# 001camellia/Speech-Imagery-EEG

Hardware: AMD Instinct MI355X
Metric: epochs/sec (B=256, C=122, T=1000) IGN 3-class (higher is better)
Workload: dtype f32

## Files before the change

### include/ign_abi.h

```cpp
#ifndef IGN_ABI_H
#define IGN_ABI_H

#include <stddef.h>
#include <stdint.h>

#ifdef __cplusplus
extern "C" {
#endif

#define IGN_ABI_VERSION 1

#define IGN_E_ARG      (-1001)
#define IGN_E_UNSUP    (-1002)
#define IGN_E_TOOBIG   (-1003)

#define IGN_DIST_L1    0
#define IGN_DIST_MSE   1
#define IGN_DIST_COS   2
#define IGN_DIST_PEARS 3
#define IGN_GATE_RBF   0x00
#define IGN_GATE_LTS   0x10

int         ign_abi_version(void);
const char* ign_last_error(void);

int ign_instnorm_fwd(const float* x_btc, float* xn_bct, float* xt_bct, int B, int T, int C, float eps,
                     void* stream);
int ign_instnorm_fwd_amax(const float* x_btc, float* xn_bct, float* xt_bct, int B, int T, int C, float eps, float* amax_slot,
                          void* stream);

int ign_transpose_btc_to_bct(const float* x_btc, float* out_bct, int B, int T, int C, void* stream);

int ign_standardise_nct_to_btc(const float* x_nct, float* out_btc, float* stats_ws, int B, int C, int T, float eps,
                               void* stream);

int ign_shapelet_fwd(const float* xn_bct, const float* w_kcl, const float* thr_kc,
                     float* p_out, float* dmin_out, int ld, int col0,
                     int32_t* tstar, float* zmu, float* d_save, float* xstat_save,
                     int B, int C, int T, int K, int L, int stride, float eps, int mode, void* stream);

int ign_shapelet_fwd_bank(const float* xn_bct, int G, const float* const* w_kcl, const float* const* thr_kc, float* p_out,
                          float* dmin_out, int ld, const int* col0, int32_t* const* tstar, float* const* zmu,
                          float* const* d_save, float* const* xstat_save, int B, int C, int T, const int* K, const int* L,
                          const int* stride, float eps, int mode, void* stream);

size_t ign_shapelet_bwd_workspace_bytes(int B, int C, int T, int K, int L, int stride, int mode);
int ign_shapelet_bwd(const float* xn_bct, const float* w_kcl, const float* g_out, const float* p_out,
                     const float* dmin_out, int ld, int col0,
                     const int32_t* tstar, const float* zmu, const float* d_save,
                     const float* xstat_save, const float* wnorm_kc ,
                     float* gw_kcl, void* workspace,
                     int B, int C, int T, int K, int L, int stride, float eps, int mode, void* stream);

size_t ign_shapelet_bwd_bank_workspace_bytes(int G, int B, int C, int T, const int* K, const int* L, const int* stride, int mode);
int ign_shapelet_bwd_bank(const float* xn_bct, int G, const float* const* w_kcl, const float* g_out, const float* p_out,
                          const float* dmin_out, int ld, const int* col0, const int32_t* const* tstar, const float* const* zmu,
                          const float* const* d_save, const float* const* xstat_save, const float* const* wnorm_kc,
                          float* const* gw_kcl, const float* const* gw_add, const float* add_scale_dev, void* workspace,
                          int B, int C, int T, const int* K, const int* L, const int* stride, float eps, int mode, void* stream);

int ign_attn_fwd(const float* q, const float* k, const float* v, float* out, float* lse,
                 int B, int L, int S, int H, int E,
                 long long q_sb, long long q_sl, long long k_sb, long long k_sl, long long v_sb, long long v_sl,
                 float scale, void* stream);
int ign_attn_fwd_x6(const float* q, const float* k, const float* v, float* out, float* lse, int B, int L, int S, int H, int E,
                    long long q_sb, long long q_sl, long long k_sb, long long k_sl, long long v_sb, long long v_sl,
                    float scale, void* stream);
int ign_attn_bwd(const float* q, const float* k, const float* v, const float* out, const float* lse, const float* gout,
                 float* gq, float* gk, float* gv, float* delta_ws,
                 int B, int L, int S, int H, int E,
                 long long q_sb, long long q_sl, long long k_sb, long long k_sl, long long v_sb, long long v_sl,
                 float scale, void* stream);
int ign_attn_bwd_x6(const float* q, const float* k, const float* v, const float* out, const float* lse, const float* gout,
                 float* gq, float* gk, float* gv, float* delta_ws,
                 int B, int L, int S, int H, int E,
                 long long q_sb, long long q_sl, long long k_sb, long long k_sl, long long v_sb, long long v_sl,
                 float scale, void* stream);
int ign_attn_fwd_bf16(const float* q, const float* k, const float* v, float* out, float* lse, int B, int L, int S, int H, int E,
                    long long q_sb, long long q_sl, long long k_sb, long long k_sl, long long v_sb, long long v_sl,
                    float scale, void* stream);
int ign_attn_bwd_bf16(const float* q, const float* k, const float* v, const float* out, const float* lse, const float* gout,
                 float* gq, float* gk, float* gv, float* delta_ws,
                 int B, int L, int S, int H, int E,
                 long long q_sb, long long q_sl, long long k_sb, long long k_sl, long long v_sb, long long v_sl,
                 float scale, void* stream);
int ign_attn_bwd_x6_strided(const float* q, const float* k, const float* v, const float* out, const float* lse, const float* gout,
                 float* gq, float* gk, float* gv, float* delta_ws,
                 int B, int L, int S, int H, int E,
                 long long q_sb, long long q_sl, long long k_sb, long long k_sl, long long v_sb, long long v_sl,
                 float scale, void* stream,
                            long long g_sb, long long g_sl, int bf16);

int ign_attn_fwd_h3(const float* q, const float* k, const float* v, float* out, float* lse,
                    int B, int L, int S, int H, int E,
                    long long q_sb, long long q_sl, long long k_sb, long long k_sl, long long v_sb, long long v_sl,
                    float scale, void* stream, const float* bq, const float* bk, const float* bv);
int ign_attn_bwd_h3(const float* q, const float* k, const float* v, const float* out, const float* lse, const float* gout,
                    float* gq, float* gk, float* gv, float* delta_ws,
                    int B, int L, int S, int H, int E,
                    long long q_sb, long long q_sl, long long k_sb, long long k_sl, long long v_sb, long long v_sl,
                    float scale, void* stream, long long g_sb, long long g_sl,
                    const float* bq, const float* bk, const float* bv, const float* bgo,
                    float* g_amax );

#define IGN_ATTN_MATH_F32  0
#define IGN_ATTN_MATH_X6   1
#define IGN_ATTN_MATH_BF16 2
#define IGN_ATTN_MATH_H3   3
int ign_attn_fwd_dropout(const float* q, const float* k, const float* v, float* out, float* lse,
                         int B, int L, int S, int H, int E,
                         long long q_sb, long long q_sl, long long k_sb, long long k_sl, long long v_sb, long long v_sl,
                         float scale, void* stream, int math, const float* bq, const float* bk, const float* bv,
                         float p, unsigned long long seed);
int ign_attn_bwd_dropout(const float* q, const float* k, const float* v, const float* out, const float* lse, const float* gout,
                         float* gq, float* gk, float* gv, float* delta_ws,
                         int B, int L, int S, int H, int E,
                         long long q_sb, long long q_sl, long long k_sb, long long k_sl, long long v_sb, long long v_sl,
                         float scale, void* stream, int math, long long g_sb, long long g_sl,
                         const float* bq, const float* bk, const float* bv, const float* bgo, float* g_amax,
                         float p, unsigned long long seed);
int ign_attn_dropout_mask(unsigned char* keep, int B, int H, int L, int S, float p, unsigned long long seed, void* stream);

int ign_head_fwd(const float* X, const float* W, const float* bias, float* out, int B, int F, int N, long long ldx,
                 void* stream);
int ign_head_bwd(const float* g_out, const float* X, const float* W, float* gX, float* gW, float* gbias,
                 int B, int F, int N, long long ldx, void* stream);
int ign_head_bwd_acc(const float* g_out, const float* X, const float* W, float* gX, float* gW, float* gbias,
                     const float* gW_add, const float* add_scale_dev, int B, int F, int N, long long ldx, void* stream);

int ign_gate_fwd(const float* sbm, const float* dnn, float* out, float* eta, int B, int N, float gating_value,
                 int use_gating_value, void* stream);
int ign_gate_bwd(const float* sbm, const float* dnn, const float* gout, const float* geta, float* gsbm, float* gdnn,
                 int B, int N, float gating_value, int use_gating_value, void* stream);

int ign_loss_fwd_bwd(const float* sbm, const float* dnn, const long long* labels, float* out, float* eta, float* loss2,
                     float* gsbm, float* gdnn, int B, int N, float beta, void* stream);
int ign_loss_fwd_bwd_reg(const float* sbm, const float* dnn, const long long* labels, const float* reg, float* out, float* eta,
                         float* loss2, float* gsbm, float* gdnn, int B, int N, float beta, void* stream);

int ign_diversity_fwd_bwd(const float* w_kcl, float* loss_part_c, float* gw_kcl, int K, int C, int L, float eps,
                          void* stream);

size_t ign_sbm_reg_workspace_bytes(int G, int C, long long nW);
int ign_sbm_reg_fwd_bwd(const float* W, float* gW_reg, long long nW, float lambda_reg, int G, const float* const* w_kcl,
                        float* const* gw_kcl, const int* K, const int* L, int C, float lambda_div, float eps, float* loss_out,
                        void* workspace, void* stream);

int ign_adam_step(float* param, const float* grad, float* exp_avg, float* exp_avg_sq, long long n, float lr,
                  float beta1, float beta2, float eps, int step, void* stream);

int ign_gather_flat(const void* const* src, const long long* off, const long long* n, int count, float* flat, void* stream);

int ign_adam_step_dev(float* param, const float* grad, float* exp_avg, float* exp_avg_sq, long long n, float lr,
                      float beta1, float beta2, float eps, int* step_dev, float* bc_dev, void* stream);

size_t ign_conv1_sumsq_workspace_bytes(int rows, int F1, int k1);
int ign_conv1_sumsq_fwd(const float* x, const float* w1, const float* mu, float* m2, void* workspace,
                        int rows, int T, int F1, int k1, int pad_left, void* stream);
int ign_conv1_sumsq_bwd(const float* x, const float* w1, const float* mu, float* g_fj, void* workspace,
                        int rows, int T, int F1, int k1, int pad_left, void* stream);

long long ign_layernorm_parts(long long R, int D);
int ign_layernorm_fwd(const float* x, const float* gamma, const float* beta, float* y, float* mean, float* rstd, long long R, int D,
                      float eps, void* stream);
int ign_layernorm_res_fwd(const float* x, const float* res, float* sum, const float* gamma, const float* beta, float* y,
                          float* mean, float* rstd, long long R, int D, float eps, void* stream);
int ign_layernorm_bwd(const float* x, const float* gy, const float* gamma, const float* mean, const float* rstd, float* gx,
                      float* dgamma, float* dbeta, float* part, long long R, int D, void* stream);
int ign_layernorm_bwd_amax(const float* x, const float* gy, const float* gamma, const float* mean, const float* rstd, float* gx,
                           float* dgamma, float* dbeta, float* part, float* amax_slot, long long R, int D, void* stream);
long long ign_autocorr_parts(int rows);
int ign_autocorr_fwd(const float* x_rows, float* part, int rows, int T, int K, void* stream);
long long ign_edge_lagprod_parts(int rows);
int ign_edge_lagprod_fwd(const float* x_rows, float* part, int rows, int T, int k, int pad_left, void* stream);
size_t ign_bn1_data_stats_workspace_bytes(int rows, int T, int k);
int ign_bn1_data_stats(const float* x_rows, int rows, int T, int k, int pad_left, void* workspace, double* G, double* S, void* stream);
int ign_autocorr_sum_fwd(const float* x_rows, float* part, float* rowsum_part, int rows, int T, int K, int* used_parts, void* stream);
int ign_bn1_fold_fwd(const float* w1, const float* gamma, const float* beta, const float* rs, const double* G, const double* S,
                     double n, float eps, float momentum, float* running_mean, float* running_var, float* alpha, float* cshift,
                     double* saved , int F1, int k, int Dm, void* stream);
int ign_bn1_fold_bwd(const float* g_alpha, const float* g_cshift, const float* w1, const float* gamma, const float* rs,
                     const double* S, const double* saved, double n, float* g_w1, float* g_gamma, float* g_beta, float* g_rs,
                     int F1, int k, int Dm, void* stream);
int ign_dwconv1d_fwd(const float* x, const float* w, float* y, int B, int C, int T, int k, int pad_left, int flip,
                     void* stream);
size_t ign_dwconv1d_bwd_weight_workspace_bytes(int B, int C, int k);
int ign_dwconv1d_bwd_weight(const float* x, const float* dy, float* dw, void* workspace, int B, int C, int T, int k,
                            int pad_left, void* stream);

int ign_chan_contract_fwd(const float* x_bct, const float* wt_ci64, float* u_bot, int B, int Ci, int Co, int T, void* stream);
size_t ign_chan_contract_bwd_weight_workspace_bytes(int B, int Ci, int Co, int T);
int ign_chan_contract_bwd_weight(const float* du_bot, const float* x_bct, float* dw_oc, void* workspace, int B, int Ci, int Co,
                                 int T, void* stream);

size_t ign_chan_stats_workspace_bytes(int B, int C);
int ign_chan_stats(const float* v_bct, double* sums_c2, void* workspace, int B, int C, int T, void* stream);
int ign_affine_elu_pool_fwd(const float* v_bct, const float* scale_c, const float* shift_c, float* out, int B, int C, int T, int P,
                            void* stream);
int ign_bn_elu_pool_bwd_sums(const float* v_bct, const float* dout, const float* scale_c, const float* shift_c, const float* mean_c,
                             double* sums_c2, void* workspace, int B, int C, int T, int P, void* stream);
int ign_bn_elu_pool_bwd_apply(const float* v_bct, const float* dout, const float* scale_c, const float* shift_c, const float* ka_c,
                              const float* kb_c, const float* kc_c, float* dv_bct, int B, int C, int T, int P, void* stream);
int ign_bn_fold_fwd(const double* sums_c2, const float* alpha_c, const float* cshift_c, const float* gamma_c, const float* beta_c,
                    float* scale_c, float* shift_c, double* fold_c2, float* running_mean, float* running_var, int C, long long n,
                    float eps, float momentum, void* stream);
int ign_bn_fold_bwd(const double* sums_c2, const double* fold_c2, const float* alpha_c, const float* gamma_c, float* ka_c, float* kb_c,
                    float* kc_c, float* dgamma_c, float* dbeta_c, float* dalpha_c, int C, long long n, float eps, void* stream);

long long ign_clconv_mtiles(long long M);
int ign_clconv_pack_weights(const float* w_oik, float* wt_fwd, float* wt_dgrad, int Co, int Ci, int k, void* stream);
int ign_clconv_fwd(const float* x, const float* wt_fwd, const float* bias, const float* pro_a, const float* pro_b,
                   float* y, float* stat_part, int B, int Tin, int Ci, int Co, int k, void* stream);
int ign_clconv_dgrad(const float* dyp, const float* wt_dgrad, const float* y_in, const float* a_in, const float* b_in,
                     const float* mean_in, const float* invstd_in, float* g_in, float* stat_part,
                     int B, int Tin, int Ci, int Co, int k, void* stream);
int ign_clconv_kpad(int C);
long long ign_clconv_x3_elems(int rows, int chans, int k);
long long ign_clconv_x6_mtiles(int B, int rows);
int ign_clconv_pack_weights_x3(const float* w_oik, void* wt3_fwd, void* wt3_dgrad, int Co, int Ci, int k, void* stream);
int ign_clconv_fwd_x6(const float* x, const void* wt3_fwd, const float* bias, const float* pro_a, const float* pro_b,
                      float* y, float* stat_part, int B, int Tin, int Ci, int Co, int k, void* stream);
int ign_clconv_dgrad_x6(const float* dyp, const void* wt3_dgrad, const float* y_in, const float* a_in, const float* b_in,
                        const float* mean_in, const float* invstd_in, float* g_in, float* stat_part,
                        int B, int Tin, int Ci, int Co, int k, void* stream);
size_t ign_clconv_wgrad_x6_workspace_bytes(int B, int Tin, int Ci, int Co, int k);
int ign_clconv_wgrad_x6(const float* dyp, int dy_pad, const float* x, const float* pro_a, const float* pro_b,
                        float* dw_oik, void* workspace, int B, int Tin, int Ci, int Co, int k, void* stream);
int ign_clconv_wgrad_x6_nsplit(int B, int Tin, int Ci, int Co, int k);
int ign_clconv_wgrad_reduce_multi(int n, const void* const* part, float* const* dw_oik, const int* nsplit, const int* Co,
                                  const int* Ci, const int* k, void* stream);
int ign_clconv_pack_weights_x3_multi(int n, const float* const* w_oik, void* const* wt3_fwd, void* const* wt3_dgrad,
                                     const int* Co, const int* Ci, const int* k, long long* const* counters, void* stream);

int ign_absmax(const float* x, long long n, float* slot , void* stream);
int ign_absmax_multi(int n, const float* const* x, const long long* count, float* const* slots, void* stream);
int ign_fcn_scan(int nl, const float* const* w, const long long* nw, const float* const* gamma_prev, const float* const* beta_prev,
                 const int* C_prev, const long long* R_prev, float* slots , float* zero, long long nzero,
                 void* stream);
int ign_clconv_pack_weights_h2_multi(int n, const float* const* w_oik, void* const* wt_fwd, void* const* wt_dgrad, const int* Co,
                                     const int* Ci, const int* k, long long* const* counters, const float* const* w_bounds,
                                     void* stream);
int ign_clconv_fwd_h3(const float* x, const void* wt_h2, const float* bias, const float* pro_a, const float* pro_b, float* y,
                      float* stat_part, const float* bound_in, const float* bound_w, int B, int Tin, int Ci, int Co, int k,
                      void* stream);
int ign_clconv_fwd_h3_amax(const float* x, const void* wt_h2, const float* bias, const float* pro_a, const float* pro_b, float* y,
                           float* stat_part, const float* bound_in, const float* bound_w, float* amax_out, int B, int Tin, int Ci,
                           int Co, int k, void* stream);
int ign_linear_dgrad_gelu_h3(const float* g, const void* wd_h2, const float* u, float* du, const float* bound_g, const float* bound_w,
                             float* amax_out, long long M, int Co, int Ci, void* stream);
int ign_clconv_dgrad_h3(const float* dyp, const void* wt_h2_dgrad, const float* y_in, const float* a_in, const float* b_in,
                        const float* mean_in, const float* invstd_in, float* g_in, float* stat_part, const float* bound_dy,
                        const float* bound_w, int B, int Tin, int Ci, int Co, int k, void* stream);
int ign_clconv_wgrad_h3(const float* dyp, int dy_pad, const float* x, const float* pro_a, const float* pro_b, float* dw_oik,
                        void* workspace, const float* bound_dy, const float* bound_x, int B, int Tin, int Ci, int Co, int k,
                        void* stream);
int ign_linear_wgrad_h3(const float* dy, const float* x, float* dw, float* db, void* workspace, const float* bound_dy,
                        const float* bound_x, long long M, int Ci, int Co, void* stream);
int ign_bn_bwd_apply_amax(const float* g, const float* y, const float* a, const float* mean, const float* invstd,
                          const float* dbeta, const float* dgamma, float* dyp, float* amax_slot, int B, int T, int C, int pad,
                          int training, void* stream);

int ign_clconv_fwd_bf16(const float* x, const void* wt3_fwd, const float* bias, const float* pro_a, const float* pro_b,
                        float* y, float* stat_part, int B, int Tin, int Ci, int Co, int k, void* stream);
int ign_clconv_dgrad_bf16(const float* dyp, const void* wt3_dgrad, const float* y_in, const float* a_in, const float* b_in,
                          const float* mean_in, const float* invstd_in, float* g_in, float* stat_part,
                          int B, int Tin, int Ci, int Co, int k, void* stream);
int ign_clconv_wgrad_bf16(const float* dyp, int dy_pad, const float* x, const float* pro_a, const float* pro_b,
                          float* dw_oik, void* workspace, int B, int Tin, int Ci, int Co, int k, void* stream);
int ign_linear_wgrad_x6(const float* dy, const float* x, float* dw, float* db, void* workspace, long long M, int Ci, int Co,
                        void* stream);
int ign_linear_wgrad_bf16(const float* dy, const float* x, float* dw, float* db, void* workspace, long long M, int Ci, int Co,
                          void* stream);
size_t ign_clconv_wgrad_workspace_bytes(int B, int Tin, int Ci, int Co, int k);
int ign_clconv_wgrad(const float* dyp, int dy_pad, const float* x, const float* pro_a, const float* pro_b,
                     float* dw_oik, void* workspace, int B, int Tin, int Ci, int Co, int k, void* stream);

int ign_bn_finalize_fwd(const float* part, int nparts, long long R, int C, const float* gamma, const float* beta,
                        float eps, float momentum, float* running_mean, float* running_var,
                        float* a, float* b, float* mean, float* invstd, void* stream);
int ign_bn_affine_eval(const float* running_mean, const float* running_var, const float* gamma, const float* beta,
                       float eps, int C, float* a, float* b, float* mean, float* invstd, void* stream);
int ign_bn_relu_pool_fwd(const float* y, const float* a, const float* b, float* pooled, int B, int T, int C, void* stream);
int ign_bn_relu_pool_head_fwd(const float* y, const float* a, const float* b, float* pooled, const float* W, const float* bias,
                              float* logits, int B, int T, int C, int N, void* stream);
long long ign_bn_relu_pool_bwd_parts(int B, int T);
int ign_bn_relu_pool_bwd(const float* y, const float* gpool, const float* a, const float* b, const float* mean,
                         const float* invstd, float* g, float* part, int B, int T, int C, void* stream);
int ign_bn_finalize_bwd(const float* part, int nparts, int C, float* dbeta, float* dgamma, void* stream);
int ign_bn_bwd_apply(const float* g, const float* y, const float* a, const float* mean, const float* invstd,
                     const float* dbeta, const float* dgamma, float* dyp, int B, int T, int C, int pad, int training,
                     void* stream);

int ign_timing_enable(int on);
int ign_timing_read(const char* label, double* total_ms, long long* launches);

#ifdef __cplusplus
}
#endif
#endif
```

### speech-imagery-eeg_amd/csrc/ign_bn.hip

```cpp
#include "ign_clconv.h"

__device__ __forceinline__ void atomic_absmax(float* slot, float v) { ign_atomic_absmax(slot, v); }
__device__ __forceinline__ float block_max_1024(float v, float* sh) {
#pragma unroll
    for (int o = 32; o > 0; o >>= 1) v = fmaxf(v, __shfl_xor(v, o, 64));
    if ((threadIdx.x & 63) == 0) sh[threadIdx.x >> 6] = v;
    __syncthreads();
    if (threadIdx.x == 0) {
        const int nw = (blockDim.x + 63) >> 6;
        for (int i = 1; i < nw; ++i) v = fmaxf(v, sh[i]);
    }
    return v;
}


constexpr int BN_CH = 8, BN_SL = 128;
__device__ __forceinline__ void bn_sum_partials(const float* __restrict__ part, int nparts, int C, double* s_out, double* q_out) {
    __shared__ double sh[2][BN_SL][BN_CH + 1];
    const int cl = threadIdx.x % BN_CH, sl = threadIdx.x / BN_CH;
    const int c = blockIdx.x * BN_CH + cl;
    double s = 0.0, q = 0.0;
    if (c < C) {
        const int per = (nparts + BN_SL - 1) / BN_SL;
        const int i0 = sl * per, i1 = min(nparts, i0 + per);
        float fs = 0.f, fq = 0.f;
        int n = 0;
        for (int i = i0; i < i1; ++i) {
            fs += part[((size_t)i * 2 + 0) * C + c];
            fq += part[((size_t)i * 2 + 1) * C + c];
            if (++n == 64) { s += (double)fs; q += (double)fq; fs = fq = 0.f; n = 0; }
        }
        s += (double)fs; q += (double)fq;
    }
    sh[0][sl][cl] = s;
    sh[1][sl][cl] = q;
    __syncthreads();
    s = q = 0.0;
    if (sl == 0) {
        for (int k = 0; k < BN_SL; ++k) { s += sh[0][k][cl]; q += sh[1][k][cl]; }
    }
    *s_out = s; *q_out = q;
}

__global__ void __launch_bounds__(1024) bn_finalize_fwd_kernel(const float* __restrict__ part, int nparts, long long R, int C,
                                       const float* __restrict__ gamma, const float* __restrict__ beta, float eps, float momentum,
                                       float* __restrict__ run_mean, float* __restrict__ run_var, float* __restrict__ a,
                                       float* __restrict__ b, float* __restrict__ mean_out, float* __restrict__ invstd_out) {
    double s, q;
    bn_sum_partials(part, nparts, C, &s, &q);
    const int c = blockIdx.x * BN_CH + threadIdx.x % BN_CH;
    if (threadIdx.x / BN_CH != 0 || c >= C) return;
    const double m = s / (double)R;
    double var = q / (double)R - m * m;
    if (var < 0.0) var = 0.0;
    const float inv = (float)(1.0 / sqrt(var + (double)eps));
    const float av = gamma[c] * inv;
    a[c] = av;
    b[c] = beta[c] - av * (float)m;
    mean_out[c] = (float)m;
    invstd_out[c] = inv;
    if (run_mean) {
        run_mean[c] = (1.f - momentum) * run_mean[c] + momentum * (float)m;
        const double unb = (R > 1) ? var * (double)R / (double)(R - 1) : var;
        run_var[c] = (1.f - momentum) * run_var[c] + momentum * (float)unb;
    }
}

__global__ void bn_affine_eval_kernel(const float* __restrict__ run_mean, const float* __restrict__ run_var,
                                      const float* __restrict__ gamma, const float* __restrict__ beta, float eps, int C,
                                      float* __restrict__ a, float* __restrict__ b, float* __restrict__ mean_out,
                                      float* __restrict__ invstd_out) {
    const int c = blockIdx.x * 256 + threadIdx.x;
    if (c >= C) return;
    const float inv = 1.f / sqrtf(run_var[c] + eps);
    const float av = gamma[c] * inv;
    a[c] = av;
    b[c] = beta[c] - av * run_mean[c];
    mean_out[c] = run_mean[c];
    invstd_out[c] = inv;
}

__global__ void __launch_bounds__(1024) bn_finalize_bwd_kernel(const float* __restrict__ part, int nparts, int C,
                                                               float* __restrict__ dbeta, float* __restrict__ dgamma) {
    double s, q;
    bn_sum_partials(part, nparts, C, &s, &q);
    const int c = blockIdx.x * BN_CH + threadIdx.x % BN_CH;
    if (threadIdx.x / BN_CH != 0 || c >= C) return;
    dbeta[c] = (float)s;
    dgamma[c] = (float)q;
}

__global__ void __launch_bounds__(256) bn_relu_pool_fwd_kernel(const float* __restrict__ y, const float* __restrict__ a,
                                                               const float* __restrict__ b, float* __restrict__ pooled, int T,
                                                               int C, const float* __restrict__ W,
                                                               const float* __restrict__ bias, float* __restrict__ logits, int N) {
    extern __shared__ float sm[];
    const int c4 = C / 4, rif = 256 / c4;
    const int col = (threadIdx.x % c4) * 4, rofs = threadIdx.x / c4;
    const float* yb = y + (size_t)blockIdx.x * T * C;
    float s[4] = {0.f, 0.f, 0.f, 0.f};
    if (rofs < rif) {
        const float4 av = *reinterpret_cast<const float4*>(a + col), bv = *reinterpret_cast<const float4*>(b + col);
        for (int t = rofs; t < T; t += rif) {
            const float4 yv = *reinterpret_cast<const float4*>(yb + (size_t)t * C + col);
            s[0] += fmaxf(fmaf(av.x, yv.x, bv.x), 0.f);
            s[1] += fmaxf(fmaf(av.y, yv.y, bv.y), 0.f);
            s[2] += fmaxf(fmaf(av.z, yv.z, bv.z), 0.f);
            s[3] += fmaxf(fmaf(av.w, yv.w, bv.w), 0.f);
        }
#pragma unroll
        for (int q = 0; q < 4; ++q) sm[rofs * C + col + q] = s[q];
    }
    __syncthreads();
    for (int c = threadIdx.x; c < C; c += 256) {
        float u = 0.f;
        for (int q = 0; q < rif; ++q) u += sm[q * C + c];
        u /= (float)T;
        pooled[(size_t)blockIdx.x * C + c] = u;
        if (W) sm[c] = u;
    }
    if (!W) return;
    __syncthreads();
    const int wave = threadIdx.x >> 6, lane = threadIdx.x & 63;
    for (int n = wave; n < N; n += 4) {
        float u = 0.f;
        for (int c = lane; c < C; c += 64) u = fmaf(sm[c], W[(size_t)n * C + c], u);
#pragma unroll
        for (int o = 32; o > 0; o >>= 1) u += __shfl_xor(u, o, 64);
        if (lane == 0) logits[(size_t)blockIdx.x * N + n] = u + (bias ? bias[n] : 0.f);
    }
}

constexpr int POOL_ROWS = 128;
__global__ void __launch_bounds__(256) bn_relu_pool_bwd_kernel(const float* __restrict__ y, const float* __restrict__ gpool,
                                                               const float* __restrict__ a, const float* __restrict__ b,
                                                               const float* __restrict__ mean, const float* __restrict__ invstd,
                                                               float* __restrict__ g, float* __restrict__ part, int T, int C) {
    extern __shared__ float sm[];
    const int c4 = C / 4, rif = 256 / c4;
    const int col = (threadIdx.x % c4) * 4, rofs = threadIdx.x / c4;
    const int bi = blockIdx.y;
    const int t0 = blockIdx.x * POOL_ROWS, t1 = min(T, t0 + POOL_ROWS);
    float s0[4] = {0.f, 0.f, 0.f, 0.f}, s1[4] = {0.f, 0.f, 0.f, 0.f};
    if (rofs < rif) {
        float av[4], bv[4], mv[4], iv[4], gp[4];
        vload<4>(av, a + col); vload<4>(bv, b + col); vload<4>(mv, mean + col); vload<4>(iv, invstd + col);
        vload<4>(gp, gpool + (size_t)bi * C + col);
        const float invT = 1.f / (float)T;
        for (int t = t0 + rofs; t < t1; t += rif) {
            const size_t off = ((size_t)bi * T + t) * C + col;
            float yy[4], gg[4];
            vload<4>(yy, y + off);
#pragma unroll
            for (int q = 0; q < 4; ++q) {
                gg[q] = (fmaf(av[q], yy[q], bv[q]) > 0.f) ? gp[q] * invT : 0.f;
                s0[q] += gg[q];
                s1[q] = fmaf(gg[q], (yy[q] - mv[q]) * iv[q], s1[q]);
            }
            vstore<4>(g + off, gg);
        }
#pragma unroll
        for (int q = 0; q < 4; ++q) { sm[rofs * C + col + q] = s0[q]; sm[(rif + rofs) * C + col + q] = s1[q]; }
    }
    __syncthreads();
    const size_t pi = (size_t)bi * gridDim.x + blockIdx.x;
    for (int c = threadIdx.x; c < C; c += 256) {
        float u = 0.f, v = 0.f;
        for (int q = 0; q < rif; ++q) { u += sm[q * C + c]; v += sm[(rif + q) * C + c]; }
        part[(pi * 2 + 0) * C + c] = u;
        part[(pi * 2 + 1) * C + c] = v;
    }
}

constexpr int APPLY_ROWS = 64;
__global__ void __launch_bounds__(256) bn_bwd_apply_kernel(const float* __restrict__ g, const float* __restrict__ y,
                                                           const float* __restrict__ a, const float* __restrict__ mean,
                                                           const float* __restrict__ invstd, const float* __restrict__ dbeta,
                                                           const float* __restrict__ dgamma, float* __restrict__ dyp, int T, int C,
                                                           int pad, long long rows_padded, float invR, int training,
                                                           float* __restrict__ amax_slot) {
    const int c4 = C / 4, rif = 256 / c4;
    const int col = (threadIdx.x % c4) * 4, rofs = threadIdx.x / c4;
    if (rofs >= rif) return;
    float amax = 0.f;
    float ca[4], c1[4], c0[4];
    vload<4>(ca, a + col);
    if (training) {
        float mv[4], iv[4], db[4], dg[4];
        vload<4>(mv, mean + col); vload<4>(iv, invstd + col); vload<4>(db, dbeta + col); vload<4>(dg, dgamma + col);
#pragma unroll
        for (int q = 0; q < 4; ++q) {
            c1[q] = -ca[q] * iv[q] * dg[q] * invR;
            c0[q] = -ca[q] * (db[q] - mv[q] * iv[q] * dg[q]) * invR;
        }
    } else {
#pragma unroll
        for (int q = 0; q < 4; ++q) c1[q] = c0[q] = 0.f;
    }
    const int Tp = T + 2 * pad;
    const long long r0 = (long long)blockIdx.x * APPLY_ROWS;
    const long long r1 = min(rows_padded, r0 + APPLY_ROWS);
    for (long long row = r0 + rofs; row < r1; row += rif) {
        const long long bi = row / Tp;
        const int tp = (int)(row - bi * Tp);
        float out[4] = {0.f, 0.f, 0.f, 0.f};
        if (tp >= pad && tp < pad + T) {
            const size_t off = ((size_t)bi * T + (tp - pad)) * C + col;
            float gg[4], yy[4] = {0.f, 0.f, 0.f, 0.f};
            vload<4>(gg, g + off);
            if (training) vload<4>(yy, y + off);
#pragma unroll
            for (int q = 0; q < 4; ++q) { out[q] = fmaf(ca[q], gg[q], fmaf(c1[q], yy[q], c0[q])); amax = fmaxf(amax, fabsf(out[q])); }
        }
        vstore<4>(dyp + (size_t)row * C + col, out);
    }
    if (amax_slot) {
#pragma unroll
        for (int o = 32; o > 0; o >>= 1) amax = fmaxf(amax, __shfl_xor(amax, o, 64));
        if ((threadIdx.x & 63) == 0) atomic_absmax(amax_slot, amax);
    }
}

__global__ void __launch_bounds__(256) absmax_kernel(const float* __restrict__ x, long long n, float* __restrict__ slot) {
    __shared__ float sh[16];
    float m = 0.f;
    const long long n4 = n >> 2;
    for (long long i = (long long)blockIdx.x * 256 + threadIdx.x; i < n4; i += (long long)gridDim.x * 256) {
        const float4 v = reinterpret_cast<const float4*>(x)[i];
        m = fmaxf(fmaxf(m, fmaxf(fabsf(v.x), fabsf(v.y))), fmaxf(fabsf(v.z), fabsf(v.w)));
    }
    if (blockIdx.x == 0)
        for (long long i = (n4 << 2) + threadIdx.x; i < n; i += 256) m = fmaxf(m, fabsf(x[i]));
    m = block_max_1024(m, sh);
    if (threadIdx.x == 0) atomic_absmax(slot, m);
}

constexpr int AMM_MAX = 16;
struct AbsmaxMultiTable { const float* x[AMM_MAX]; long long n[AMM_MAX]; float* slot[AMM_MAX]; };
__global__ void __launch_bounds__(256) absmax_multi_kernel(const AbsmaxMultiTable t) {
    __shared__ float sh[16];
    const int g = blockIdx.y;
    const float* __restrict__ x = t.x[g];
    const long long n = t.n[g];
    float m = 0.f;
    if (((uintptr_t)x & 15) == 0) {
        const long long n4 = n >> 2;
        for (long long i = (long long)blockIdx.x * 256 + threadIdx.x; i < n4; i += (long long)gridDim.x * 256) {
            const float4 v = reinterpret_cast<const float4*>(x)[i];
            m = fmaxf(fmaxf(m, fmaxf(fabsf(v.x), fabsf(v.y))), fmaxf(fabsf(v.z), fabsf(v.w)));
        }
        if (blockIdx.x == 0)
            for (long long i = (n4 << 2) + threadIdx.x; i < n; i += 256) m = fmaxf(m, fabsf(x[i]));
    } else {
        for (long long i = (long long)blockIdx.x * 256 + threadIdx.x; i < n; i += (long long)gridDim.x * 256) m = fmaxf(m, fabsf(x[i]));
    }
    m = block_max_1024(m, sh);
    if (threadIdx.x == 0) atomic_absmax(t.slot[g], m);
}

constexpr int SCAN_LMAX = 8;
struct FcnScanTable {
    const float* w[SCAN_LMAX]; long long nw[SCAN_LMAX];
    const float* gamma[SCAN_LMAX]; const float* beta[SCAN_LMAX]; int C[SCAN_LMAX]; float sqrtR[SCAN_LMAX];
};
__global__ void __launch_bounds__(1024) fcn_scan_kernel(const FcnScanTable t, float* __restrict__ slots, float* __restrict__ zero,
                                                        long long nzero) {
    __shared__ float sh[16];
    const int l = blockIdx.x;
    for (long long i = (long long)l * 1024 + threadIdx.x; i < nzero; i += (long long)gridDim.x * 1024) zero[i] = 0.f;
    float m = 0.f;
    for (long long i = threadIdx.x; i < t.nw[l]; i += 1024) m = fmaxf(m, fabsf(t.w[l][i]));
    m = block_max_1024(m, sh);
    if (threadIdx.x == 0) slots[4 * l + 0] = m;
    __syncthreads();
    float a = 0.f;
    if (t.gamma[l])
        for (int c = threadIdx.x; c < t.C[l]; c += 1024) a = fmaxf(a, fmaf(fabsf(t.gamma[l][c]), t.sqrtR[l], fabsf(t.beta[l][c])));
    a = block_max_1024(a, sh);
    if (threadIdx.x == 0) { slots[4 * l + 1] = a; slots[4 * l + 2] = 0.f; slots[4 * l + 3] = 0.f; }
}

extern "C" int ign_absmax(const float* x, long long n, float* slot, void* stream) {
    if (!x || !slot || n <= 0 || ((uintptr_t)x & 15)) { ign_set_error("ign_absmax: null / unaligned pointer or n <= 0"); return IGN_E_ARG; }
    const long long blocks = (n / 4 + 256 * 8 - 1) / (256 * 8);
    IgnScopedTimer tm("absmax", (hipStream_t)stream);
    hipLaunchKernelGGL(absmax_kernel, dim3((unsigned)(blocks < 1 ? 1 : (blocks > 2048 ? 2048 : blocks))), dim3(256), 0,
                       (hipStream_t)stream, x, n, slot);
    return ign_check_launch("absmax_kernel");
}

extern "C" int ign_absmax_multi(int n, const float* const* x, const long long* count, float* const* slots, void* stream) {
    if (n <= 0 || n > AMM_MAX || !x || !count || !slots) { ign_set_error("ign_absmax_multi: n=%d outside 1..%d or null table", n, AMM_MAX); return IGN_E_ARG; }
    AbsmaxMultiTable t;
    long long nmax = 0;
    for (int i = 0; i < n; ++i) {
        if (!x[i] || !slots[i] || count[i] <= 0) { ign_set_error("ign_absmax_multi: tensor %d: null pointer or empty", i); return IGN_E_ARG; }
        t.x[i] = x[i]; t.n[i] = count[i]; t.slot[i] = slots[i];
        nmax = count[i] > nmax ? count[i] : nmax;
    }
    long long blocks = (nmax / 4 + 256 * 8 - 1) / (256 * 8);
    blocks = blocks < 1 ? 1 : (blocks > 256 ? 256 : blocks);
    IgnScopedTimer tm("absmax", (hipStream_t)stream);
    hipLaunchKernelGGL(absmax_multi_kernel, dim3((unsigned)blocks, (unsigned)n), dim3(256), 0, (hipStream_t)stream, t);
    return ign_check_launch("absmax_multi_kernel");
}

extern "C" int ign_fcn_scan(int nl, const float* const* w, const long long* nw, const float* const* gamma_prev,
                            const float* const* beta_prev, const int* C_prev, const long long* R_prev, float* slots, float* zero,
                            long long nzero, void* stream) {
    if (nzero < 0 || (nzero > 0 && !zero)) { ign_set_error("ign_fcn_scan: nzero=%lld with zero=%p", nzero, (void*)zero); return IGN_E_ARG; }
    if (nl <= 0 || nl > SCAN_LMAX || !w || !nw || !slots) { ign_set_error("ign_fcn_scan: nl=%d outside 1..%d or null table", nl, SCAN_LMAX); return IGN_E_ARG; }
    FcnScanTable t;
    for (int l = 0; l < nl; ++l) {
        if (!w[l] || nw[l] <= 0) { ign_set_error("ign_fcn_scan: layer %d: null weights", l); return IGN_E_ARG; }
        t.w[l] = w[l]; t.nw[l] = nw[l];
        const bool has = gamma_prev && gamma_prev[l];
        if (has && (!beta_prev || !beta_prev[l] || !C_prev || !R_prev || C_prev[l] <= 0 || R_prev[l] <= 1)) {
            ign_set_error("ign_fcn_scan: layer %d: BatchNorm in front needs beta, C > 0 and R > 1", l);
            return IGN_E_ARG;
        }
        t.gamma[l] = has ? gamma_prev[l] : nullptr; t.beta[l] = has ? beta_prev[l] : nullptr;
        t.C[l] = has ? C_prev[l] : 0; t.sqrtR[l] = has ? sqrtf((float)(R_prev[l] - 1)) : 0.f;
    }
    hipLaunchKernelGGL(fcn_scan_kernel, dim3(nl), dim3(1024), 0, (hipStream_t)stream, t, slots, zero, nzero);
    return ign_check_launch("fcn_scan_kernel");
}

static int bn_check(const char* who, long long R, int C) {
    if (R <= 0 || C <= 0 || (C & 3) || C > 1024) {
        ign_set_error("%s: need R > 0 and 4 <= C <= 1024 with C %% 4 == 0 (R=%lld C=%d)", who, R, C);
        return IGN_E_ARG;
    }
    return 0;
}

extern "C" int ign_bn_finalize_fwd(const float* part, int nparts, long long R, int C, const float* gamma, const float* beta,
                                   float eps, float momentum, float* running_mean, float* running_var, float* a, float* b,
                                   float* mean, float* invstd, void* stream) {
    if (!part || nparts <= 0 || R <= 0 || C <= 0 || !gamma || !beta || !a || !b || !mean || !invstd) {
        ign_set_error("ign_bn_finalize_fwd: bad argument");
        return IGN_E_ARG;
    }
    hipLaunchKernelGGL(bn_finalize_fwd_kernel, dim3((C + BN_CH - 1) / BN_CH), dim3(BN_CH * BN_SL), 0, (hipStream_t)stream, part, nparts, R, C, gamma, beta,
                       eps, momentum, running_mean, running_var, a, b, mean, invstd);
    return ign_check_launch("bn_finalize_fwd_kernel");
}

extern "C" int ign_bn_affine_eval(const float* running_mean, const float* running_var, const float* gamma, const float* beta,
                                  float eps, int C, float* a, float* b, float* mean, float* invstd, void* stream) {
    if (!running_mean || !running_var || !gamma || !beta || C <= 0 || !a || !b || !mean || !invstd) {
        ign_set_error("ign_bn_affine_eval: bad argument");
        return IGN_E_ARG;
    }
    hipLaunchKernelGGL(bn_affine_eval_kernel, dim3((C + 255) / 256), dim3(256), 0, (hipStream_t)stream, running_mean, running_var,
                       gamma, beta, eps, C, a, b, mean, invstd);
    return ign_check_launch("bn_affine_eval_kernel");
}

extern "C" int ign_bn_finalize_bwd(const float* part, int nparts, int C, float* dbeta, float* dgamma, void* stream) {
    if (!part || nparts <= 0 || C <= 0 || !dbeta || !dgamma) {
        ign_set_error("ign_bn_finalize_bwd: bad argument");
        return IGN_E_ARG;
    }
    hipLaunchKernelGGL(bn_finalize_bwd_kernel, dim3((C + BN_CH - 1) / BN_CH), dim3(BN_CH * BN_SL), 0, (hipStream_t)stream, part, nparts, C, dbeta, dgamma);
    return ign_check_launch("bn_finalize_bwd_kernel");
}

extern "C" int ign_bn_relu_pool_fwd(const float* y, const float* a, const float* b, float* pooled, int B, int T, int C,
                                    void* stream) {
    int rc;
    if ((rc = bn_check("ign_bn_relu_pool_fwd", (long long)B * T, C))) return rc;
    if (!y || !a || !b || !pooled) { ign_set_error("ign_bn_relu_pool_fwd: null pointer"); return IGN_E_ARG; }
    const int rif = 256 / (C / 4);
    IgnScopedTimer tm("bn_relu_pool_fwd", (hipStream_t)stream);
    hipLaunchKernelGGL(bn_relu_pool_fwd_kernel, dim3(B), dim3(256), (size_t)rif * C * 4, (hipStream_t)stream, y, a, b, pooled, T, C,
                       (const float*)nullptr, (const float*)nullptr, (float*)nullptr, 0);
    return ign_check_launch("bn_relu_pool_fwd_kernel");
}

extern "C" int ign_bn_relu_pool_head_fwd(const float* y, const float* a, const float* b, float* pooled, const float* W,
                                         const float* bias, float* logits, int B, int T, int C, int N, void* stream) {
    int rc;
    if ((rc = bn_check("ign_bn_relu_pool_head_fwd", (long long)B * T, C))) return rc;
    if (!y || !a || !b || !pooled || !W || !logits || N <= 0) {
        ign_set_error("ign_bn_relu_pool_head_fwd: null pointer or N=%d", N);
        return IGN_E_ARG;
    }
    const int rif = 256 / (C / 4);
    IgnScopedTimer tm("bn_relu_pool_fwd", (hipStream_t)stream);
    hipLaunchKernelGGL(bn_relu_pool_fwd_kernel, dim3(B), dim3(256), (size_t)rif * C * 4, (hipStream_t)stream, y, a, b, pooled, T, C,
                       W, bias, logits, N);
    return ign_check_launch("bn_relu_pool_fwd_kernel");
}

extern "C" long long ign_bn_relu_pool_bwd_parts(int B, int T) { return (long long)B * ((T + POOL_ROWS - 1) / POOL_ROWS); }

extern "C" int ign_bn_relu_pool_bwd(const float* y, const float* gpool, const float* a, const float* b, const float* mean,
                                    const float* invstd, float* g, float* part, int B, int T, int C, void* stream) {
    int rc;
    if ((rc = bn_check("ign_bn_relu_pool_bwd", (long long)B * T, C))) return rc;
    if (!y || !gpool || !a || !b || !mean || !invstd || !g || !part) { ign_set_error("ign_bn_relu_pool_bwd: null pointer"); return IGN_E_ARG; }
    const int rif = 256 / (C / 4);
    IgnScopedTimer tm("bn_relu_pool_bwd", (hipStream_t)stream);
    hipLaunchKernelGGL(bn_relu_pool_bwd_kernel, dim3((T + POOL_ROWS - 1) / POOL_ROWS, B), dim3(256), (size_t)2 * rif * C * 4,
                       (hipStream_t)stream, y, gpool, a, b, mean, invstd, g, part, T, C);
    return ign_check_launch("bn_relu_pool_bwd_kernel");
}

extern "C" int ign_bn_bwd_apply(const float* g, const float* y, const float* a, const float* mean, const float* invstd,
                                const float* dbeta, const float* dgamma, float* dyp, int B, int T, int C, int pad, int training,
                                void* stream) {
    return ign_bn_bwd_apply_amax(g, y, a, mean, invstd, dbeta, dgamma, dyp, nullptr, B, T, C, pad, training, stream);
}

extern "C" int ign_bn_bwd_apply_amax(const float* g, const float* y, const float* a, const float* mean, const float* invstd,
                                     const float* dbeta, const float* dgamma, float* dyp, float* amax_slot, int B, int T, int C,
                                     int pad, int training, void* stream) {
    int rc;
    if ((rc = bn_check("ign_bn_bwd_apply", (long long)B * T, C))) return rc;
    if (!g || !a || !dyp || pad < 0 || (training && (!y || !mean || !invstd || !dbeta || !dgamma))) {
        ign_set_error("ign_bn_bwd_apply: null pointer / negative pad");
        return IGN_E_ARG;
    }
    const long long rows = (long long)B * (T + 2 * pad);
    IgnScopedTimer tm("bn_bwd_apply", (hipStream_t)stream);
    hipLaunchKernelGGL(bn_bwd_apply_kernel, dim3((unsigned)((rows + APPLY_ROWS - 1) / APPLY_ROWS)), dim3(256), 0, (hipStream_t)stream,
                       g, y, a, mean, invstd, dbeta, dgamma, dyp, T, C, pad, rows, 1.0f / (float)((long long)B * T), training, amax_slot);
    return ign_check_launch("bn_bwd_apply_kernel");
}
```

### speech-imagery-eeg_amd/csrc/ign_clconv.h

```cpp
#pragma once
#include "ign_common.h"

typedef float f32x16 __attribute__((ext_vector_type(16)));
#define MFMA32(a, b, c) __builtin_amdgcn_mfma_f32_32x32x2f32((a), (b), (c), 0, 0, 0)

__device__ __forceinline__ int acc_row16(int r, int h) { return (r & 3) + 8 * (r >> 2) + 4 * h; }

constexpr int TM = 128, TN = 128, KC = 16;
constexpr int NT_PITCH = KC + 4;
constexpr int TN_PITCH = 128 + 8;

struct RowMap {
    int rows_logical;
    int row0;
    int row_pitch;
    long long sample_pitch;
};
__device__ __forceinline__ long long row_off(const RowMap& rm, int m) {
    const int s = m / rm.rows_logical;
    const int r = m - s * rm.rows_logical;
    return (long long)s * rm.sample_pitch + (long long)(rm.row0 + r) * rm.row_pitch;
}

template <int V> struct VecT;
template <> struct VecT<1> { typedef float T; };
template <> struct VecT<2> { typedef float2 T; };
template <> struct VecT<4> { typedef float4 T; };

template <int V>
__device__ __forceinline__ void vload(float (&d)[V], const float* p) {
    if (V == 4) { const float4 t = *reinterpret_cast<const float4*>(p); d[0] = t.x; d[1] = t.y; d[2] = t.z; d[3] = t.w; }
    else if (V == 2) { const float2 t = *reinterpret_cast<const float2*>(p); d[0] = t.x; d[1] = t.y; }
    else d[0] = *p;
}
template <int V>
__device__ __forceinline__ void vstore(float* p, const float (&d)[V]) {
    if (V == 4) *reinterpret_cast<float4*>(p) = make_float4(d[0], d[1], d[2], d[3]);
    else if (V == 2) *reinterpret_cast<float2*>(p) = make_float2(d[0], d[1]);
    else *p = d[0];
}

enum { EPI_BIAS_STATS = 0, EPI_MASK_STATS = 1, EPI_GELU_BWD = 2 };

__device__ __forceinline__ float ign_gelu_grad(float u) {
    const float cdf = 0.5f * (1.f + erff(u * 0.70710678118654752f));
    const float pdf = 0.3989422804014327f * expf(-0.5f * u * u);
    return fmaf(u, pdf, cdf);
}

struct GemmNTArgs {
    const float* A; RowMap am; int K;
    const float* Bt; int ldb;
    float* C; int M, N;
    const float* bias;
    const float* pro_a; const float* pro_b; int pro_c;
    float* part;
    const float* ey; const float* ea; const float* eb; const float* emean; const float* einv;
    int mtiles, ntiles;
    const unsigned short* B3; int Kp;
    float* amax_out;
};

template <int EPI, bool FULL, bool SC = false>
__device__ __forceinline__ void nt_epilogue_body(const GemmNTArgs& a, const f32x16 (&acc)[2][2], float (&s1)[2], float (&s2)[2],
                                                 int m0, int n0, int m_lim, float osc = 1.f) {
    const int lane = threadIdx.x & 63, wave = threadIdx.x >> 6;
    const int l31 = lane & 31, h = lane >> 5;
    const int wm = wave & 1, wn = wave >> 1;
    float amax = 0.f;
#pragma unroll
    for (int j = 0; j < 2; ++j) {
        const int n = n0 + wn * 64 + j * 32 + l31;
        const bool n_ok = FULL || n < a.N;
        const int nc = n_ok ? n : a.N - 1;
        const float bv = (EPI == EPI_BIAS_STATS && a.bias) ? a.bias[nc] : 0.f;
        float ea = 0.f, eb = 0.f, em = 0.f, ei = 0.f;
        if (EPI == EPI_MASK_STATS) { ea = a.ea[nc]; eb = a.eb[nc]; em = a.emean[nc]; ei = a.einv[nc]; }
#pragma unroll
        for (int i = 0; i < 2; ++i) {
            const int mb = m0 + wm * 64 + i * 32;
            float yv[16];
            if (EPI == EPI_MASK_STATS || EPI == EPI_GELU_BWD) {
#pragma unroll
                for (int r = 0; r < 16; ++r) {
                    const int m = mb + acc_row16(r, h);
                    const int mc = FULL ? m : min(m, m_lim - 1);
                    yv[r] = a.ey[(long long)mc * a.N + nc];
                }
            }
#pragma unroll
            for (int r = 0; r < 16; ++r) {
                const int m = mb + acc_row16(r, h);
                const bool ok = FULL || (n_ok && m < m_lim);
                float v = SC ? acc[i][j][r] * osc : acc[i][j][r];
                if (EPI == EPI_BIAS_STATS) {
                    v += bv;
                    if (ok) { s1[j] += v; s2[j] = fmaf(v, v, s2[j]); }
                } else if (EPI == EPI_GELU_BWD) {
                    v *= ign_gelu_grad(yv[r]);
                } else {
                    v = (fmaf(ea, yv[r], eb) > 0.f) ? v : 0.f;
                    if (ok) { s1[j] += v; s2[j] = fmaf(v, (yv[r] - em) * ei, s2[j]); }
                }
                if (ok) a.C[(long long)m * a.N + n] = v;
                if (SC && ok) amax = fmaxf(amax, fabsf(v));
            }
        }
    }
    if (SC && a.amax_out) {
#pragma unroll
        for (int o = 32; o > 0; o >>= 1) amax = fmaxf(amax, __shfl_xor(amax, o, 64));
        if (lane == 0) ign_atomic_absmax(a.amax_out, amax);
    }
}

template <int EPI, bool SC = false>
__device__ __forceinline__ void nt_epilogue(const GemmNTArgs& a, const f32x16 (&acc)[2][2], float* red, int mt, int m0, int n0,
                                            int m_lim, float osc = 1.f) {
    const int tid = threadIdx.x, lane = tid & 63, wave = tid >> 6;
    const int l31 = lane & 31, h = lane >> 5;
    const int wm = wave & 1, wn = wave >> 1;
    float s1[2] = {0.f, 0.f}, s2[2] = {0.f, 0.f};
    if (m0 + TM <= m_lim && n0 + TN <= a.N) nt_epilogue_body<EPI, true, SC>(a, acc, s1, s2, m0, n0, m_lim, osc);
    else nt_epilogue_body<EPI, false, SC>(a, acc, s1, s2, m0, n0, m_lim, osc);
    if (a.part) {
#pragma unroll
        for (int j = 0; j < 2; ++j) {
            s1[j] += __shfl_xor(s1[j], 32, 64);
            s2[j] += __shfl_xor(s2[j], 32, 64);
            if (h == 0) {
                const int col = wn * 64 + j * 32 + l31;
                red[(wm * 2 + 0) * TN + col] = s1[j];
                red[(wm * 2 + 1) * TN + col] = s2[j];
            }
        }
        __syncthreads();
        if (tid < TN && n0 + tid < a.N) {
            a.part[((long long)mt * 2 + 0) * a.N + n0 + tid] = red[0 * TN + tid] + red[2 * TN + tid];
            a.part[((long long)mt * 2 + 1) * a.N + n0 + tid] = red[1 * TN + tid] + red[3 * TN + tid];
        }
    }
}


struct ConvX6Args {
    GemmNTArgs g;
    long long sample_pitch;
    int rows_in;
    int cin, cp, k;
    int trows;
    int tps;
    int nprod;
    const float* bound_a;
    const float* bound_b;
};

__device__ __forceinline__ float ign_pow2_scale(const float* bound) {
    if (!bound) return 1.f;
    const float b = *bound;
    if (!(b > 0.f) || !(b < INFINITY)) return 1.f;
    int e;
    (void)frexpf(b, &e);
    e = 14 - e;
    e = e < -60 ? -60 : (e > 60 ? 60 : e);
    return ldexpf(1.f, e);
}

inline int ign_vec_width(int c) { return (c % 4 == 0) ? 4 : (c % 2 == 0) ? 2 : 1; }

int ign_clconv_launch_x6t(const ConvX6Args& a, int epi, int V, bool pro, hipStream_t s);
int ign_clconv_launch_wgrad_reduce(const float* part, float* dw_oik, int nsplit, int Co, int Ci, int k, hipStream_t s);
```

### speech-imagery-eeg_amd/csrc/ign_clconv_f32.hip

```cpp
#include "ign_clconv.h"

template <int V, bool PRO, int EPI>
__global__ void __launch_bounds__(256, 2) clconv_nt_kernel(const GemmNTArgs a) {
    constexpr int VPR = KC / V;
    constexpr int RPP = 256 / VPR;
    constexpr int NPASS = TM / RPP;
    __shared__ __attribute__((aligned(16))) float smem[2][(TM + TN) * NT_PITCH];

    const int nwg = a.mtiles * a.ntiles;
    int lid = blockIdx.x;
    {
        const int per = nwg / 8;
        if (lid < per * 8) lid = (lid & 7) * per + (lid >> 3);
    }
    const int mt = lid / a.ntiles, nt = lid - mt * a.ntiles;
    const int m0 = mt * TM, n0 = nt * TN;

    const int tid = threadIdx.x, lane = tid & 63, wave = tid >> 6;
    const int l31 = lane & 31, h = lane >> 5;
    const int wm = wave & 1, wn = wave >> 1;

    const int sq = tid % VPR, sr = tid / VPR;
    const float* arow[NPASS];
    const float* brow[NPASS];
// ... 148 lines not shown
#pragma unroll
                for (int v = 0; v < VQ; ++v) rq[i][v] = 0.f;
                rq_ok[i] = false;
            }
        }
    };
    auto lstore = [&](int buf) {
        float* Ps = smem[buf];
        float* Qs = Ps + KC * TN_PITCH;
#pragma unroll
        for (int i = 0; i < 2; ++i) vstore<4>(Ps + (pr + 8 * i) * TN_PITCH + pc, rp[i]);
#pragma unroll
        for (int i = 0; i < QNPASS; ++i) {
            if (PRO && rq_ok[i]) {
#pragma unroll
                for (int v = 0; v < VQ; ++v) rq[i][v] = fmaxf(fmaf(qa[v], rq[i][v], qb[v]), 0.f);
            }
            vstore<VQ>(Qs + (qr + QRPP * i) * TN_PITCH + qc, rq[i]);
        }
    };

    if (m_begin < m_end) {
        gload(m_begin);
        lstore(0);
    }
    __syncthreads();
    int buf = 0;
    for (int mb = m_begin; mb < m_end; mb += KC, buf ^= 1) {
        if (mb + KC < m_end) gload(mb + KC);
        const float* Ps = smem[buf] + h * TN_PITCH + wm * 64 + 2 * l31;
        const float* Qs = smem[buf] + KC * TN_PITCH + h * TN_PITCH + wn * 64 + 2 * l31;
#pragma unroll
        for (int s = 0; s < KC / 2; ++s) {
            const float2 pv = *reinterpret_cast<const float2*>(Ps + 2 * s * TN_PITCH);
            const float2 qv = *reinterpret_cast<const float2*>(Qs + 2 * s * TN_PITCH);
            acc[0][0] = MFMA32(pv.x, qv.x, acc[0][0]);
            acc[0][1] = MFMA32(pv.x, qv.y, acc[0][1]);
            acc[1][0] = MFMA32(pv.y, qv.x, acc[1][0]);
            acc[1][1] = MFMA32(pv.y, qv.y, acc[1][1]);
        }
        if (mb + KC < m_end) lstore(buf ^ 1);
        __syncthreads();
    }

    float* out = a.part + (long long)split * a.NP * a.NQ;
    const int kk = q0 + wn * 64 + 2 * l31;
#pragma unroll
    for (int i = 0; i < 2; ++i)
#pragma unroll
        for (int r = 0; r < 16; ++r) {
            const int co = p0 + wm * 64 + 2 * acc_row16(r, h) + i;
            if (co < a.NP) {
                float* o = out + (long long)co * a.NQ + kk;
                if (!(a.NQ & 1) && kk + 1 < a.NQ) {
                    *reinterpret_cast<float2*>(o) = make_float2(acc[i][0][r], acc[i][1][r]);
                } else {
                    if (kk < a.NQ) o[0] = acc[i][0][r];
                    if (kk + 1 < a.NQ) o[1] = acc[i][1][r];
                }
            }
        }
}

__global__ void __launch_bounds__(256) wgrad_reduce_kernel(const float* __restrict__ part, float* __restrict__ dw, int nsplit,
                                                           int Co, int Ci, int k) {
    const long long n = (long long)Co * Ci * k;
    const long long i = (long long)blockIdx.x * 256 + threadIdx.x;
    if (i >= n) return;
    float s = 0.f;
    int p = 0;
    for (; p + 8 <= nsplit; p += 8) {
        float v[8];
#pragma unroll
        for (int u = 0; u < 8; ++u) v[u] = part[(long long)(p + u) * n + i];
#pragma unroll
        for (int u = 0; u < 8; ++u) s += v[u];
    }
    for (; p < nsplit; ++p) s += part[(long long)p * n + i];
    const int ci = (int)(i % Ci);
    const long long t = i / Ci;
    const int j = (int)(t % k);
    const long long co = t / k;
    dw[(co * Ci + ci) * k + j] = s;
}

constexpr int WRED_LMAX = 8;
struct WgradReduceTable {
    const float* part[WRED_LMAX];
    float* dw[WRED_LMAX];
    int nsplit[WRED_LMAX], Co[WRED_LMAX], Ci[WRED_LMAX], k[WRED_LMAX];
};
__global__ void __launch_bounds__(256) wgrad_reduce_multi_kernel(const WgradReduceTable t) {
    const int l = blockIdx.y;
    const int Co = t.Co[l], Ci = t.Ci[l], k = t.k[l], nsplit = t.nsplit[l];
    const float* __restrict__ part = t.part[l];
    const long long n = (long long)Co * Ci * k;
    const long long i = (long long)blockIdx.x * 256 + threadIdx.x;
    if (i >= n) return;
    float s = 0.f;
    int p = 0;
    for (; p + 8 <= nsplit; p += 8) {
        float v[8];
#pragma unroll
        for (int u = 0; u < 8; ++u) v[u] = part[(long long)(p + u) * n + i];
#pragma unroll
        for (int u = 0; u < 8; ++u) s += v[u];
    }
    for (; p < nsplit; ++p) s += part[(long long)p * n + i];
    const int ci = (int)(i % Ci);
    const long long tt = i / Ci;
    const int j = (int)(tt % k);
    const long long co = tt / k;
    t.dw[l][(co * Ci + ci) * k + j] = s;
}

extern "C" int ign_clconv_wgrad_reduce_multi(int n, const void* const* part, float* const* dw_oik, const int* nsplit, const int* Co,
                                             const int* Ci, const int* k, void* stream) {
    if (n <= 0 || n > WRED_LMAX || !part || !dw_oik || !nsplit || !Co || !Ci || !k) {
        ign_set_error("ign_clconv_wgrad_reduce_multi: n=%d outside 1..%d or null table", n, WRED_LMAX);
        return IGN_E_ARG;
    }
    WgradReduceTable t;
    long long nmax = 0;
    for (int l = 0; l < n; ++l) {
        if (!part[l] || !dw_oik[l] || nsplit[l] <= 0 || Co[l] <= 0 || Ci[l] <= 0 || k[l] <= 0) {
            ign_set_error("ign_clconv_wgrad_reduce_multi: layer %d: bad argument", l);
            return IGN_E_ARG;
        }
        t.part[l] = (const float*)part[l]; t.dw[l] = dw_oik[l]; t.nsplit[l] = nsplit[l]; t.Co[l] = Co[l]; t.Ci[l] = Ci[l]; t.k[l] = k[l];
        const long long e = (long long)Co[l] * Ci[l] * k[l];
        nmax = e > nmax ? e : nmax;
    }
    hipLaunchKernelGGL(wgrad_reduce_multi_kernel, dim3((unsigned)((nmax + 255) / 256), (unsigned)n), dim3(256), 0, (hipStream_t)stream, t);
    return ign_check_launch("wgrad_reduce_multi_kernel");
}

__global__ void __launch_bounds__(256) pack_weights_kernel(const float* __restrict__ w, float* __restrict__ wt,
                                                           float* __restrict__ wd, int Co, int Ci, int k) {
    const long long n = (long long)Co * Ci * k;
    const long long i = (long long)blockIdx.x * 256 + threadIdx.x;
    if (i >= n) return;
    const int j = (int)(i % k);
    const long long t = i / k;
    const int ci = (int)(t % Ci);
    const long long co = t / Ci;
    const float v = w[i];
    wt[(co * k + j) * Ci + ci] = v;
    if (wd) wd[((long long)ci * k + (k - 1 - j)) * Co + co] = v;
}

template <int EPI>
static int launch_nt(const GemmNTArgs& a, int V, bool pro, hipStream_t s) {
    const dim3 grid((unsigned)(a.mtiles * a.ntiles)), block(256);
#define IGN_NT(VV, PP) hipLaunchKernelGGL((clconv_nt_kernel<VV, PP, EPI>), grid, block, 0, s, a)
    if (V == 4) { if (pro) IGN_NT(4, true); else IGN_NT(4, false); }
    else if (V == 2) { if (pro) IGN_NT(2, true); else IGN_NT(2, false); }
    else { if (pro) IGN_NT(1, true); else IGN_NT(1, false); }
#undef IGN_NT
    return ign_check_launch("clconv_nt_kernel");
}

extern "C" long long ign_clconv_mtiles(long long M) { return (M + TM - 1) / TM; }

extern "C" int ign_clconv_pack_weights(const float* w_oik, float* wt_fwd, float* wt_dgrad, int Co, int Ci, int k, void* stream) {
    if (!w_oik || !wt_fwd || Co <= 0 || Ci <= 0 || k <= 0) {
        ign_set_error("ign_clconv_pack_weights: bad argument (Co=%d Ci=%d k=%d)", Co, Ci, k);
        return IGN_E_ARG;
    }
    const long long n = (long long)Co * Ci * k;
    hipLaunchKernelGGL(pack_weights_kernel, dim3((unsigned)((n + 255) / 256)), dim3(256), 0, (hipStream_t)stream, w_oik, wt_fwd,
                       wt_dgrad, Co, Ci, k);
    return ign_check_launch("pack_weights_kernel");
}

static int clconv_fwd_impl(const char* who, int x6, const float* x, const void* wt, const float* bias, const float* pro_a,
                           const float* pro_b, float* y, float* stat_part, int B, int Tin, int Ci, int Co, int k, void* stream,
                           const float* bound_a = nullptr, const float* bound_w = nullptr, float* amax_out = nullptr,
                           int epi = EPI_BIAS_STATS, const float* ey = nullptr) {
    const int Tout = Tin - k + 1;
    if (!x || !wt || !y || B <= 0 || Ci <= 0 || Co <= 0 || k <= 0 || Tout <= 0 || ((pro_a == nullptr) != (pro_b == nullptr))) {
        ign_set_error("%s: bad argument (B=%d Tin=%d Ci=%d Co=%d k=%d)", who, B, Tin, Ci, Co, k);
        return IGN_E_ARG;
    }
    const long long M = (long long)B * Tout;
    if (M > 0x7fffffffLL / 2) { ign_set_error("%s: B*Tout = %lld rows exceed the 2^30 row index space", who, M); return IGN_E_TOOBIG; }
    GemmNTArgs a{};
    a.A = x; a.am = RowMap{Tout, 0, Ci, (long long)Tin * Ci}; a.K = k * Ci;
    a.Bt = x6 ? nullptr : (const float*)wt; a.ldb = k * Ci; a.C = y; a.M = (int)M; a.N = Co; a.bias = bias;
    a.B3 = x6 ? (const unsigned short*)wt : nullptr; a.Kp = 0;
    a.pro_a = pro_a; a.pro_b = pro_b; a.pro_c = Ci; a.part = stat_part; a.amax_out = amax_out; a.ey = ey;
    a.mtiles = (int)((M + TM - 1) / TM); a.ntiles = (Co + TN - 1) / TN;
    IgnScopedTimer tm("clconv_fwd", (hipStream_t)stream);
    if (x6) {
        if (k > 16) { ign_set_error("%s: k=%d > 16 taps", who, k); return IGN_E_UNSUP; }
        ConvX6Args c{};
        c.g = a;
        c.cin = Ci; c.cp = (Ci + 15) / 16 * 16; c.k = k; c.g.Kp = k * c.cp;
        c.sample_pitch = (long long)Tin * Ci; c.rows_in = Tin; c.trows = Tout; c.tps = (Tout + TM - 1) / TM;
        c.g.mtiles = B * c.tps; c.nprod = x6; c.bound_a = bound_a; c.bound_b = bound_w;
        return ign_clconv_launch_x6t(c, epi, ign_vec_width(Ci), pro_a != nullptr, (hipStream_t)stream);
    }
    if (epi != EPI_BIAS_STATS) { ign_set_error("%s: epilogue %d needs the split kernels", who, epi); return IGN_E_UNSUP; }
    return launch_nt<EPI_BIAS_STATS>(a, ign_vec_width(Ci), pro_a != nullptr, (hipStream_t)stream);
}

extern "C" int ign_clconv_fwd(const float* x, const float* wt, const float* bias, const float* pro_a, const float* pro_b,
                              float* y, float* stat_part, int B, int Tin, int Ci, int Co, int k, void* stream) {
    return clconv_fwd_impl("ign_clconv_fwd", 0, x, wt, bias, pro_a, pro_b, y, stat_part, B, Tin, Ci, Co, k, stream);
}

extern "C" int ign_clconv_fwd_x6(const float* x, const void* wt3, const float* bias, const float* pro_a, const float* pro_b,
                                 float* y, float* stat_part, int B, int Tin, int Ci, int Co, int k, void* stream) {
    return clconv_fwd_impl("ign_clconv_fwd_x6", 6, x, wt3, bias, pro_a, pro_b, y, stat_part, B, Tin, Ci, Co, k, stream);
}

extern "C" int ign_clconv_fwd_bf16(const float* x, const void* wt3, const float* bias, const float* pro_a, const float* pro_b,
                                   float* y, float* stat_part, int B, int Tin, int Ci, int Co, int k, void* stream) {
    return clconv_fwd_impl("ign_clconv_fwd_bf16", 1, x, wt3, bias, pro_a, pro_b, y, stat_part, B, Tin, Ci, Co, k, stream);
}

extern "C" int ign_clconv_fwd_h3(const float* x, const void* wt_h2, const float* bias, const float* pro_a, const float* pro_b,
                                 float* y, float* stat_part, const float* bound_in, const float* bound_w, int B, int Tin, int Ci,
                                 int Co, int k, void* stream) {
    return ign_clconv_fwd_h3_amax(x, wt_h2, bias, pro_a, pro_b, y, stat_part, bound_in, bound_w, nullptr, B, Tin, Ci, Co, k, stream);
}

extern "C" int ign_clconv_fwd_h3_amax(const float* x, const void* wt_h2, const float* bias, const float* pro_a, const float* pro_b,
                                      float* y, float* stat_part, const float* bound_in, const float* bound_w, float* amax_out, int B,
                                      int Tin, int Ci, int Co, int k, void* stream) {
    if (!bound_in || !bound_w) { ign_set_error("ign_clconv_fwd_h3: null operand bound"); return IGN_E_ARG; }
    return clconv_fwd_impl("ign_clconv_fwd_h3", 3, x, wt_h2, bias, pro_a, pro_b, y, stat_part, B, Tin, Ci, Co, k, stream, bound_in,
                           bound_w, amax_out);
}

extern "C" int ign_linear_dgrad_gelu_h3(const float* g, const void* wd_h2, const float* u, float* du, const float* bound_g,
                                        const float* bound_w, float* amax_out, long long M, int Co, int Ci, void* stream) {
    if (!bound_g || !bound_w || !u) { ign_set_error("ign_linear_dgrad_gelu_h3: null bound / pre-activation"); return IGN_E_ARG; }
    if (M <= 0 || M > 0x3fffffffLL || Ci % 256 || Co % 4) {
        ign_set_error("ign_linear_dgrad_gelu_h3: needs 0 < M < 2^30, Ci %% 256 == 0, Co %% 4 == 0 (M=%lld Co=%d Ci=%d)", M, Co, Ci);
        return IGN_E_UNSUP;
    }
    return clconv_fwd_impl("ign_linear_dgrad_gelu_h3", 3, g, wd_h2, nullptr, nullptr, nullptr, du, nullptr, 1, (int)M, Co, Ci, 1, stream,
                           bound_g, bound_w, amax_out, EPI_GELU_BWD, u);
}

static int clconv_dgrad_impl(const char* who, int x6, const float* dyp, const void* wt_dgrad, const float* y_in, const float* a_in,
                             const float* b_in, const float* mean_in, const float* invstd_in, float* g_in, float* stat_part, int B,
                             int Tin, int Ci, int Co, int k, void* stream, const float* bound_a = nullptr,
                             const float* bound_w = nullptr) {
    const int Tout = Tin - k + 1;
    if (!dyp || !wt_dgrad || !y_in || !a_in || !b_in || !mean_in || !invstd_in || !g_in || B <= 0 || Ci <= 0 || Co <= 0 || k <= 0 ||
        Tout <= 0) {
        ign_set_error("%s: bad argument (B=%d Tin=%d Ci=%d Co=%d k=%d)", who, B, Tin, Ci, Co, k);
        return IGN_E_ARG;
    }
    const long long M = (long long)B * Tin;
    if (M > 0x7fffffffLL / 2) { ign_set_error("%s: B*Tin = %lld rows exceed the 2^30 row index space", who, M); return IGN_E_TOOBIG; }
    GemmNTArgs a{};
    a.A = dyp; a.am = RowMap{Tin, 0, Co, (long long)(Tout + 2 * (k - 1)) * Co}; a.K = k * Co;
    a.Bt = x6 ? nullptr : (const float*)wt_dgrad; a.ldb = k * Co; a.C = g_in; a.M = (int)M; a.N = Ci;
    a.B3 = x6 ? (const unsigned short*)wt_dgrad : nullptr; a.Kp = 0;
    a.part = stat_part; a.ey = y_in; a.ea = a_in; a.eb = b_in; a.emean = mean_in; a.einv = invstd_in;
    a.mtiles = (int)((M + TM - 1) / TM); a.ntiles = (Ci + TN - 1) / TN;
    IgnScopedTimer tm("clconv_dgrad", (hipStream_t)stream);
    if (x6) {
        if (k > 16) { ign_set_error("%s: k=%d > 16 taps", who, k); return IGN_E_UNSUP; }
        ConvX6Args c{};
        c.g = a;
        c.cin = Co; c.cp = (Co + 15) / 16 * 16; c.k = k; c.g.Kp = k * c.cp;
        c.sample_pitch = (long long)(Tout + 2 * (k - 1)) * Co; c.rows_in = Tout + 2 * (k - 1); c.trows = Tin; c.tps = (Tin + TM - 1) / TM;
        c.g.mtiles = B * c.tps; c.nprod = x6; c.bound_a = bound_a; c.bound_b = bound_w;
        return ign_clconv_launch_x6t(c, EPI_MASK_STATS, ign_vec_width(Co), false, (hipStream_t)stream);
    }
    return launch_nt<EPI_MASK_STATS>(a, ign_vec_width(Co), false, (hipStream_t)stream);
}

extern "C" int ign_clconv_dgrad(const float* dyp, const float* wt_dgrad, const float* y_in, const float* a_in, const float* b_in,
                                const float* mean_in, const float* invstd_in, float* g_in, float* stat_part, int B, int Tin,
                                int Ci, int Co, int k, void* stream) {
    return clconv_dgrad_impl("ign_clconv_dgrad", 0, dyp, wt_dgrad, y_in, a_in, b_in, mean_in, invstd_in, g_in, stat_part, B, Tin,
                             Ci, Co, k, stream);
}

extern "C" int ign_clconv_dgrad_x6(const float* dyp, const void* wt3_dgrad, const float* y_in, const float* a_in, const float* b_in,
                                   const float* mean_in, const float* invstd_in, float* g_in, float* stat_part, int B, int Tin,
                                   int Ci, int Co, int k, void* stream) {
    return clconv_dgrad_impl("ign_clconv_dgrad_x6", 6, dyp, wt3_dgrad, y_in, a_in, b_in, mean_in, invstd_in, g_in, stat_part, B,
                             Tin, Ci, Co, k, stream);
}

extern "C" int ign_clconv_dgrad_bf16(const float* dyp, const void* wt3_dgrad, const float* y_in, const float* a_in, const float* b_in,
                                     const float* mean_in, const float* invstd_in, float* g_in, float* stat_part, int B, int Tin,
                                     int Ci, int Co, int k, void* stream) {
    return clconv_dgrad_impl("ign_clconv_dgrad_bf16", 1, dyp, wt3_dgrad, y_in, a_in, b_in, mean_in, invstd_in, g_in, stat_part, B,
                             Tin, Ci, Co, k, stream);
}

extern "C" int ign_clconv_dgrad_h3(const float* dyp, const void* wt_h2_dgrad, const float* y_in, const float* a_in, const float* b_in,
                                   const float* mean_in, const float* invstd_in, float* g_in, float* stat_part, const float* bound_dy,
                                   const float* bound_w, int B, int Tin, int Ci, int Co, int k, void* stream) {
    if (!bound_dy || !bound_w) { ign_set_error("ign_clconv_dgrad_h3: null operand bound"); return IGN_E_ARG; }
    return clconv_dgrad_impl("ign_clconv_dgrad_h3", 3, dyp, wt_h2_dgrad, y_in, a_in, b_in, mean_in, invstd_in, g_in, stat_part, B,
                             Tin, Ci, Co, k, stream, bound_dy, bound_w);
}

static int wgrad_splits(long long M, int tiles) {
    long long s = (1024 + tiles - 1) / tiles;
    const long long max_s = (M + 8 * KC - 1) / (8 * KC);
    if (s > max_s) s = max_s;
    if (s < 1) s = 1;
    return (int)s;
}

extern "C" size_t ign_clconv_wgrad_workspace_bytes(int B, int Tin, int Ci, int Co, int k) {
    const int Tout = Tin - k + 1;
    if (B <= 0 || Tout <= 0 || Ci <= 0 || Co <= 0) return 0;
    const int tiles = ((Co + 127) / 128) * ((k * Ci + 127) / 128);
    return (size_t)wgrad_splits((long long)B * Tout, tiles) * Co * k * Ci * sizeof(float);
}

extern "C" int ign_clconv_wgrad(const float* dyp, int dy_pad, const float* x, const float* pro_a, const float* pro_b,
                                float* dw_oik, void* workspace, int B, int Tin, int Ci, int Co, int k, void* stream) {
    static const char* who = "ign_clconv_wgrad";
    const int Tout = Tin - k + 1;
    if (!dyp || !x || !dw_oik || !workspace || B <= 0 || Ci <= 0 || Co <= 0 || k <= 0 || Tout <= 0 || dy_pad < 0 ||
        ((pro_a == nullptr) != (pro_b == nullptr))) {
        ign_set_error("%s: bad argument (B=%d Tin=%d Ci=%d Co=%d k=%d pad=%d)", who, B, Tin, Ci, Co, k, dy_pad);
        return IGN_E_ARG;
    }
    if (Co % 4) { ign_set_error("%s: Co=%d must be a multiple of 4", who, Co); return IGN_E_UNSUP; }
    const long long M = (long long)B * Tout;
    if (M > 0x7fffffffLL / 2) { ign_set_error("%s: B*Tout = %lld rows exceed the 2^30 row index space", who, M); return IGN_E_TOOBIG; }
    hipStream_t s = (hipStream_t)stream;
    GemmTNArgs a{};
    a.P = dyp; a.pm = RowMap{Tout, dy_pad, Co, (long long)(Tout + 2 * dy_pad) * Co}; a.NP = Co;
    a.Q = x; a.qm = RowMap{Tout, 0, Ci, (long long)Tin * Ci}; a.NQ = k * Ci;
    a.pro_a = pro_a; a.pro_b = pro_b; a.pro_c = Ci;
    a.part = (float*)workspace; a.M = (int)M;
    a.ptiles = (Co + 127) / 128; a.qtiles = (k * Ci + 127) / 128;
    a.nsplit = wgrad_splits(M, a.ptiles * a.qtiles);
    const dim3 grid((unsigned)(a.ptiles * a.qtiles), (unsigned)a.nsplit), block(256);
    const int V = ign_vec_width(Ci);
    const bool pro = pro_a != nullptr;
    {
        IgnScopedTimer tm("clconv_wgrad", s);
#define IGN_TN(VV, PP) hipLaunchKernelGGL((clconv_tn_kernel<VV, PP>), grid, block, 0, s, a)
        if (V == 4) { if (pro) IGN_TN(4, true); else IGN_TN(4, false); }
        else if (V == 2) { if (pro) IGN_TN(2, true); else IGN_TN(2, false); }
        else { if (pro) IGN_TN(1, true); else IGN_TN(1, false); }
#undef IGN_TN
    }
    int rc;
    if ((rc = ign_check_launch("clconv_tn_kernel"))) return rc;
    return ign_clconv_launch_wgrad_reduce((const float*)workspace, dw_oik, a.nsplit, Co, Ci, k, s);
}

int ign_clconv_launch_wgrad_reduce(const float* part, float* dw_oik, int nsplit, int Co, int Ci, int k, hipStream_t s) {
    const long long n = (long long)Co * Ci * k;
    hipLaunchKernelGGL(wgrad_reduce_kernel, dim3((unsigned)((n + 255) / 256)), dim3(256), 0, s, part, dw_oik, nsplit, Co, Ci, k);
    return ign_check_launch("wgrad_reduce_kernel");
}
```

### speech-imagery-eeg_amd/csrc/ign_clconv_x6.hip

```cpp
#include "ign_clconv.h"

typedef __bf16 bf16x8 __attribute__((ext_vector_type(8)));
constexpr int X6_PITCH = KC + 8;
constexpr int X6_PLANE = TM * X6_PITCH;
constexpr int X6_BLOCK = 3 * TN * KC;

typedef float f32x2 __attribute__((ext_vector_type(2)));
typedef __bf16 bf16x2 __attribute__((ext_vector_type(2)));
__device__ __forceinline__ void split3_pair(f32x2 v, bf16x2& x0, bf16x2& x1, bf16x2& x2) {
    x0 = __builtin_convertvector(v, bf16x2);
    f32x2 r = v - __builtin_convertvector(x0, f32x2);
    x1 = __builtin_convertvector(r, bf16x2);
    r -= __builtin_convertvector(x1, f32x2);
    x2 = __builtin_convertvector(r, bf16x2);
}
template <int V>
__device__ __forceinline__ void split3_store(const float (&t)[V], __bf16* d, int plane);
template <>
__device__ __forceinline__ void split3_store<1>(const float (&t)[1], __bf16* d, int plane);
__device__ __forceinline__ void split3(float v, __bf16& x0, __bf16& x1, __bf16& x2) {
    x0 = (__bf16)v;
    float r = v - (float)x0;
    x1 = (__bf16)r;
    r -= (float)x1;
    x2 = (__bf16)r;
}
template <>
__device__ __forceinline__ void split3_store<1>(const float (&t)[1], __bf16* d, int plane) {
    __bf16 x0, x1, x2;
    split3(t[0], x0, x1, x2);
    d[0] = x0; d[plane] = x1; d[2 * plane] = x2;
}
template <>
__device__ __forceinline__ void split3_store<2>(const float (&t)[2], __bf16* d, int plane) {
    bf16x2 x0, x1, x2;
    split3_pair(f32x2{t[0], t[1]}, x0, x1, x2);
    *reinterpret_cast<bf16x2*>(d) = x0;
    *reinterpret_cast<bf16x2*>(d + plane) = x1;
    *reinterpret_cast<bf16x2*>(d + 2 * plane) = x2;
}
template <>
__device__ __forceinline__ void split3_store<4>(const float (&t)[4], __bf16* d, int plane) {
    typedef __bf16 bf16x4 __attribute__((ext_vector_type(4)));
    bf16x2 a0, a1, a2, b0, b1, b2;
    split3_pair(f32x2{t[0], t[1]}, a0, a1, a2);
    split3_pair(f32x2{t[2], t[3]}, b0, b1, b2);
    *reinterpret_cast<bf16x4*>(d) = __builtin_shufflevector(a0, b0, 0, 1, 2, 3);
    *reinterpret_cast<bf16x4*>(d + plane) = __builtin_shufflevector(a1, b1, 0, 1, 2, 3);
    *reinterpret_cast<bf16x4*>(d + 2 * plane) = __builtin_shufflevector(a2, b2, 0, 1, 2, 3);
}

typedef _Float16 f16x2 __attribute__((ext_vector_type(2)));
typedef _Float16 f16x4 __attribute__((ext_vector_type(4)));
typedef _Float16 f16x8 __attribute__((ext_vector_type(8)));
__device__ __forceinline__ void split2h_pair(f32x2 v, f16x2& x0, f16x2& x1) {
    x0 = __builtin_convertvector(v, f16x2);
    x1 = __builtin_convertvector(v - __builtin_convertvector(x0, f32x2), f16x2);
}
template <int V>
__device__ __forceinline__ void split2h_store(const float (&t)[V], __bf16* d, int plane) {
    _Float16* dh = reinterpret_cast<_Float16*>(d);
    if constexpr (V == 1) {
        const _Float16 x0 = (_Float16)t[0];
        dh[0] = x0; dh[plane] = (_Float16)(t[0] - (float)x0);
    } else if constexpr (V == 2) {
        f16x2 x0, x1;
        split2h_pair(f32x2{t[0], t[1]}, x0, x1);
        *reinterpret_cast<f16x2*>(dh) = x0;
        *reinterpret_cast<f16x2*>(dh + plane) = x1;
    } else {
        f16x2 a0, a1, b0, b1;
        split2h_pair(f32x2{t[0], t[1]}, a0, a1);
        split2h_pair(f32x2{t[2], t[3]}, b0, b1);
        *reinterpret_cast<f16x4*>(dh) = __builtin_shufflevector(a0, b0, 0, 1, 2, 3);
        *reinterpret_cast<f16x4*>(dh + plane) = __builtin_shufflevector(a1, b1, 0, 1, 2, 3);
    }
}

template <int V, int NP>
__device__ __forceinline__ void split_store(const float (&t)[V], __bf16* d, int plane) {
    if constexpr (NP == 3) {
        split3_store<V>(t, d, plane);
    } else if constexpr (NP == 2) {
        split2h_store<V>(t, d, plane);
    } else if constexpr (V == 1) {
        d[0] = (__bf16)t[0];
    } else if constexpr (V == 2) {
        *reinterpret_cast<bf16x2*>(d) = __builtin_convertvector(f32x2{t[0], t[1]}, bf16x2);
    } else {
        typedef __bf16 bf16x4 __attribute__((ext_vector_type(4)));
        const bf16x2 a = __builtin_convertvector(f32x2{t[0], t[1]}, bf16x2), b = __builtin_convertvector(f32x2{t[2], t[3]}, bf16x2);
        *reinterpret_cast<bf16x4*>(d) = __builtin_shufflevector(a, b, 0, 1, 2, 3);
    }
}

template <int NP>
__device__ __forceinline__ f32x16 mfma16(const bf16x8& a, const bf16x8& b, const f32x16& c) {
    if constexpr (NP == 2)
        return __builtin_amdgcn_mfma_f32_32x32x16_f16(__builtin_bit_cast(f16x8, a), __builtin_bit_cast(f16x8, b), c, 0, 0, 0);
    else
        return __builtin_amdgcn_mfma_f32_32x32x16_bf16(a, b, c, 0, 0, 0);
}

#ifndef IGN_H3_WAVES
#define IGN_H3_WAVES 3
#endif
constexpr int X6T_SPAN = TM + 15;
constexpr int X6T_APLANE = X6T_SPAN * X6_PITCH;

template <int NP> struct X6tLds {
    static constexpr int NPL = (NP == 2) ? 2 : 3;
    static constexpr int ABUF = NPL * X6T_APLANE, BBUF = NPL * X6_PLANE;
    static constexpr size_t BYTES = (size_t)2 * (ABUF + BBUF) * sizeof(unsigned short);
};
template <int NP, int EPI> struct X6tWaves { static constexpr int N = (NP == 2 && EPI == EPI_BIAS_STATS) ? IGN_H3_WAVES : 2; };
template <int V, bool PRO, int EPI, int NP>
__global__ void __launch_bounds__(256, (X6tWaves<NP, EPI>::N)) clconv_x6t_kernel(const ConvX6Args ca) {
    const GemmNTArgs& a = ca.g;
    constexpr int VPR = KC / V;
    constexpr int APASS = (X6T_SPAN * VPR + 255) / 256;
    constexpr int X6T_ABUF = X6tLds<NP>::ABUF, X6T_BBUF = X6tLds<NP>::BBUF;
    extern __shared__ __attribute__((aligned(16))) unsigned short smem16[];
    __bf16* Abuf = reinterpret_cast<__bf16*>(smem16);
    __bf16* Bbuf = Abuf + 2 * X6T_ABUF;

    const int nwg = a.mtiles * a.ntiles;
    int lid = blockIdx.x;
    {
        const int per = nwg / 8;
        if (lid < per * 8) lid = (lid & 7) * per + (lid >> 3);
    }
    const int mt = lid / a.ntiles, nt = lid - mt * a.ntiles;
    const int bi = mt / ca.tps, tt = mt - bi * ca.tps;
    const int t0 = tt * TM, n0 = nt * TN;
    const int tid = threadIdx.x, lane = tid & 63, wave = tid >> 6;
    const int l31 = lane & 31, h = lane >> 5;
    const int wm = wave & 1, wn = wave >> 1;
    const int span = TM + ca.k - 1;
    const int nvec = span * VPR;

    const float* abase = a.A + (long long)bi * ca.sample_pitch;
    const int brw = tid >> 1, bh = tid & 1;
    const unsigned short* bsrc = a.B3 + (size_t)nt * (size_t)(ca.cp / KC) * ca.k * X6_BLOCK + (size_t)brw * KC + 8 * bh;
    constexpr size_t bplane = (size_t)TN * KC;

    f32x16 acc[2][2];
#pragma unroll
    for (int i = 0; i < 2; ++i)
#pragma unroll
        for (int j = 0; j < 2; ++j)
#pragma unroll
            for (int r = 0; r < 16; ++r) acc[i][j][r] = 0.f;

    float ra[APASS][V];
    float pa[V], pb[V];
    bool a_ok = false;
    uint4 rb00, rb01 = {}, rb02 = {}, rb10, rb11 = {}, rb12 = {};
    const int ncc = ca.cp / KC;
    const int nstep = ncc * ca.k;

    const float sa = (NP == 2) ? ign_pow2_scale(ca.bound_a) : 1.f;
    const float osc = (NP == 2) ? 1.f / (sa * ign_pow2_scale(ca.bound_b)) : 1.f;
    auto aload = [&](int cc) {
        const int ch = cc * KC + (tid % VPR) * V;
        a_ok = ch < ca.cin;
        if (PRO && a_ok) {
            vload<V>(pa, a.pro_a + ch); vload<V>(pb, a.pro_b + ch);
            if constexpr (NP == 2) {
#pragma unroll
                for (int v = 0; v < V; ++v) { pa[v] *= sa; pb[v] *= sa; }
            }
        }
#pragma unroll
        for (int p = 0; p < APASS; ++p) {
            const int idx = tid + p * 256;
            const int row = idx / VPR;
            if (a_ok && idx < nvec) vload<V>(ra[p], abase + (long long)min(t0 + row, ca.rows_in - 1) * ca.cin + ch);
            else {
#pragma unroll
                for (int v = 0; v < V; ++v) ra[p][v] = 0.f;
            }
        }
    };
    auto astore = [&](int buf) {
        __bf16* st = Abuf + buf * X6T_ABUF;
#pragma unroll
        for (int p = 0; p < APASS; ++p) {
            const int idx = tid + p * 256;
            if (idx < nvec) {
                const int row = idx / VPR, q = idx - row * VPR;
                float tv[V];
#pragma unroll
                for (int v = 0; v < V; ++v) {
                    tv[v] = ra[p][v];
                    if (PRO && a_ok) tv[v] = fmaxf(fmaf(pa[v], tv[v], pb[v]), 0.f);
                    else if (NP == 2) tv[v] *= sa;
                }
                split_store<V, NP>(tv, st + row * X6_PITCH + q * V, X6T_APLANE);
            }
        }
    };
    auto boff = [&](int st) {
        st = min(st, nstep - 1);
        return (size_t)st * X6_BLOCK;
    };
    auto bstore = [&](int buf, const uint4& r0, const uint4& r1, const uint4& r2) {
        __bf16* st = Bbuf + buf * X6T_BBUF + brw * X6_PITCH + 8 * bh;
        *reinterpret_cast<uint4*>(st) = r0;
        if constexpr (NP >= 2) *reinterpret_cast<uint4*>(st + X6_PLANE) = r1;
        if constexpr (NP == 3) *reinterpret_cast<uint4*>(st + 2 * X6_PLANE) = r2;
    };
#define IGN_BLOAD(r0, r1, r2, st)                                                                       \
    do {                                                                                                \
        const size_t off_ = boff(st);                                                                   \
        r0 = *reinterpret_cast<const uint4*>(bsrc + off_);                                              \
        if constexpr (NP >= 2) r1 = *reinterpret_cast<const uint4*>(bsrc + bplane + off_);              \
        if constexpr (NP == 3) r2 = *reinterpret_cast<const uint4*>(bsrc + 2 * bplane + off_);          \
    } while (0)

    aload(0);
    IGN_BLOAD(rb00, rb01, rb02, 0);
    IGN_BLOAD(rb10, rb11, rb12, 1);
    astore(0);
    bstore(0, rb00, rb01, rb02);
    __syncthreads();

    int cc = 0, j = 0;
    auto body = [&](int step, bool odd) {
        if (odd) IGN_BLOAD(rb10, rb11, rb12, step + 2);
        else IGN_BLOAD(rb00, rb01, rb02, step + 2);
        const bool next_span = cc + 1 < ncc;
        if (j == 0 && next_span) aload(cc + 1);
        const __bf16* As = Abuf + (cc & 1) * X6T_ABUF + (wm * 64 + l31 + j) * X6_PITCH + 8 * h;
        const __bf16* Bs = Bbuf + (step & 1) * X6T_BBUF + (wn * 64 + l31) * X6_PITCH + 8 * h;
        bf16x8 af[2][NP], bf[2][NP];
#pragma unroll
        for (int i = 0; i < 2; ++i)
#pragma unroll
            for (int pl = 0; pl < NP; ++pl) {
                af[i][pl] = *reinterpret_cast<const bf16x8*>(As + pl * X6T_APLANE + i * 32 * X6_PITCH);
                bf[i][pl] = *reinterpret_cast<const bf16x8*>(Bs + pl * X6_PLANE + i * 32 * X6_PITCH);
            }
        __builtin_amdgcn_sched_barrier(0);
#define IGN_X6(pa_, pb_)                                                                                   \
        acc[0][0] = mfma16<NP>(af[0][pa_], bf[0][pb_], acc[0][0]);                                         \
        acc[0][1] = mfma16<NP>(af[0][pa_], bf[1][pb_], acc[0][1]);                                         \
        acc[1][0] = mfma16<NP>(af[1][pa_], bf[0][pb_], acc[1][0]);                                         \
        acc[1][1] = mfma16<NP>(af[1][pa_], bf[1][pb_], acc[1][1]);
        if constexpr (NP == 3) { IGN_X6(2, 0) IGN_X6(0, 2) IGN_X6(1, 1) IGN_X6(1, 0) IGN_X6(0, 1) }
        if constexpr (NP == 2) { IGN_X6(1, 0) IGN_X6(0, 1) }
        IGN_X6(0, 0)
#undef IGN_X6
        __builtin_amdgcn_sched_barrier(0);
        if (odd) bstore((step + 1) & 1, rb00, rb01, rb02);
        else bstore((step + 1) & 1, rb10, rb11, rb12);
        if (j + 1 == ca.k) {
            if (next_span) astore((cc + 1) & 1);
            j = 0; ++cc;
        } else {
            ++j;
        }
        __syncthreads();
    };
    for (int step = 0; step < nstep; step += 2) {
        body(step, false);
        if (step + 1 < nstep) body(step + 1, true);
    }
#undef IGN_BLOAD
    const int m0 = bi * ca.trows + t0;
    nt_epilogue<EPI, NP == 2>(a, acc, reinterpret_cast<float*>(smem16), mt, m0, n0, bi * ca.trows + min(ca.trows, t0 + TM), osc);
}

#ifndef IGN_H3W_WAVES
#define IGN_H3W_WAVES 2
#endif
template <int NP> struct X6wLds {
    static constexpr int NPL = NP == 3 ? 3 : (NP == 2 ? 2 : 1);
    static constexpr int ABUF = NPL * TM * X6_PITCH;
    static constexpr int BBUF = 2 * NPL * X6_PLANE;
    static constexpr size_t BYTES = (size_t)2 * (ABUF + BBUF) * sizeof(unsigned short);
    static constexpr int WAVES = NP == 2 ? IGN_H3W_WAVES : 2;
};

template <int NP, int EPI = EPI_BIAS_STATS>
__global__ void __launch_bounds__(512, X6wLds<NP>::WAVES) clconv_x6w_kernel(const ConvX6Args ca) {
    const GemmNTArgs& a = ca.g;
    extern __shared__ __attribute__((aligned(16))) unsigned short smem16[];
    constexpr int X6W_ABUF = X6wLds<NP>::ABUF, X6W_BBUF = X6wLds<NP>::BBUF, NPL = X6wLds<NP>::NPL;
    __bf16* Abuf = reinterpret_cast<__bf16*>(smem16);
    __bf16* Bbuf = Abuf + 2 * X6W_ABUF;
    constexpr int APLANE = TM * X6_PITCH;

    const int ntw = a.N / 256;
    const int nwg = a.mtiles * ntw;
    int lid = blockIdx.x;
    {
        const int per = nwg / 8;
        if (lid < per * 8) lid = (lid & 7) * per + (lid >> 3);
    }
    const int mt = lid / ntw, nw = lid - mt * ntw;
    const int m0 = mt * TM, n0 = nw * 256;
    const int tid = threadIdx.x, lane = tid & 63, wave = tid >> 6;
    const int l31 = lane & 31, h = lane >> 5;
    const int wm = wave & 1, wn = wave >> 1;
    const int ncc = ca.cp / KC;

    f32x16 acc[2][2];
#pragma unroll
    for (int i = 0; i < 2; ++i)
#pragma unroll
        for (int j = 0; j < 2; ++j)
#pragma unroll
            for (int r = 0; r < 16; ++r) acc[i][j][r] = 0.f;

    const int arow = tid >> 2, ach = (tid & 3) * 4;
    const float* ap = a.A + (long long)min(m0 + arow, a.M - 1) * ca.cin + ach;
    float ra0[4], ra1[4];
    const int bt = tid >> 8, brw = (tid & 255) >> 1, bh = tid & 1;
    const unsigned short* bsrc = a.B3 + (size_t)(2 * nw + bt) * (size_t)ncc * X6_BLOCK + (size_t)brw * KC + 8 * bh;
    constexpr size_t bplane = (size_t)TN * KC;
    uint4 rb00, rb01 = {}, rb02 = {}, rb10, rb11 = {}, rb12 = {};

    const float sa = (NP == 2) ? ign_pow2_scale(ca.bound_a) : 1.f;
    const float osc = (NP == 2) ? 1.f / (sa * ign_pow2_scale(ca.bound_b)) : 1.f;
#define IGN_ALOADW(ra_, cc_)                                                                 \
    do {                                                                                     \
        const int c_ = min((cc_), ncc - 1);                                                  \
        if (c_ * KC + ach < ca.cin) vload<4>(ra_, ap + c_ * KC);           \
        else ra_[0] = ra_[1] = ra_[2] = ra_[3] = 0.f;                                        \
    } while (0)
    auto astore = [&](int buf, const float (&r)[4]) {
        if constexpr (NP == 2) {
            const float rs[4] = {r[0] * sa, r[1] * sa, r[2] * sa, r[3] * sa};
            split_store<4, NP>(rs, Abuf + buf * X6W_ABUF + arow * X6_PITCH + ach, APLANE);
        } else {
            split_store<4, NP>(r, Abuf + buf * X6W_ABUF + arow * X6_PITCH + ach, APLANE);
        }
    };
    auto bstore = [&](int buf, const uint4& r0, const uint4& r1, const uint4& r2) {
        __bf16* st = Bbuf + buf * X6W_BBUF + bt * NPL * X6_PLANE + brw * X6_PITCH + 8 * bh;
        *reinterpret_cast<uint4*>(st) = r0;
        if constexpr (NP >= 2) *reinterpret_cast<uint4*>(st + X6_PLANE) = r1;
        if constexpr (NP == 3) *reinterpret_cast<uint4*>(st + 2 * X6_PLANE) = r2;
    };
#define IGN_BLOADW(r0, r1, r2, st)                                                                      \
    do {                                                                                                \
        const size_t off_ = (size_t)min((st), ncc - 1) * X6_BLOCK;                                      \
        r0 = *reinterpret_cast<const uint4*>(bsrc + off_);                                              \
        if constexpr (NP >= 2) r1 = *reinterpret_cast<const uint4*>(bsrc + bplane + off_);              \
        if constexpr (NP == 3) r2 = *reinterpret_cast<const uint4*>(bsrc + 2 * bplane + off_);          \
    } while (0)

    IGN_ALOADW(ra0, 0);
    IGN_BLOADW(rb00, rb01, rb02, 0);
    IGN_ALOADW(ra1, 1);
    IGN_BLOADW(rb10, rb11, rb12, 1);
    astore(0, ra0);
    bstore(0, rb00, rb01, rb02);
    __syncthreads();

    const bool late = wave >= 4;
    auto mm = [&](int step) {
        const __bf16* As = Abuf + (step & 1) * X6W_ABUF + (wm * 64 + l31) * X6_PITCH + 8 * h;
        const __bf16* Bs = Bbuf + (step & 1) * X6W_BBUF + (wn >> 1) * NPL * X6_PLANE + ((wn & 1) * 64 + l31) * X6_PITCH + 8 * h;
        bf16x8 af[2][NP], bf[2][NP];
#pragma unroll
        for (int i = 0; i < 2; ++i)
#pragma unroll
            for (int pl = 0; pl < NP; ++pl) {
                af[i][pl] = *reinterpret_cast<const bf16x8*>(As + pl * APLANE + i * 32 * X6_PITCH);
                bf[i][pl] = *reinterpret_cast<const bf16x8*>(Bs + pl * X6_PLANE + i * 32 * X6_PITCH);
            }
        __builtin_amdgcn_sched_barrier(0);
#define IGN_X6(pa_, pb_)                                                                                   \
        acc[0][0] = mfma16<NP>(af[0][pa_], bf[0][pb_], acc[0][0]);                                         \
        acc[0][1] = mfma16<NP>(af[0][pa_], bf[1][pb_], acc[0][1]);                                         \
        acc[1][0] = mfma16<NP>(af[1][pa_], bf[0][pb_], acc[1][0]);                                         \
        acc[1][1] = mfma16<NP>(af[1][pa_], bf[1][pb_], acc[1][1]);
        if constexpr (NP == 3) { IGN_X6(2, 0) IGN_X6(0, 2) IGN_X6(1, 1) }
        if constexpr (NP >= 2) { IGN_X6(1, 0) IGN_X6(0, 1) }
        IGN_X6(0, 0)
#undef IGN_X6
        __builtin_amdgcn_sched_barrier(0);
    };
    auto body = [&](int step, bool odd) {
        if (odd) { IGN_BLOADW(rb10, rb11, rb12, step + 2); IGN_ALOADW(ra1, step + 2); }
        else { IGN_BLOADW(rb00, rb01, rb02, step + 2); IGN_ALOADW(ra0, step + 2); }
        const bool next = step + 1 < ncc;
        auto st = [&]() {
            if (odd) { bstore((step + 1) & 1, rb00, rb01, rb02); if (next) astore((step + 1) & 1, ra0); }
            else { bstore((step + 1) & 1, rb10, rb11, rb12); if (next) astore((step + 1) & 1, ra1); }
            __builtin_amdgcn_sched_barrier(0);
        };
        if (late) { st(); mm(step); } else { mm(step); st(); }
        __syncthreads();
    };
    for (int step = 0; step < ncc; step += 2) {
        body(step, false);
        if (step + 1 < ncc) body(step + 1, true);
    }
#undef IGN_BLOADW
#undef IGN_ALOADW
    float s1[2] = {0.f, 0.f}, s2[2] = {0.f, 0.f};
    const int m_lim = a.M;
    if (m0 + TM <= m_lim) nt_epilogue_body<EPI, true, NP == 2>(a, acc, s1, s2, m0, n0, m_lim, osc);
    else nt_epilogue_body<EPI, false, NP == 2>(a, acc, s1, s2, m0, n0, m_lim, osc);
}

__device__ __forceinline__ void pack_weights_x3t_body(const float* __restrict__ w, unsigned short* __restrict__ wt3,
                                                      unsigned short* __restrict__ wd3, int Co, int Ci, int k, int Cip, int Cop,
                                                      long long i, const float* __restrict__ bound = nullptr) {
    const long long nf = (long long)((Co + TN - 1) / TN) * (Cip / KC) * k * (TN * KC);
    const long long nd = wd3 ? (long long)((Ci + TN - 1) / TN) * (Cop / KC) * k * (TN * KC) : 0;
    const bool fwd = i < nf;
    if (!fwd && i >= nf + nd) return;
    const long long e = fwd ? i : i - nf;
    const int q = (int)(e % KC);
    long long t = e / KC;
    const int row = (int)(t % TN);
    t /= TN;
    const int j = (int)(t % k);
    t /= k;
    const int ncc = (fwd ? Cip : Cop) / KC;
    const int cc = (int)(t % ncc);
    const int nt = (int)(t / ncc);
    const int n = nt * TN + row, c = cc * KC + q;
    float v = 0.f;
    if (fwd) { if (n < Co && c < Ci) v = w[((long long)n * Ci + c) * k + j]; }
    else     { if (n < Ci && c < Co) v = w[((long long)c * Ci + n) * k + (k - 1 - j)]; }
    const long long blk = ((long long)(nt * ncc + cc) * k + j) * X6_BLOCK + (long long)row * KC + q;
    if (bound) {
        const float sv = v * ign_pow2_scale(bound);
        const _Float16 h0 = (_Float16)sv;
        _Float16* dh = reinterpret_cast<_Float16*>(fwd ? wt3 : wd3) + blk;
        dh[0] = h0; dh[TN * KC] = (_Float16)(sv - (float)h0);
        return;
    }
    __bf16 x0, x1, x2;
    split3(v, x0, x1, x2);
    __bf16* dst = reinterpret_cast<__bf16*>(fwd ? wt3 : wd3) + blk;
    dst[0] = x0; dst[TN * KC] = x1; dst[2 * TN * KC] = x2;
}

__global__ void __launch_bounds__(256) pack_weights_x3t_kernel(const float* __restrict__ w, unsigned short* __restrict__ wt3,
                                                               unsigned short* __restrict__ wd3, int Co, int Ci, int k, int Cip,
                                                               int Cop) {
    pack_weights_x3t_body(w, wt3, wd3, Co, Ci, k, Cip, Cop, (long long)blockIdx.x * 256 + threadIdx.x);
}

constexpr int PACK_LMAX = 8;
struct PackMultiTable {
    const float* w[PACK_LMAX];
    unsigned short* wt3[PACK_LMAX];
    unsigned short* wd3[PACK_LMAX];
    long long* counter[PACK_LMAX];
    const float* bound[PACK_LMAX];
    int Co[PACK_LMAX], Ci[PACK_LMAX], k[PACK_LMAX];
};
__global__ void __launch_bounds__(256) pack_weights_x3t_multi_kernel(const PackMultiTable t) {
    const int l = blockIdx.y;
    if (blockIdx.x == 0 && threadIdx.x == 0 && t.counter[l]) *t.counter[l] += 1;
    pack_weights_x3t_body(t.w[l], t.wt3[l], t.wd3[l], t.Co[l], t.Ci[l], t.k[l], (t.Ci[l] + 15) / 16 * 16, (t.Co[l] + 15) / 16 * 16,
                          (long long)blockIdx.x * 256 + threadIdx.x, t.bound[l]);
}

typedef short s16x4 __attribute__((ext_vector_type(4)));
typedef short s16x8 __attribute__((ext_vector_type(8)));
constexpr int WG_PITCH = 64 + 32;

struct WgradX6Args {
    const float* dy; long long dy_sample_pitch; int dy_row0;
    const float* x; long long x_sample_pitch;
    const float* pro_a; const float* pro_b;
    float* part;
    int B, Tin, Tout, Ci, Co, k;
    int cps;
    int nunits, nsplit, citiles;
    const float* bound_dy; const float* bound_x;
};

__device__ __forceinline__ bf16x8 lds_tr8(const __bf16* p0, const __bf16* p1) {
    typedef __attribute__((address_space(3))) s16x4* lds_p;
    const s16x4 lo = __builtin_amdgcn_ds_read_tr16_b64_v4i16((lds_p)(p0));
    const s16x4 hi = __builtin_amdgcn_ds_read_tr16_b64_v4i16((lds_p)(p1));
    const s16x8 v = __builtin_shufflevector(lo, hi, 0, 1, 2, 3, 4, 5, 6, 7);
    return __builtin_bit_cast(bf16x8, v);
}

template <int KT, int NR, int VX, bool PRO, int NP>
__global__ void __launch_bounds__(256, ((NP == 2 && KT <= 5) ? IGN_H3_WAVES : 2)) clconv_wgrad_x6_kernel(const WgradX6Args a) {
    constexpr int RU = 16 * NR;
    constexpr int SPAN = RU + KT - 1;
    constexpr int PPLANE = RU * WG_PITCH, QPLANE = SPAN * WG_PITCH;
    constexpr int NPL = (NP == 2) ? 2 : 3;
    constexpr int STAGE = NPL * (PPLANE + QPLANE);
    constexpr int XVPR = 64 / VX;
    constexpr int XPASS = (SPAN * XVPR + 255) / 256;
    constexpr int DPASS = NR;
    extern __shared__ __attribute__((aligned(16))) unsigned short smem16[];
    __bf16* smem = reinterpret_cast<__bf16*>(smem16);

    const int tile = blockIdx.x;
    const int cot = tile / a.citiles, cit = tile - cot * a.citiles;
    const int co0 = cot * 64, ci0 = cit * 64;
    const int split = blockIdx.y;
    const int per = (a.nunits + a.nsplit - 1) / a.nsplit;
    const int u_begin = split * per, u_end = min(a.nunits, u_begin + per);

    const int tid = threadIdx.x, lane = tid & 63, wave = tid >> 6;
    const int l31 = lane & 31, h = lane >> 5;
    const int wco = wave & 1, wci = wave >> 1;

    const int dr = tid >> 4, dc = (tid & 15) * 4;
    const bool d_ok = co0 + dc < a.Co;
    const int xq = (tid % XVPR) * VX;
    const bool x_ok = ci0 + xq < a.Ci;
    float pa[VX], pb[VX];
    if (PRO && x_ok) { vload<VX>(pa, a.pro_a + ci0 + xq); vload<VX>(pb, a.pro_b + ci0 + xq); }
    const float sdy = (NP == 2) ? ign_pow2_scale(a.bound_dy) : 1.f;
    const float sx = (NP == 2) ? ign_pow2_scale(a.bound_x) : 1.f;
    const float osc = (NP == 2) ? 1.f / (sdy * sx) : 1.f;
    if (NP == 2 && PRO && x_ok) {
#pragma unroll
        for (int v = 0; v < VX; ++v) { pa[v] *= sx; pb[v] *= sx; }
    }

    f32x16 acc[KT];
#pragma unroll
    for (int j = 0; j < KT; ++j)
#pragma unroll
        for (int r = 0; r < 16; ++r) acc[j][r] = 0.f;

    float rd[DPASS][4], rx[XPASS][VX];
    auto gload = [&](int u) {
        const int b = u / a.cps, t0 = (u - b * a.cps) * RU;
        const float* dyb = a.dy + (long long)b * a.dy_sample_pitch + (long long)a.dy_row0 * a.Co + co0 + dc;
        const float* xb = a.x + (long long)b * a.x_sample_pitch + ci0 + xq;
#pragma unroll
        for (int p = 0; p < DPASS; ++p) {
            const int t = t0 + dr + 16 * p;
            if (d_ok && t < a.Tout) vload<4>(rd[p], dyb + (long long)t * a.Co);
            else { rd[p][0] = rd[p][1] = rd[p][2] = rd[p][3] = 0.f; }
        }
#pragma unroll
        for (int p = 0; p < XPASS; ++p) {
            const int row = (tid + p * 256) / XVPR;
            if (x_ok && row < SPAN) vload<VX>(rx[p], xb + (long long)min(t0 + row, a.Tin - 1) * a.Ci);
            else {
#pragma unroll
                for (int v = 0; v < VX; ++v) rx[p][v] = 0.f;
            }
        }
    };
    auto lstore = [&](int buf) {
        __bf16* P = smem + buf * STAGE;
        __bf16* Q = P + NPL * PPLANE;
#pragma unroll
        for (int p = 0; p < DPASS; ++p) {
            if constexpr (NP == 2) {
#pragma unroll
                for (int v = 0; v < 4; ++v) rd[p][v] *= sdy;
            }
            split_store<4, NP>(rd[p], P + (dr + 16 * p) * WG_PITCH + dc, PPLANE);
        }
#pragma unroll
        for (int p = 0; p < XPASS; ++p) {
            const int row = (tid + p * 256) / XVPR;
            if (row < SPAN) {
                float tv[VX];
#pragma unroll
                for (int v = 0; v < VX; ++v) {
                    tv[v] = rx[p][v];
                    if (PRO && x_ok) tv[v] = fmaxf(fmaf(pa[v], tv[v], pb[v]), 0.f);
                    else if (NP == 2) tv[v] *= sx;
                }
                split_store<VX, NP>(tv, Q + row * WG_PITCH + xq, QPLANE);
            }
        }
    };

    const int u16 = lane & 15, q4 = u16 >> 2, p4 = u16 & 3, G1 = (lane >> 4) & 1;
    const int row_lo = 8 * h + q4;
    const int acol = wco * 32 + 16 * G1 + 4 * p4;
    const int bcol = wci * 32 + 16 * G1 + 4 * p4;

    if (u_begin < u_end) {
        gload(u_begin);
        lstore(0);
    }
    __syncthreads();
    int buf = 0;
    for (int u = u_begin; u < u_end; ++u, buf ^= 1) {
        if (u + 1 < u_end) gload(u + 1);
        const __bf16* P = smem + buf * STAGE;
        const __bf16* Q = P + NPL * PPLANE;
#pragma unroll
        for (int s = 0; s < NR; ++s) {
            bf16x8 af[NP];
#pragma unroll
            for (int pl = 0; pl < NP; ++pl) {
                const __bf16* base = P + pl * PPLANE + (16 * s + row_lo) * WG_PITCH + acol;
                af[pl] = lds_tr8(base, base + 4 * WG_PITCH);
            }
            bf16x8 bf[2][NP];
#pragma unroll
            for (int pl = 0; pl < NP; ++pl) {
                const __bf16* base = Q + pl * QPLANE + (16 * s + row_lo) * WG_PITCH + bcol;
                bf[0][pl] = lds_tr8(base, base + 4 * WG_PITCH);
            }
#pragma unroll
            for (int j = 0; j < KT; ++j) {
                if (j + 1 < KT) {
#pragma unroll
                    for (int pl = 0; pl < NP; ++pl) {
                        const __bf16* base = Q + pl * QPLANE + (16 * s + row_lo + j + 1) * WG_PITCH + bcol;
                        bf[(j + 1) & 1][pl] = lds_tr8(base, base + 4 * WG_PITCH);
                    }
                }
                __builtin_amdgcn_sched_barrier(0);
                const bf16x8(&b)[NP] = bf[j & 1];
                if constexpr (NP == 3) {
                    acc[j] = mfma16<NP>(af[2], b[0], acc[j]);
                    acc[j] = mfma16<NP>(af[0], b[2], acc[j]);
                    acc[j] = mfma16<NP>(af[1], b[1], acc[j]);
                }
                if constexpr (NP >= 2) {
                    acc[j] = mfma16<NP>(af[1], b[0], acc[j]);
                    acc[j] = mfma16<NP>(af[0], b[1], acc[j]);
                }
                acc[j] = mfma16<NP>(af[0], b[0], acc[j]);
                __builtin_amdgcn_sched_barrier(0);
            }
        }
        if (u + 1 < u_end) lstore(buf ^ 1);
        __syncthreads();
    }

    float* out = a.part + (long long)split * a.Co * a.k * a.Ci;
    const int ci = ci0 + wci * 32 + l31;
    if (ci < a.Ci) {
#pragma unroll
        for (int j = 0; j < KT; ++j)
#pragma unroll
            for (int r = 0; r < 16; ++r) {
                const int co = co0 + wco * 32 + acc_row16(r, h);
                if (co < a.Co) out[((long long)co * a.k + j) * a.Ci + ci] = (NP == 2) ? acc[j][r] * osc : acc[j][r];
            }
    }
}

constexpr int W1_PITCH = 128 + 32;
constexpr int W1_PLANE = 16 * W1_PITCH;

struct Wgrad1Args {
    const float* dy; const float* x; float* part;
    float* part_b;
    long long M;
    int Ci, Co, nunits, nsplit, citiles, ntiles;
    const float* bound_dy; const float* bound_x;
};

template <int NP>
__global__ void __launch_bounds__(256, (NP == 2 ? IGN_H3_WAVES : 2)) clconv_wgrad_x6_k1_kernel(const Wgrad1Args a) {
    extern __shared__ __attribute__((aligned(16))) unsigned short smem16[];
    __bf16* smem = reinterpret_cast<__bf16*>(smem16);
    constexpr int NPL = (NP == 2) ? 2 : 3;
    constexpr int W1_STAGE = 2 * NPL * W1_PLANE;
    const int xcd = blockIdx.x & 7, seq = blockIdx.x >> 3;
    const int tile = seq % a.ntiles;
    const int split = (seq / a.ntiles) * 8 + xcd;
    if (split >= a.nsplit) return;
    const int cot = tile / a.citiles, cit = tile - cot * a.citiles;
    const int co0 = cot * 128, ci0 = cit * 128;
    const int per = (a.nunits + a.nsplit - 1) / a.nsplit;
    const int u_begin = split * per, u_end = min(a.nunits, u_begin + per);

    const int tid = threadIdx.x, lane = tid & 63, wave = tid >> 6;
    const int l31 = lane & 31, h = lane >> 5;
    const int wco = wave & 1, wci = wave >> 1;

    const int sr = tid >> 5, sc = (tid & 31) * 4;
    const bool d_ok = co0 + sc < a.Co, x_ok = ci0 + sc < a.Ci;
    const float* dyp = a.dy + co0 + sc;
    const float* xp = a.x + ci0 + sc;

    f32x16 acc[2][2];
#pragma unroll
    for (int i = 0; i < 2; ++i)
#pragma unroll
        for (int j = 0; j < 2; ++j)
#pragma unroll
            for (int r = 0; r < 16; ++r) acc[i][j][r] = 0.f;

    float rd[2][4], rx[2][4];
    const float sdy = (NP == 2) ? ign_pow2_scale(a.bound_dy) : 1.f;
    const float sx = (NP == 2) ? ign_pow2_scale(a.bound_x) : 1.f;
    const float osc = (NP == 2) ? 1.f / (sdy * sx) : 1.f;
    const bool want_b = a.part_b != nullptr && cit == 0;
    float bsum[4] = {0.f, 0.f, 0.f, 0.f};
    auto gload = [&](int u) {
#pragma unroll
        for (int p = 0; p < 2; ++p) {
            const long long m = (long long)u * 16 + sr + 8 * p;
            if (d_ok && m < a.M) vload<4>(rd[p], dyp + m * a.Co);
            else { rd[p][0] = rd[p][1] = rd[p][2] = rd[p][3] = 0.f; }
            if (x_ok && m < a.M) vload<4>(rx[p], xp + m * a.Ci);
            else { rx[p][0] = rx[p][1] = rx[p][2] = rx[p][3] = 0.f; }
        }
    };
    auto lstore = [&](int buf) {
        __bf16* P = smem + buf * W1_STAGE;
        __bf16* Q = P + NPL * W1_PLANE;
        if (want_b) {
#pragma unroll
            for (int v = 0; v < 4; ++v) bsum[v] += rd[0][v] + rd[1][v];
        }
#pragma unroll
        for (int p = 0; p < 2; ++p) {
            if constexpr (NP == 2) {
#pragma unroll
                for (int v = 0; v < 4; ++v) { rd[p][v] *= sdy; rx[p][v] *= sx; }
            }
            split_store<4, NP>(rd[p], P + (sr + 8 * p) * W1_PITCH + sc, W1_PLANE);
            split_store<4, NP>(rx[p], Q + (sr + 8 * p) * W1_PITCH + sc, W1_PLANE);
        }
    };

    const int u16 = lane & 15, q4 = u16 >> 2, p4 = u16 & 3, G1 = (lane >> 4) & 1;
    const int roff = (8 * h + q4) * W1_PITCH + 16 * G1 + 4 * p4;

    if (u_begin < u_end) {
        gload(u_begin);
        lstore(0);
    }
    __syncthreads();
    int buf = 0;
    for (int u = u_begin; u < u_end; ++u, buf ^= 1) {
        if (u + 1 < u_end) gload(u + 1);
        const __bf16* P = smem + buf * W1_STAGE + roff + wco * 64;
        const __bf16* Q = smem + buf * W1_STAGE + NPL * W1_PLANE + roff + wci * 64;
        bf16x8 bf[2][NP], af[2][NP];
#pragma unroll
        for (int j = 0; j < 2; ++j)
#pragma unroll
            for (int pl = 0; pl < NP; ++pl) {
                bf[j][pl] = lds_tr8(Q + pl * W1_PLANE + 32 * j, Q + pl * W1_PLANE + 32 * j + 4 * W1_PITCH);
                af[j][pl] = lds_tr8(P + pl * W1_PLANE + 32 * j, P + pl * W1_PLANE + 32 * j + 4 * W1_PITCH);
            }
        __builtin_amdgcn_sched_barrier(0);
#define IGN_W1(pa_, pb_)                                                                                   \
        acc[0][0] = mfma16<NP>(af[0][pa_], bf[0][pb_], acc[0][0]);                                         \
        acc[0][1] = mfma16<NP>(af[0][pa_], bf[1][pb_], acc[0][1]);                                         \
        acc[1][0] = mfma16<NP>(af[1][pa_], bf[0][pb_], acc[1][0]);                                         \
        acc[1][1] = mfma16<NP>(af[1][pa_], bf[1][pb_], acc[1][1]);
        if constexpr (NP == 3) { IGN_W1(2, 0) IGN_W1(0, 2) IGN_W1(1, 1) }
        if constexpr (NP >= 2) { IGN_W1(1, 0) IGN_W1(0, 1) }
        IGN_W1(0, 0)
#undef IGN_W1
        __builtin_amdgcn_sched_barrier(0);
        if (u + 1 < u_end) lstore(buf ^ 1);
        __syncthreads();
    }

    if (want_b) {
        float* red = reinterpret_cast<float*>(smem16);
        *reinterpret_cast<float4*>(red + sr * 128 + sc) = make_float4(bsum[0], bsum[1], bsum[2], bsum[3]);
        __syncthreads();
        if (tid < 128 && co0 + tid < a.Co) {
            float t = 0.f;
#pragma unroll
            for (int r = 0; r < 8; ++r) t += red[r * 128 + tid];
            a.part_b[(long long)split * a.Co + co0 + tid] = t;
        }
    }
    float* out = a.part + (long long)split * a.Co * a.Ci;
#pragma unroll
    for (int j = 0; j < 2; ++j) {
        const int ci = ci0 + wci * 64 + 32 * j + l31;
        if (ci < a.Ci) {
#pragma unroll
            for (int i = 0; i < 2; ++i)
#pragma unroll
                for (int r = 0; r < 16; ++r) {
                    const int co = co0 + wco * 64 + 32 * i + acc_row16(r, h);
                    if (co < a.Co) out[(long long)co * a.Ci + ci] = (NP == 2) ? acc[i][j][r] * osc : acc[i][j][r];
                }
        }
    }
}

template <int EPI, int NP>
static int launch_x6t(const ConvX6Args& a, int V, bool pro, hipStream_t s) {
    const dim3 grid((unsigned)(a.g.mtiles * a.g.ntiles)), block(256);
#define IGN_X6T(VV, PP)                                                                                                      \
    do {                                                                                                                     \
        static bool once = false;                                                                                            \
        if (!once) {                                                                                                         \
            (void)hipFuncSetAttribute(reinterpret_cast<const void*>(&clconv_x6t_kernel<VV, PP, EPI, NP>),                     \
                                      hipFuncAttributeMaxDynamicSharedMemorySize, (int)X6tLds<NP>::BYTES);                   \
            once = true;                                                                                                     \
        }                                                                                                                    \
        hipLaunchKernelGGL((clconv_x6t_kernel<VV, PP, EPI, NP>), grid, block, X6tLds<NP>::BYTES, s, a);                       \
    } while (0)
    if (V == 4) { if (pro) IGN_X6T(4, true); else IGN_X6T(4, false); }
    else if (V == 2) { if (pro) IGN_X6T(2, true); else IGN_X6T(2, false); }
    else { if (pro) IGN_X6T(1, true); else IGN_X6T(1, false); }
#undef IGN_X6T
    return ign_check_launch("clconv_x6t_kernel");
}

template <int NP, int EPI = EPI_BIAS_STATS>
static int launch_x6w(const ConvX6Args& a, hipStream_t s) {
    static bool once = false;
    if (!once) {
        (void)hipFuncSetAttribute(reinterpret_cast<const void*>(&clconv_x6w_kernel<NP, EPI>), hipFuncAttributeMaxDynamicSharedMemorySize,
                                  (int)X6wLds<NP>::BYTES);
        once = true;
    }
    const unsigned nwg = (unsigned)(a.g.mtiles * (a.g.N / 256));
    hipLaunchKernelGGL((clconv_x6w_kernel<NP, EPI>), dim3(nwg), dim3(512), X6wLds<NP>::BYTES, s, a);
    return ign_check_launch("clconv_x6w_kernel");
}

int ign_clconv_launch_x6t(const ConvX6Args& a, int epi, int V, bool pro, hipStream_t s) {
    if (epi == EPI_GELU_BWD) {
        if (!(a.k == 1 && a.g.N % 256 == 0 && V == 4 && !pro && !a.g.part && a.tps * 1 == a.g.mtiles && a.trows == a.g.M && a.nprod == 3
              && a.g.ey)) {
            ign_set_error("ign_clconv_launch_x6t: the GELU-gradient epilogue needs k = 1, N %% 256 == 0, C %% 4 == 0, the f16x3 arithmetic");
            return IGN_E_UNSUP;
        }
        return launch_x6w<2, EPI_GELU_BWD>(a, s);
    }
    if (a.k == 1 && a.g.N % 256 == 0 && V == 4 && !pro && epi == EPI_BIAS_STATS && !a.g.part &&
        a.tps * 1 == a.g.mtiles && a.trows == a.g.M)
        return a.nprod == 1 ? launch_x6w<1>(a, s) : a.nprod == 3 ? launch_x6w<2>(a, s) : launch_x6w<3>(a, s);
    if (a.nprod == 1)
        return epi == EPI_BIAS_STATS ? launch_x6t<EPI_BIAS_STATS, 1>(a, V, pro, s) : launch_x6t<EPI_MASK_STATS, 1>(a, V, pro, s);
    if (a.nprod == 3)
        return epi == EPI_BIAS_STATS ? launch_x6t<EPI_BIAS_STATS, 2>(a, V, pro, s) : launch_x6t<EPI_MASK_STATS, 2>(a, V, pro, s);
    return epi == EPI_BIAS_STATS ? launch_x6t<EPI_BIAS_STATS, 3>(a, V, pro, s) : launch_x6t<EPI_MASK_STATS, 3>(a, V, pro, s);
}

extern "C" int ign_clconv_kpad(int C) { return (C + 15) / 16 * 16; }
extern "C" long long ign_clconv_x3_elems(int rows, int chans, int k) {
    return 3LL * ((rows + TN - 1) / TN) * TN * k * ((chans + 15) / 16 * 16);
}
extern "C" long long ign_clconv_x6_mtiles(int B, int rows) { return (long long)B * ((rows + TM - 1) / TM); }

extern "C" int ign_clconv_pack_weights_x3(const float* w_oik, void* wt3_fwd, void* wt3_dgrad, int Co, int Ci, int k, void* stream) {
    if (!w_oik || !wt3_fwd || Co <= 0 || Ci <= 0 || k <= 0) {
        ign_set_error("ign_clconv_pack_weights_x3: bad argument (Co=%d Ci=%d k=%d)", Co, Ci, k);
        return IGN_E_ARG;
    }
    const int Cip = ign_clconv_kpad(Ci), Cop = ign_clconv_kpad(Co);
    const long long n = ign_clconv_x3_elems(Co, Ci, k) / 3 + (wt3_dgrad ? ign_clconv_x3_elems(Ci, Co, k) / 3 : 0);
    hipLaunchKernelGGL(pack_weights_x3t_kernel, dim3((unsigned)((n + 255) / 256)), dim3(256), 0, (hipStream_t)stream, w_oik,
                       (unsigned short*)wt3_fwd, (unsigned short*)wt3_dgrad, Co, Ci, k, Cip, Cop);
    return ign_check_launch("pack_weights_x3t_kernel");
}

static int pack_multi_impl(int n, const float* const* w_oik, void* const* wt3_fwd, void* const* wt3_dgrad, const int* Co, const int* Ci,
                           const int* k, long long* const* counters, const float* const* bounds, void* stream);

extern "C" int ign_clconv_pack_weights_x3_multi(int n, const float* const* w_oik, void* const* wt3_fwd, void* const* wt3_dgrad,
                                               const int* Co, const int* Ci, const int* k, long long* const* counters, void* stream) {
    return pack_multi_impl(n, w_oik, wt3_fwd, wt3_dgrad, Co, Ci, k, counters, nullptr, stream);
}

extern "C" int ign_clconv_pack_weights_h2_multi(int n, const float* const* w_oik, void* const* wt_fwd, void* const* wt_dgrad,
                                               const int* Co, const int* Ci, const int* k, long long* const* counters,
                                               const float* const* w_bounds, void* stream) {
    if (!w_bounds) { ign_set_error("ign_clconv_pack_weights_h2_multi: null bound table"); return IGN_E_ARG; }
    for (int l = 0; l < n && l < PACK_LMAX; ++l)
        if (!w_bounds[l]) { ign_set_error("ign_clconv_pack_weights_h2_multi: layer %d: null weight bound", l); return IGN_E_ARG; }
    return pack_multi_impl(n, w_oik, wt_fwd, wt_dgrad, Co, Ci, k, counters, w_bounds, stream);
}

static int pack_multi_impl(int n, const float* const* w_oik, void* const* wt3_fwd, void* const* wt3_dgrad, const int* Co, const int* Ci,
                           const int* k, long long* const* counters, const float* const* bounds, void* stream) {
    if (n <= 0 || n > PACK_LMAX || !w_oik || !wt3_fwd || !Co || !Ci || !k) {
        ign_set_error("ign_clconv_pack_weights_x3_multi: n=%d outside 1..%d or null table", n, PACK_LMAX);
        return IGN_E_ARG;
    }
    PackMultiTable t;
    long long nmax = 0;
    for (int l = 0; l < n; ++l) {
        if (!w_oik[l] || !wt3_fwd[l] || Co[l] <= 0 || Ci[l] <= 0 || k[l] <= 0) {
            ign_set_error("ign_clconv_pack_weights_x3_multi: layer %d: bad argument (Co=%d Ci=%d k=%d)", l, Co[l], Ci[l], k[l]);
            return IGN_E_ARG;
        }
        t.w[l] = w_oik[l]; t.wt3[l] = (unsigned short*)wt3_fwd[l]; t.wd3[l] = wt3_dgrad ? (unsigned short*)wt3_dgrad[l] : nullptr;
        t.counter[l] = counters ? counters[l] : nullptr;
        t.bound[l] = bounds ? bounds[l] : nullptr;
        t.Co[l] = Co[l]; t.Ci[l] = Ci[l]; t.k[l] = k[l];
        const long long e = ign_clconv_x3_elems(Co[l], Ci[l], k[l]) / 3 + (t.wd3[l] ? ign_clconv_x3_elems(Ci[l], Co[l], k[l]) / 3 : 0);
        nmax = e > nmax ? e : nmax;
    }
    hipLaunchKernelGGL(pack_weights_x3t_multi_kernel, dim3((unsigned)((nmax + 255) / 256), (unsigned)n), dim3(256), 0,
                       (hipStream_t)stream, t);
    return ign_check_launch("pack_weights_x3t_multi_kernel");
}

template <int KT, int NR, int NP>
static int launch_wgrad_x6(const WgradX6Args& a, int V, bool pro, dim3 grid, hipStream_t s) {
    constexpr size_t lds = (size_t)2 * (NP == 2 ? 2 : 3) * ((16 * NR) + (16 * NR + KT - 1)) * WG_PITCH * sizeof(unsigned short);
#define IGN_WG(VV, PP)                                                                                                       \
    do {                                                                                                                     \
        static bool once = false;                                                                                            \
        if (!once) {                                                                                                         \
            (void)hipFuncSetAttribute(reinterpret_cast<const void*>(&clconv_wgrad_x6_kernel<KT, NR, VV, PP, NP>),             \
                                      hipFuncAttributeMaxDynamicSharedMemorySize, (int)lds);                                 \
            once = true;                                                                                                     \
        }                                                                                                                    \
        hipLaunchKernelGGL((clconv_wgrad_x6_kernel<KT, NR, VV, PP, NP>), grid, dim3(256), lds, s, a);                         \
    } while (0)
    if (V == 4) { if (pro) IGN_WG(4, true); else IGN_WG(4, false); }
    else if (V == 2) { if (pro) IGN_WG(2, true); else IGN_WG(2, false); }
    else { if (pro) IGN_WG(1, true); else IGN_WG(1, false); }
#undef IGN_WG
    return ign_check_launch("clconv_wgrad_x6_kernel");
}

static int wgrad_x6_rows_per_unit(int k) { return (k == 8 || k == 5) ? 16 : (k == 3 || k == 2) ? 32 : 0; }
static int wgrad_x6_splits(int nunits, int tiles) {
    int s = (512 + tiles - 1) / tiles;
    const int max_s = (nunits + 15) / 16;
    if (s > max_s) s = max_s;
    return s < 1 ? 1 : s;
}

static int wgrad_x6_k1_splits(long long M, int Ci, int Co, int* nunits, int* tiles) {
    *nunits = (int)((M + 15) / 16);
    *tiles = ((Co + 127) / 128) * ((Ci + 127) / 128);
    int s = (512 + *tiles - 1) / *tiles;
    const int max_s = (*nunits + 31) / 32;
    if (s > max_s) s = max_s;
    return s < 1 ? 1 : s;
}

extern "C" size_t ign_clconv_wgrad_x6_workspace_bytes(int B, int Tin, int Ci, int Co, int k) {
    if (k == 1 && B > 0 && Tin > 0 && Ci > 0 && Co > 0) {
        int nunits, tiles;
        return (size_t)wgrad_x6_k1_splits((long long)B * Tin, Ci, Co, &nunits, &tiles) * Co * (Ci + 1) * sizeof(float);
    }
    const int Tout = Tin - k + 1, ru = wgrad_x6_rows_per_unit(k);
    if (B <= 0 || Tout <= 0 || Ci <= 0 || Co <= 0 || !ru) return 0;
    const int tiles = ((Co + 63) / 64) * ((Ci + 63) / 64);
    const int nunits = B * ((Tout + ru - 1) / ru);
    return (size_t)wgrad_x6_splits(nunits, tiles) * Co * k * Ci * sizeof(float);
}

template <int NP>
static int wgrad_x6_impl(const char* who, const float* dyp, int dy_pad, const float* x, const float* pro_a, const float* pro_b,
                         float* dw_oik, void* workspace, int B, int Tin, int Ci, int Co, int k, void* stream,
                         float* db = nullptr, const float* bound_dy = nullptr, const float* bound_x = nullptr) {
    const int Tout = Tin - k + 1, ru = wgrad_x6_rows_per_unit(k);
    const bool defer = dw_oik == nullptr && k > 1;
    if (!dyp || !x || (!dw_oik && !defer) || !workspace || B <= 0 || Ci <= 0 || Co <= 0 || k <= 0 || Tout <= 0 || dy_pad < 0 ||
        ((pro_a == nullptr) != (pro_b == nullptr))) {
        ign_set_error("%s: bad argument (B=%d Tin=%d Ci=%d Co=%d k=%d pad=%d)", who, B, Tin, Ci, Co, k, dy_pad);
        return IGN_E_ARG;
    }
    hipStream_t s = (hipStream_t)stream;
    if (k == 1) {
        if (Co % 4 || Ci % 4 || dy_pad || pro_a) {
            ign_set_error("%s: k = 1 needs Co %% 4 == 0, Ci %% 4 == 0, no padding, no prologue (Co=%d Ci=%d)", who, Co, Ci);
            return IGN_E_UNSUP;
        }
        Wgrad1Args w{};
        w.dy = dyp; w.x = x; w.part = (float*)workspace; w.M = (long long)B * Tin; w.Ci = Ci; w.Co = Co;
        int tiles;
        w.nsplit = wgrad_x6_k1_splits(w.M, Ci, Co, &w.nunits, &tiles);
        w.citiles = (Ci + 127) / 128; w.ntiles = tiles;
        w.part_b = db ? (float*)workspace + (size_t)w.nsplit * Co * Ci : nullptr;
        w.bound_dy = bound_dy; w.bound_x = bound_x;
        constexpr size_t w1_lds = (size_t)2 * 2 * (NP == 2 ? 2 : 3) * W1_PLANE * sizeof(unsigned short);
        static bool once = false;
        if (!once) {
            (void)hipFuncSetAttribute(reinterpret_cast<const void*>(&clconv_wgrad_x6_k1_kernel<NP>),
                                      hipFuncAttributeMaxDynamicSharedMemorySize, (int)w1_lds);
            once = true;
        }
        {
            IgnScopedTimer tm("clconv_wgrad", s);
            hipLaunchKernelGGL(clconv_wgrad_x6_k1_kernel<NP>, dim3((unsigned)(tiles * ((w.nsplit + 7) / 8 * 8))), dim3(256), w1_lds,
                               s, w);
        }
        int rc1 = ign_check_launch("clconv_wgrad_x6_k1_kernel");
        if (rc1) return rc1;
        if (db && (rc1 = ign_clconv_launch_wgrad_reduce(w.part_b, db, w.nsplit, Co, 1, 1, s))) return rc1;
        return ign_clconv_launch_wgrad_reduce((const float*)workspace, dw_oik, w.nsplit, Co, Ci, 1, s);
    }
    if (Co % 4 || !ru) { ign_set_error("%s: needs Co %% 4 == 0 and k in {1,2,3,5,8} (Co=%d k=%d)", who, Co, k); return IGN_E_UNSUP; }
    WgradX6Args a{};
    a.dy = dyp; a.dy_sample_pitch = (long long)(Tout + 2 * dy_pad) * Co; a.dy_row0 = dy_pad;
    a.x = x; a.x_sample_pitch = (long long)Tin * Ci; a.pro_a = pro_a; a.pro_b = pro_b;
    a.part = (float*)workspace; a.B = B; a.Tin = Tin; a.Tout = Tout; a.Ci = Ci; a.Co = Co; a.k = k;
    a.cps = (Tout + ru - 1) / ru; a.nunits = B * a.cps;
    a.bound_dy = bound_dy; a.bound_x = bound_x;
    a.citiles = (Ci + 63) / 64;
    const int tiles = ((Co + 63) / 64) * a.citiles;
    a.nsplit = wgrad_x6_splits(a.nunits, tiles);
    const dim3 grid((unsigned)tiles, (unsigned)a.nsplit);
    const int V = ign_vec_width(Ci);
    const bool pro = pro_a != nullptr;
    int rc;
    {
        IgnScopedTimer tm("clconv_wgrad", s);
        if (k == 8) rc = launch_wgrad_x6<8, 1, NP>(a, V, pro, grid, s);
        else if (k == 5) rc = launch_wgrad_x6<5, 1, NP>(a, V, pro, grid, s);
        else if (k == 3) rc = launch_wgrad_x6<3, 2, NP>(a, V, pro, grid, s);
        else rc = launch_wgrad_x6<2, 2, NP>(a, V, pro, grid, s);
    }
    if (rc) return rc;
    if (defer) return 0;
    return ign_clconv_launch_wgrad_reduce((const float*)workspace, dw_oik, a.nsplit, Co, Ci, k, s);
}

extern "C" int ign_clconv_wgrad_x6_nsplit(int B, int Tin, int Ci, int Co, int k) {
    const int Tout = Tin - k + 1, ru = wgrad_x6_rows_per_unit(k);
    if (B <= 0 || Tout <= 0 || Ci <= 0 || Co <= 0 || !ru) return 0;
    return wgrad_x6_splits(B * ((Tout + ru - 1) / ru), ((Co + 63) / 64) * ((Ci + 63) / 64));
}


extern "C" int ign_clconv_wgrad_x6(const float* dyp, int dy_pad, const float* x, const float* pro_a, const float* pro_b,
                                   float* dw_oik, void* workspace, int B, int Tin, int Ci, int Co, int k, void* stream) {
    return wgrad_x6_impl<3>("ign_clconv_wgrad_x6", dyp, dy_pad, x, pro_a, pro_b, dw_oik, workspace, B, Tin, Ci, Co, k, stream);
}

extern "C" int ign_clconv_wgrad_bf16(const float* dyp, int dy_pad, const float* x, const float* pro_a, const float* pro_b,
                                     float* dw_oik, void* workspace, int B, int Tin, int Ci, int Co, int k, void* stream) {
    return wgrad_x6_impl<1>("ign_clconv_wgrad_bf16", dyp, dy_pad, x, pro_a, pro_b, dw_oik, workspace, B, Tin, Ci, Co, k, stream);
}

extern "C" int ign_clconv_wgrad_h3(const float* dyp, int dy_pad, const float* x, const float* pro_a, const float* pro_b,
                                   float* dw_oik, void* workspace, const float* bound_dy, const float* bound_x, int B, int Tin,
                                   int Ci, int Co, int k, void* stream) {
    if (!bound_dy || !bound_x) { ign_set_error("ign_clconv_wgrad_h3: null operand bound"); return IGN_E_ARG; }
    return wgrad_x6_impl<2>("ign_clconv_wgrad_h3", dyp, dy_pad, x, pro_a, pro_b, dw_oik, workspace, B, Tin, Ci, Co, k, stream, nullptr,
                            bound_dy, bound_x);
}
extern "C" int ign_linear_wgrad_h3(const float* dy, const float* x, float* dw, float* db, void* workspace, const float* bound_dy,
                                   const float* bound_x, long long M, int Ci, int Co, void* stream) {
    if (M <= 0 || M > 0x7fffffffLL) { ign_set_error("ign_linear_wgrad_h3: M = %lld rows out of range", M); return IGN_E_ARG; }
    if (!bound_dy || !bound_x) { ign_set_error("ign_linear_wgrad_h3: null operand bound"); return IGN_E_ARG; }
    return wgrad_x6_impl<2>("ign_linear_wgrad_h3", dy, 0, x, nullptr, nullptr, dw, workspace, 1, (int)M, Ci, Co, 1, stream, db, bound_dy,
                            bound_x);
}

extern "C" int ign_linear_wgrad_x6(const float* dy, const float* x, float* dw, float* db, void* workspace, long long M, int Ci,
                                   int Co, void* stream) {
    if (M <= 0 || M > 0x7fffffffLL) { ign_set_error("ign_linear_wgrad_x6: M = %lld rows out of range", M); return IGN_E_ARG; }
    return wgrad_x6_impl<3>("ign_linear_wgrad_x6", dy, 0, x, nullptr, nullptr, dw, workspace, 1, (int)M, Ci, Co, 1, stream, db);
}
extern "C" int ign_linear_wgrad_bf16(const float* dy, const float* x, float* dw, float* db, void* workspace, long long M, int Ci,
                                     int Co, void* stream) {
    if (M <= 0 || M > 0x7fffffffLL) { ign_set_error("ign_linear_wgrad_bf16: M = %lld rows out of range", M); return IGN_E_ARG; }
    return wgrad_x6_impl<1>("ign_linear_wgrad_bf16", dy, 0, x, nullptr, nullptr, dw, workspace, 1, (int)M, Ci, Co, 1, stream, db);
}
```

### speech-imagery-eeg_amd/ign_hip/_lib.py

```python
import ctypes
import os
import threading

_CSRC = os.path.join(os.path.dirname(os.path.dirname(os.path.abspath(__file__))), "csrc")
_LOCK = threading.Lock()
_LIB = None

c_f = ctypes.POINTER(ctypes.c_float)
c_i32 = ctypes.POINTER(ctypes.c_int32)
vp, ci, cf, sz, ll, cd = ctypes.c_void_p, ctypes.c_int, ctypes.c_float, ctypes.c_size_t, ctypes.c_longlong, ctypes.c_double

SIGNATURES = {
    "ign_abi_version": (ci, []),
    "ign_last_error": (ctypes.c_char_p, []),
    "ign_instnorm_fwd": (ci, [vp, vp, vp, ci, ci, ci, cf, vp]),
    "ign_transpose_btc_to_bct": (ci, [vp, vp, ci, ci, ci, vp]),
    "ign_instnorm_fwd_amax": (ci, [vp, vp, vp, ci, ci, ci, cf, vp, vp]),
    "ign_standardise_nct_to_btc": (ci, [vp, vp, vp, ci, ci, ci, cf, vp]),
    "ign_shapelet_fwd": (ci, [vp, vp, vp, vp, vp, ci, ci, vp, vp, vp, vp, ci, ci, ci, ci, ci, ci, cf, ci, vp]),
    "ign_shapelet_fwd_bank": (ci, [vp, ci, vp, vp, vp, vp, ci, vp, vp, vp, vp, vp, ci, ci, ci, vp, vp, vp, cf, ci, vp]),
    "ign_shapelet_bwd_workspace_bytes": (sz, [ci, ci, ci, ci, ci, ci, ci]),
    "ign_layernorm_parts": (ll, [ll, ci]),
    "ign_layernorm_fwd": (ci, [vp, vp, vp, vp, vp, vp, ll, ci, cf, vp]),
    "ign_bn1_data_stats_workspace_bytes": (sz, [ci, ci, ci]),
    "ign_bn1_data_stats": (ci, [vp, ci, ci, ci, ci, vp, vp, vp, vp]),
    "ign_autocorr_sum_fwd": (ci, [vp, vp, vp, ci, ci, ci, ctypes.POINTER(ctypes.c_int), vp]),
    "ign_bn1_fold_fwd": (ci, [vp, vp, vp, vp, vp, vp, cd, cf, cf, vp, vp, vp, vp, vp, ci, ci, ci, vp]),
    "ign_bn1_fold_bwd": (ci, [vp, vp, vp, vp, vp, vp, vp, cd, vp, vp, vp, vp, ci, ci, ci, vp]),
    "ign_layernorm_res_fwd": (ci, [vp, vp, vp, vp, vp, vp, vp, vp, ll, ci, cf, vp]),
    "ign_layernorm_bwd": (ci, [vp, vp, vp, vp, vp, vp, vp, vp, vp, ll, ci, vp]),
    "ign_layernorm_bwd_amax": (ci, [vp, vp, vp, vp, vp, vp, vp, vp, vp, vp, ll, ci, vp]),
    "ign_autocorr_parts": (ll, [ci]),
    "ign_autocorr_fwd": (ci, [vp, vp, ci, ci, ci, vp]),
    "ign_edge_lagprod_parts": (ll, [ci]),
    "ign_edge_lagprod_fwd": (ci, [vp, vp, ci, ci, ci, ci, vp]),
    "ign_attn_fwd": (ci, [vp, vp, vp, vp, vp, ci, ci, ci, ci, ci, ll, ll, ll, ll, ll, ll, cf, vp]),
    "ign_attn_fwd_x6": (ci, [vp, vp, vp, vp, vp, ci, ci, ci, ci, ci, ll, ll, ll, ll, ll, ll, cf, vp]),
    "ign_attn_bwd": (ci, [vp, vp, vp, vp, vp, vp, vp, vp, vp, vp, ci, ci, ci, ci, ci, ll, ll, ll, ll, ll, ll, cf, vp]),
    "ign_attn_bwd_x6": (ci, [vp, vp, vp, vp, vp, vp, vp, vp, vp, vp, ci, ci, ci, ci, ci, ll, ll, ll, ll, ll, ll, cf, vp]),
    "ign_attn_bwd_x6_strided": (ci, [vp, vp, vp, vp, vp, vp, vp, vp, vp, vp, ci, ci, ci, ci, ci, ll, ll, ll, ll, ll, ll, cf, vp, ll, ll,
                                     ci]),
    "ign_attn_fwd_bf16": (ci, [vp, vp, vp, vp, vp, ci, ci, ci, ci, ci, ll, ll, ll, ll, ll, ll, cf, vp]),
    "ign_attn_bwd_bf16": (ci, [vp, vp, vp, vp, vp, vp, vp, vp, vp, vp, ci, ci, ci, ci, ci, ll, ll, ll, ll, ll, ll, cf, vp]),
    "ign_attn_fwd_h3": (ci, [vp, vp, vp, vp, vp, ci, ci, ci, ci, ci, ll, ll, ll, ll, ll, ll, cf, vp, vp, vp, vp]),
    "ign_attn_bwd_h3": (ci, [vp, vp, vp, vp, vp, vp, vp, vp, vp, vp, ci, ci, ci, ci, ci, ll, ll, ll, ll, ll, ll, cf, vp, ll, ll,
                             vp, vp, vp, vp, vp]),
    "ign_attn_fwd_dropout": (ci, [vp, vp, vp, vp, vp, ci, ci, ci, ci, ci, ll, ll, ll, ll, ll, ll, cf, vp, ci, vp, vp, vp, cf,
                                  ctypes.c_ulonglong]),
    "ign_attn_bwd_dropout": (ci, [vp, vp, vp, vp, vp, vp, vp, vp, vp, vp, ci, ci, ci, ci, ci, ll, ll, ll, ll, ll, ll, cf, vp, ci, ll,
                                  ll, vp, vp, vp, vp, vp, cf, ctypes.c_ulonglong]),
    "ign_attn_dropout_mask": (ci, [vp, ci, ci, ci, ci, cf, ctypes.c_ulonglong, vp]),
    "ign_head_fwd": (ci, [vp, vp, vp, vp, ci, ci, ci, ll, vp]),
    "ign_head_bwd": (ci, [vp, vp, vp, vp, vp, vp, ci, ci, ci, ll, vp]),
    "ign_gate_fwd": (ci, [vp, vp, vp, vp, ci, ci, cf, ci, vp]),
    "ign_gate_bwd": (ci, [vp, vp, vp, vp, vp, vp, ci, ci, cf, ci, vp]),
    "ign_loss_fwd_bwd": (ci, [vp, vp, vp, vp, vp, vp, vp, vp, ci, ci, cf, vp]),
    "ign_diversity_fwd_bwd": (ci, [vp, vp, vp, ci, ci, ci, cf, vp]),
    "ign_adam_step": (ci, [vp, vp, vp, vp, ll, cf, cf, cf, cf, ci, vp]),
    "ign_gather_flat": (ci, [vp, vp, vp, ci, vp, vp]),
    "ign_adam_step_dev": (ci, [vp, vp, vp, vp, ll, cf, cf, cf, cf, vp, vp, vp]),
    "ign_conv1_sumsq_workspace_bytes": (sz, [ci, ci, ci]),
    "ign_conv1_sumsq_fwd": (ci, [vp, vp, vp, vp, vp, ci, ci, ci, ci, ci, vp]),
    "ign_conv1_sumsq_bwd": (ci, [vp, vp, vp, vp, vp, ci, ci, ci, ci, ci, vp]),
    "ign_dwconv1d_fwd": (ci, [vp, vp, vp, ci, ci, ci, ci, ci, ci, vp]),
    "ign_dwconv1d_bwd_weight_workspace_bytes": (sz, [ci, ci, ci]),
    "ign_dwconv1d_bwd_weight": (ci, [vp, vp, vp, vp, ci, ci, ci, ci, ci, vp]),
    "ign_chan_contract_fwd": (ci, [vp, vp, vp, ci, ci, ci, ci, vp]),
    "ign_chan_contract_bwd_weight_workspace_bytes": (sz, [ci, ci, ci, ci]),
    "ign_chan_contract_bwd_weight": (ci, [vp, vp, vp, vp, ci, ci, ci, ci, vp]),
    "ign_chan_stats_workspace_bytes": (sz, [ci, ci]),
    "ign_chan_stats": (ci, [vp, vp, vp, ci, ci, ci, vp]),
    "ign_affine_elu_pool_fwd": (ci, [vp, vp, vp, vp, ci, ci, ci, ci, vp]),
    "ign_bn_elu_pool_bwd_sums": (ci, [vp, vp, vp, vp, vp, vp, vp, ci, ci, ci, ci, vp]),
    "ign_bn_elu_pool_bwd_apply": (ci, [vp, vp, vp, vp, vp, vp, vp, vp, ci, ci, ci, ci, vp]),
    "ign_bn_fold_fwd": (ci, [vp, vp, vp, vp, vp, vp, vp, vp, vp, vp, ci, ll, cf, cf, vp]),
    "ign_bn_fold_bwd": (ci, [vp, vp, vp, vp, vp, vp, vp, vp, vp, vp, ci, ll, cf, vp]),
    "ign_clconv_mtiles": (ll, [ll]),
    "ign_clconv_pack_weights": (ci, [vp, vp, vp, ci, ci, ci, vp]),
    "ign_clconv_fwd": (ci, [vp, vp, vp, vp, vp, vp, vp, ci, ci, ci, ci, ci, vp]),
    "ign_clconv_dgrad": (ci, [vp, vp, vp, vp, vp, vp, vp, vp, vp, ci, ci, ci, ci, ci, vp]),
    "ign_clconv_kpad": (ci, [ci]),
    "ign_clconv_x6_mtiles": (ll, [ci, ci]),
    "ign_clconv_x3_elems": (ll, [ci, ci, ci]),
    "ign_clconv_pack_weights_x3": (ci, [vp, vp, vp, ci, ci, ci, vp]),
    "ign_clconv_fwd_x6": (ci, [vp, vp, vp, vp, vp, vp, vp, ci, ci, ci, ci, ci, vp]),
    "ign_clconv_dgrad_x6": (ci, [vp, vp, vp, vp, vp, vp, vp, vp, vp, ci, ci, ci, ci, ci, vp]),
    "ign_clconv_wgrad_x6_workspace_bytes": (sz, [ci, ci, ci, ci, ci]),
    "ign_clconv_wgrad_x6": (ci, [vp, ci, vp, vp, vp, vp, vp, ci, ci, ci, ci, ci, vp]),
    "ign_clconv_fwd_bf16": (ci, [vp, vp, vp, vp, vp, vp, vp, ci, ci, ci, ci, ci, vp]),
    "ign_clconv_dgrad_bf16": (ci, [vp, vp, vp, vp, vp, vp, vp, vp, vp, ci, ci, ci, ci, ci, vp]),
    "ign_clconv_wgrad_bf16": (ci, [vp, ci, vp, vp, vp, vp, vp, ci, ci, ci, ci, ci, vp]),
    "ign_linear_wgrad_x6": (ci, [vp, vp, vp, vp, vp, ll, ci, ci, vp]),
    "ign_linear_wgrad_bf16": (ci, [vp, vp, vp, vp, vp, ll, ci, ci, vp]),
    "ign_clconv_wgrad_workspace_bytes": (sz, [ci, ci, ci, ci, ci]),
    "ign_clconv_wgrad": (ci, [vp, ci, vp, vp, vp, vp, vp, ci, ci, ci, ci, ci, vp]),
    "ign_bn_finalize_fwd": (ci, [vp, ci, ll, ci, vp, vp, cf, cf, vp, vp, vp, vp, vp, vp, vp]),
    "ign_bn_affine_eval": (ci, [vp, vp, vp, vp, cf, ci, vp, vp, vp, vp, vp]),
    "ign_bn_relu_pool_fwd": (ci, [vp, vp, vp, vp, ci, ci, ci, vp]),
    "ign_bn_relu_pool_head_fwd": (ci, [vp, vp, vp, vp, vp, vp, vp, ci, ci, ci, ci, vp]),
    "ign_bn_relu_pool_bwd_parts": (ll, [ci, ci]),
    "ign_bn_relu_pool_bwd": (ci, [vp, vp, vp, vp, vp, vp, vp, vp, ci, ci, ci, vp]),
    "ign_bn_finalize_bwd": (ci, [vp, ci, ci, vp, vp, vp]),
    "ign_bn_bwd_apply": (ci, [vp, vp, vp, vp, vp, vp, vp, vp, ci, ci, ci, ci, ci, vp]),
    "ign_timing_enable": (ci, [ci]),
    "ign_timing_read": (ci, [ctypes.c_char_p, ctypes.POINTER(ctypes.c_double), ctypes.POINTER(ctypes.c_longlong)]),
    "ign_clconv_wgrad_x6_nsplit": (ci, [ci, ci, ci, ci, ci]),
    "ign_clconv_wgrad_reduce_multi": (ci, [ci, vp, vp, vp, vp, vp, vp, vp]),
    "ign_clconv_pack_weights_x3_multi": (ci, [ci, vp, vp, vp, vp, vp, vp, vp, vp]),
    "ign_absmax": (ci, [vp, ll, vp, vp]),
    "ign_absmax_multi": (ci, [ci, vp, vp, vp, vp]),
    "ign_fcn_scan": (ci, [ci, vp, vp, vp, vp, vp, vp, vp, vp, ll, vp]),
    "ign_clconv_pack_weights_h2_multi": (ci, [ci, vp, vp, vp, vp, vp, vp, vp, vp, vp]),
    "ign_clconv_fwd_h3": (ci, [vp, vp, vp, vp, vp, vp, vp, vp, vp, ci, ci, ci, ci, ci, vp]),
    "ign_clconv_fwd_h3_amax": (ci, [vp, vp, vp, vp, vp, vp, vp, vp, vp, vp, ci, ci, ci, ci, ci, vp]),
    "ign_linear_dgrad_gelu_h3": (ci, [vp, vp, vp, vp, vp, vp, vp, ll, ci, ci, vp]),
    "ign_clconv_dgrad_h3": (ci, [vp, vp, vp, vp, vp, vp, vp, vp, vp, vp, vp, ci, ci, ci, ci, ci, vp]),
    "ign_clconv_wgrad_h3": (ci, [vp, ci, vp, vp, vp, vp, vp, vp, vp, ci, ci, ci, ci, ci, vp]),
    "ign_linear_wgrad_h3": (ci, [vp, vp, vp, vp, vp, vp, vp, ll, ci, ci, vp]),
    "ign_bn_bwd_apply_amax": (ci, [vp, vp, vp, vp, vp, vp, vp, vp, vp, ci, ci, ci, ci, ci, vp]),
    "ign_head_bwd_acc": (ci, [vp, vp, vp, vp, vp, vp, vp, vp, ci, ci, ci, ll, vp]),
    "ign_loss_fwd_bwd_reg": (ci, [vp, vp, vp, vp, vp, vp, vp, vp, vp, ci, ci, cf, vp]),
    "ign_sbm_reg_workspace_bytes": (sz, [ci, ci, ll]),
    "ign_sbm_reg_fwd_bwd": (ci, [vp, vp, ll, cf, ci, vp, vp, vp, vp, ci, cf, cf, vp, vp, vp]),
    "ign_shapelet_bwd_bank_workspace_bytes": (sz, [ci, ci, ci, ci, vp, vp, vp, ci]),
    "ign_shapelet_bwd_bank": (ci, [vp, ci, vp, vp, vp, vp, ci, vp, vp, vp, vp, vp, vp, vp, vp, vp, vp, ci, ci, ci, vp, vp, vp, cf, ci,
                                   vp]),
    "ign_shapelet_bwd": (ci, [vp, vp, vp, vp, vp, ci, ci, vp, vp, vp, vp, vp, vp, vp, ci, ci, ci, ci, ci, ci, cf, ci, vp]),
}


class IgnError(RuntimeError):
    pass


_RAW_STREAM = None

PARAM_GENERATION = [0]


def stream():
    global _RAW_STREAM
    import torch
    if _RAW_STREAM is None:
        _RAW_STREAM = getattr(torch._C, "_cuda_getCurrentRawStream", False)
    if _RAW_STREAM:
        return ctypes.c_void_p(_RAW_STREAM(torch.cuda.current_device()))
    return ctypes.c_void_p(torch.cuda.current_stream().cuda_stream)


def lib_path():
    return os.path.join(_CSRC, "libign_hip.so")


def lib():
    global _LIB
    if _LIB is not None:
        return _LIB
    with _LOCK:
        if _LIB is None:
            path = lib_path()
            if not os.path.exists(path):
                raise IgnError(f"{path} not found: the HIP extension is not built "
                               f"(run `make -C {_CSRC} -j8` or __graft_entry__.build()); there is no CPU fallback")
            h = ctypes.CDLL(path)
            for name, (res, args) in SIGNATURES.items():
                fn = getattr(h, name)
                fn.restype, fn.argtypes = res, args
            if h.ign_abi_version() != 1:
                raise IgnError(f"{path}: ABI version {h.ign_abi_version()} != 1")
            _LIB = h
    return _LIB


def require():
    return lib()


def check(rc, what):
    if rc != 0:
        msg = lib().ign_last_error().decode("utf-8", "replace")
        raise IgnError(f"{what} failed (rc={rc}): {msg}")


def timing_enable(on=True):
    lib().ign_timing_enable(1 if on else 0)


def timing_read(label):
    ms, n = ctypes.c_double(0.0), ctypes.c_longlong(0)
    check(lib().ign_timing_read(label.encode(), ctypes.byref(ms), ctypes.byref(n)), "ign_timing_read")
    return ms.value, n.value
```

### speech-imagery-eeg_amd/ign_hip/fcn.py

```python
import ctypes
import os

import torch

from . import _lib


CONV_MATH = os.environ.get("IGN_CONV_MATH", "f16x3")
DEBUG = None


def _ptr(t):
    return ctypes.c_void_p(t.data_ptr()) if t is not None else None


_stream = _lib.stream


def _attached_bound(t):
    cb = getattr(t, "_ign_bound", None)
    if cb is None or cb[1] != t._version or cb[2] != t.data_ptr():
        return None
    if torch.cuda.is_current_stream_capturing() and not (len(cb) > 3 and cb[3]):
        return None
    return cb[0]


class BnState:

    def __init__(self, bn):
        self.eps = float(bn.eps)
        self.use_batch_stats = bn.training or not bn.track_running_stats
        self.running_mean = self.running_var = None
        self.momentum = 0.0
        self.bump = None
        if bn.track_running_stats:
            self.running_mean, self.running_var = bn.running_mean, bn.running_var
            if bn.training:
                if bn.momentum is None:
                    if bn.num_batches_tracked is not None:
                        bn.num_batches_tracked.add_(1)
                    self.momentum = 1.0 / float(bn.num_batches_tracked)
                else:
                    self.bump = bn.num_batches_tracked
                    self.momentum = float(bn.momentum)
        self.update_running = bn.training and bn.track_running_stats


class FcnBodyFn(torch.autograd.Function):

    @staticmethod
    def forward(ctx, x, states_math, *params):
        L = _lib.lib()
        states, math, has_head = states_math
        head_w, head_b = (params[-2], params[-1]) if has_head else (None, None)
        if has_head:
            params = params[:-2]
        if not x.is_cuda or x.dtype != torch.float32:
            raise _lib.IgnError(f"fcn_body: needs a float32 GPU tensor, got {x.dtype} on {x.device} (no CPU fallback)")
        x = x.contiguous()
        B = x.shape[0]
        nl = len(params) // 4
        dev = x.device
        f32 = dict(device=dev, dtype=torch.float32)
        need_grad = any(ctx.needs_input_grad[2:2 + len(params)])
        if math == "f16x3" and not (all(st.use_batch_stats for st in states) and nl <= 8):
            math = "bf16x6"
        h3 = math == "f16x3"
        x6 = math in ("bf16x6", "bf16", "f16x3")
        conv_fwd = L.ign_clconv_fwd_bf16 if math == "bf16" else L.ign_clconv_fwd_x6
        slots = zbuf = xbound = None
        fp = lambda t, off: ctypes.c_void_p(t.data_ptr() + 4 * off)
        inputs, affine, wds, shapes = [x], [], [], []
        pa = pb = None
        packed = None
        if x6 and nl <= 8:
            ws_ = [params[4 * l].contiguous() for l in range(nl)]
            wts = [torch.empty(int(L.ign_clconv_x3_elems(w.shape[0], w.shape[1], w.shape[2])), device=dev, dtype=torch.bfloat16)
                   for w in ws_]
            wds_ = [torch.empty(int(L.ign_clconv_x3_elems(w.shape[1], w.shape[0], w.shape[2])), device=dev, dtype=torch.bfloat16)
                    if (l > 0 and need_grad) else None for l, w in enumerate(ws_)]
            vpa, ia, lla = ctypes.c_void_p * nl, ctypes.c_int * nl, ctypes.c_longlong * nl
            pv = lambda ts: vpa(*[(t.data_ptr() if t is not None else None) for t in ts])
            bumps = [st.bump for st in states]
            bump_tab = pv(bumps) if any(b is not None for b in bumps) else None
            dims = (ia(*[w.shape[0] for w in ws_]), ia(*[w.shape[1] for w in ws_]), ia(*[w.shape[2] for w in ws_]))
            if h3:
                slots = torch.empty(4 * nl, **f32)
                gam = [None] + [params[4 * (l - 1) + 2].contiguous() for l in range(1, nl)]
                bet = [None] + [params[4 * (l - 1) + 3].contiguous() for l in range(1, nl)]
                Touts, T_ = [], x.shape[1]
                for w in ws_:
                    T_ = T_ - w.shape[2] + 1
                    Touts.append(T_)
                zbuf = torch.empty(sum(w.shape[0] for w in ws_), **f32) if need_grad else None
                _lib.check(L.ign_fcn_scan(nl, pv(ws_), lla(*[w.numel() for w in ws_]), pv(gam), pv(bet),
                                          ia(*([0] + [ws_[l - 1].shape[0] for l in range(1, nl)])),
                                          lla(*([0] + [B * Touts[l - 1] for l in range(1, nl)])), _ptr(slots), _ptr(zbuf),
                                          zbuf.numel() if zbuf is not None else 0, _stream()), "ign_fcn_scan")
                xbound = _attached_bound(x)
                if xbound is None:
                    _lib.check(L.ign_absmax(_ptr(x), x.numel(), fp(slots, 1), _stream()), "ign_absmax")
                    xbound = slots[1:2]
                _lib.check(L.ign_clconv_pack_weights_h2_multi(nl, pv(ws_), pv(wts), pv(wds_), *dims, bump_tab,
                                                              vpa(*[slots.data_ptr() + 16 * l for l in range(nl)]), _stream()),
                           "ign_clconv_pack_weights_h2_multi")
            else:
                _lib.check(L.ign_clconv_pack_weights_x3_multi(nl, pv(ws_), pv(wts), pv(wds_), *dims, bump_tab, _stream()),
                           "ign_clconv_pack_weights_x3_multi")
            packed = (wts, wds_)
        else:
            bumps = [st.bump for st in states if st.bump is not None]
            if bumps:
                torch._foreach_add_(bumps, 1)
        for l in range(nl):
            w, b, gamma, beta = (p.contiguous() for p in params[4 * l:4 * l + 4])
            Co, Ci, k = w.shape
            h = inputs[-1]
            Tin = h.shape[1]
            Tout = Tin - k + 1
            if h.shape[2] != Ci or Tout <= 0 or Co % 4:
                raise _lib.IgnError(f"fcn_body block {l + 1}: input {tuple(h.shape)} vs weight {tuple(w.shape)}")
            st = states[l]
            y = torch.empty(B, Tout, Co, **f32)
            nparts = int(L.ign_clconv_x6_mtiles(B, Tout) if x6 else L.ign_clconv_mtiles(B * Tout))
            part = torch.empty(nparts, 2, Co, **f32) if st.use_batch_stats else None
            want_wd = l > 0 and need_grad
            if x6:
                if packed is not None:
                    wt, wd = packed[0][l], packed[1][l]
                else:
                    wt = torch.empty(int(L.ign_clconv_x3_elems(Co, Ci, k)), device=dev, dtype=torch.bfloat16)
                    wd = torch.empty(int(L.ign_clconv_x3_elems(Ci, Co, k)), device=dev, dtype=torch.bfloat16) if want_wd else None
                    _lib.check(L.ign_clconv_pack_weights_x3(_ptr(w), _ptr(wt), _ptr(wd), Co, Ci, k, _stream()),
                               "ign_clconv_pack_weights_x3")
                if h3:
                    _lib.check(L.ign_clconv_fwd_h3(_ptr(h), _ptr(wt), _ptr(b), _ptr(pa), _ptr(pb), _ptr(y), _ptr(part),
                                                   fp(slots, 4 * l + 1) if l else _ptr(xbound), fp(slots, 4 * l), B, Tin, Ci, Co, k,
                                                   _stream()), "ign_clconv_fwd_h3")
                else:
                    _lib.check(conv_fwd(_ptr(h), _ptr(wt), _ptr(b), _ptr(pa), _ptr(pb), _ptr(y), _ptr(part), B, Tin, Ci, Co, k,
                                        _stream()), "ign_clconv_fwd_x6")
            else:
                wt = torch.empty(Co, k * Ci, **f32)
                wd = torch.empty(Ci, k * Co, **f32) if want_wd else None
                _lib.check(L.ign_clconv_pack_weights(_ptr(w), _ptr(wt), _ptr(wd), Co, Ci, k, _stream()), "ign_clconv_pack_weights")
                _lib.check(L.ign_clconv_fwd(_ptr(h), _ptr(wt), _ptr(b), _ptr(pa), _ptr(pb), _ptr(y), _ptr(part), B, Tin, Ci, Co, k,
                                            _stream()), "ign_clconv_fwd")
            a, bb, mean, invstd = (torch.empty(Co, **f32) for _ in range(4))
            if st.use_batch_stats:
                _lib.check(L.ign_bn_finalize_fwd(_ptr(part), nparts, B * Tout, Co, _ptr(gamma), _ptr(beta), st.eps, st.momentum,
                                                 _ptr(st.running_mean if st.update_running else None),
                                                 _ptr(st.running_var if st.update_running else None), _ptr(a), _ptr(bb), _ptr(mean),
                                                 _ptr(invstd), _stream()), "ign_bn_finalize_fwd")
            else:
                _lib.check(L.ign_bn_affine_eval(_ptr(st.running_mean), _ptr(st.running_var), _ptr(gamma), _ptr(beta), st.eps, Co,
                                                _ptr(a), _ptr(bb), _ptr(mean), _ptr(invstd), _stream()), "ign_bn_affine_eval")
            inputs.append(y)
            affine.append((a, bb, mean, invstd))
            wds.append(wd)
            shapes.append((Co, Ci, k, Tin, Tout))
            pa, pb = a, bb
        y_last = inputs[-1]
        Cl, Tl = y_last.shape[2], y_last.shape[1]
        pooled = torch.empty(B, Cl, **f32)
        head = None
        if has_head:
            head_w = head_w.contiguous()
            N = head_w.shape[0]
            if head_w.shape[1] != Cl or head_w.dtype != torch.float32:
                raise _lib.IgnError(f"fcn_body: head weight {tuple(head_w.shape)} {head_w.dtype} does not fit {Cl} pooled channels")
            out = torch.empty(B, N, **f32)
            _lib.check(L.ign_bn_relu_pool_head_fwd(_ptr(y_last), _ptr(pa), _ptr(pb), _ptr(pooled), _ptr(head_w), _ptr(head_b), _ptr(out),
                                                   B, Tl, Cl, N, _stream()), "ign_bn_relu_pool_head_fwd")
            head = (pooled, head_w, head_b is not None)
        else:
            out = pooled
            _lib.check(L.ign_bn_relu_pool_fwd(_ptr(y_last), _ptr(pa), _ptr(pb), _ptr(pooled), B, Tl, Cl, _stream()),
                       "ign_bn_relu_pool_fwd")
        ctx.head = head
        ctx.head_needs = tuple(ctx.needs_input_grad[-2:]) if has_head else None
        ctx.saved = (inputs, affine, wds, shapes, [st.use_batch_stats for st in states], math, slots, zbuf, xbound) \
            if (need_grad or (has_head and any(ctx.head_needs))) else None
        ctx.body_grad = need_grad
        return out

    @staticmethod
    def backward(ctx, gpool):
        if ctx.saved is None:
            raise _lib.IgnError("fcn_body backward called but the forward ran without parameter gradients enabled")
        if ctx.needs_input_grad[0]:
            raise _lib.IgnError("fcn_body: gradient w.r.t. the input series is not implemented (inputs are data)")
        L = _lib.lib()
        inputs, affine, wds, shapes, batch_stats, math, slots, zbuf, xbound = ctx.saved
        h3 = math == "f16x3"
        x6 = math in ("bf16x6", "bf16", "f16x3")
        fp = lambda t, off: ctypes.c_void_p(t.data_ptr() + 4 * off)
        nl = len(shapes)
        B = inputs[0].shape[0]
        dev = gpool.device
        f32 = dict(device=dev, dtype=torch.float32)
        gpool = gpool.contiguous()
        head_grads = ()
        if ctx.head is not None:
            pooled, head_w, has_b = ctx.head
            N, Cl = head_w.shape
            glog = gpool
            gpool = torch.empty(B, Cl, **f32)
            ghw = torch.empty_like(head_w)
            ghb = torch.empty(N, **f32) if has_b else None
            _lib.check(L.ign_head_bwd(_ptr(glog), _ptr(pooled), _ptr(head_w), _ptr(gpool), _ptr(ghw), _ptr(ghb), B, Cl, N, Cl, _stream()),
                       "ign_head_bwd")
            head_grads = (ghw if ctx.head_needs[0] else None, ghb if ctx.head_needs[1] else None)
            if not ctx.body_grad:
                ctx.saved = None
                return (None, None, *([None] * (4 * nl)), *head_grads)
        grads = [None] * (4 * nl)
        zoff, ztot = [], 0
        for (Co_, _, _, _, _), bs_ in zip(shapes, batch_stats):
            zoff.append(ztot)
            ztot += Co_ if bs_ else 0
        if zbuf is None or zbuf.numel() != ztot:
            zbuf = torch.zeros(ztot, **f32) if ztot else None

        Co, Ci, k, Tin, Tout = shapes[-1]
        a, bb, mean, invstd = affine[-1]
        y = inputs[-1]
        g = torch.empty_like(y)
        nparts = int(L.ign_bn_relu_pool_bwd_parts(B, Tout))
        part = torch.empty(nparts, 2, Co, **f32)
        _lib.check(L.ign_bn_relu_pool_bwd(_ptr(y), _ptr(gpool), _ptr(a), _ptr(bb), _ptr(mean), _ptr(invstd), _ptr(g), _ptr(part),
                                          B, Tout, Co, _stream()), "ign_bn_relu_pool_bwd")
        defer = x6 and all(sh[2] in (2, 3, 5, 8) for sh in shapes) and nl <= 8
        deferred = []
        for l in range(nl - 1, -1, -1):
            Co, Ci, k, Tin, Tout = shapes[l]
            a, bb, mean, invstd = affine[l]
            y = inputs[l + 1]
            dbeta, dgamma = torch.empty(Co, **f32), torch.empty(Co, **f32)
            _lib.check(L.ign_bn_finalize_bwd(_ptr(part), nparts, Co, _ptr(dbeta), _ptr(dgamma), _stream()), "ign_bn_finalize_bwd")
            pad = (k - 1) if l > 0 else 0
            dyp = torch.empty(B, Tout + 2 * pad, Co, **f32)
            training = 1 if batch_stats[l] else 0
            _lib.check(L.ign_bn_bwd_apply_amax(_ptr(g), _ptr(y), _ptr(a), _ptr(mean), _ptr(invstd), _ptr(dbeta), _ptr(dgamma), _ptr(dyp),
                                               fp(slots, 4 * l + 2) if h3 else None, B, Tout, Co, pad, training, _stream()),
                       "ign_bn_bwd_apply")
            if DEBUG is not None:
                DEBUG[f"g{l}"], DEBUG[f"dyp{l}"], DEBUG[f"dbeta{l}"], DEBUG[f"dgamma{l}"] = g.clone(), dyp.clone(), dbeta.clone(), dgamma.clone()
            del g
            pa, pb = (affine[l - 1][0], affine[l - 1][1]) if l > 0 else (None, None)
            wx6 = x6 and k in (2, 3, 5, 8)
            ws_bytes = (L.ign_clconv_wgrad_x6_workspace_bytes if wx6 else L.ign_clconv_wgrad_workspace_bytes)(B, Tin, Ci, Co, k)
            ws = torch.empty(int(ws_bytes) // 4, **f32)
            dw = torch.empty(Co, Ci, k, **f32)
            wgrad = (L.ign_clconv_wgrad_bf16 if math == "bf16" else L.ign_clconv_wgrad_x6) if wx6 else L.ign_clconv_wgrad
            if h3 and wx6:
                _lib.check(L.ign_clconv_wgrad_h3(_ptr(dyp), pad, _ptr(inputs[l]), _ptr(pa), _ptr(pb), None if defer else _ptr(dw), _ptr(ws),
                                                 fp(slots, 4 * l + 2), fp(slots, 4 * l + 1) if l else _ptr(xbound), B, Tin, Ci, Co, k, _stream()),
                           "ign_clconv_wgrad_h3")
            else:
                _lib.check(wgrad(_ptr(dyp), pad, _ptr(inputs[l]), _ptr(pa), _ptr(pb), None if defer else _ptr(dw), _ptr(ws), B, Tin,
                                 Ci, Co, k, _stream()), "ign_clconv_wgrad")
            if defer:
                deferred.append((ws, dw, int(L.ign_clconv_wgrad_x6_nsplit(B, Tin, Ci, Co, k)), Co, Ci, k))
            del ws
            grads[4 * l + 0] = dw
            grads[4 * l + 1] = zbuf[zoff[l]:zoff[l] + Co] if training else dyp.sum(dim=(0, 1))
            grads[4 * l + 2] = dgamma
            grads[4 * l + 3] = dbeta
            if l > 0:
                pa_, pb_, pm_, pi_ = affine[l - 1]
                g = torch.empty(B, Tin, Ci, **f32)
                nparts = int(L.ign_clconv_x6_mtiles(B, Tin) if x6 else L.ign_clconv_mtiles(B * Tin))
                part = torch.empty(nparts, 2, Ci, **f32)
                dgrad = (L.ign_clconv_dgrad_bf16 if math == "bf16" else L.ign_clconv_dgrad_x6) if x6 else L.ign_clconv_dgrad
                if h3:
                    _lib.check(L.ign_clconv_dgrad_h3(_ptr(dyp), _ptr(wds[l]), _ptr(inputs[l]), _ptr(pa_), _ptr(pb_), _ptr(pm_), _ptr(pi_),
                                                     _ptr(g), _ptr(part), fp(slots, 4 * l + 2), fp(slots, 4 * l), B, Tin, Ci, Co, k,
                                                     _stream()), "ign_clconv_dgrad_h3")
                else:
                    _lib.check(dgrad(_ptr(dyp), _ptr(wds[l]), _ptr(inputs[l]), _ptr(pa_), _ptr(pb_), _ptr(pm_), _ptr(pi_),
                                     _ptr(g), _ptr(part), B, Tin, Ci, Co, k, _stream()), "ign_clconv_dgrad")
            del dyp
        if deferred:
            n = len(deferred)
            vpa, ia = ctypes.c_void_p * n, ctypes.c_int * n
            _lib.check(L.ign_clconv_wgrad_reduce_multi(n, vpa(*[d[0].data_ptr() for d in deferred]), vpa(*[d[1].data_ptr() for d in deferred]),
                                                       ia(*[d[2] for d in deferred]), ia(*[d[3] for d in deferred]),
                                                       ia(*[d[4] for d in deferred]), ia(*[d[5] for d in deferred]), _stream()),
                       "ign_clconv_wgrad_reduce_multi")
        ctx.saved = None
        return (None, None, *grads, *head_grads)


def fcn_body(x, blocks, math=None, head=None):
    if math is None:
        math = "bf16" if torch.is_autocast_enabled() else CONV_MATH
    states = [BnState(bn) for _, bn in blocks]
    params = []
    for conv, bn in blocks:
        if conv.bias is None or bn.weight is None or bn.bias is None:
            raise _lib.IgnError("fcn_body: Conv1d needs a bias and BatchNorm1d needs affine parameters")
        if conv.stride != (1,) or conv.padding != (0,) or conv.dilation != (1,) or conv.groups != 1:
            raise _lib.IgnError("fcn_body: only stride-1, unpadded, undilated, ungrouped Conv1d is implemented")
        params += [conv.weight, conv.bias, bn.weight, bn.bias]
    if head is not None:
        if head.weight.shape[0] > 16:
            raise _lib.IgnError("fcn_body: the fused head covers up to 16 outputs")
        return FcnBodyFn.apply(x, (states, math, True), *params, head.weight, head.bias)
    return FcnBodyFn.apply(x, (states, math, False), *params)
```

Measured before the change: 2.880.

## Fold BatchNorm backward into conv dgrad/wgrad prologues, skip materialized gradients

```diff
diff --git a/include/ign_abi.h b/include/ign_abi.h
--- a/include/ign_abi.h
+++ b/include/ign_abi.h
@@ -291,6 +291,23 @@
                      const float* dbeta, const float* dgamma, float* dyp, int B, int T, int C, int pad, int training,
                      void* stream);
 
+int ign_bn_relu_pool_bwd_ext(const float* y, const float* gpool, const float* a, const float* b, const float* mean,
+                             const float* invstd, float* part, float* ext, int B, int T, int C, void* stream);
+int ign_bn_finalize_bwd_pool(const float* part, const float* ext, const float* gpool, int B, int T, int C, const float* a,
+                             const float* mean, const float* invstd, float* dbeta, float* dgamma, float* c1, float* c0,
+                             float* dy_bound, void* stream);
+int ign_bn_finalize_bwd_fold(const float* part, int nparts, long long R, int C, const float* a, const float* mean,
+                             const float* invstd, float* dbeta, float* dgamma, float* c1, float* c0, void* stream);
+int ign_clconv_dgrad_fold(int nprod, const float* g, const float* gpool, const float* y, const float* fa, const float* fb,
+                          const float* c1, const float* c0, const void* wt_dgrad, const float* y_in, const float* a_in,
+                          const float* b_in, const float* mean_in, const float* invstd_in, float* g_in, float* stat_part,
+                          const float* bound_dy, const float* bound_w, float* amax_g, int B, int Tin, int Ci, int Co, int k,
+                          void* stream);
+int ign_clconv_wgrad_fold(int nprod, const float* g, const float* gpool, const float* y, const float* fa, const float* fb,
+                          const float* c1, const float* c0, const float* x, const float* pro_a, const float* pro_b,
+                          float* dw_oik, void* workspace, const float* bound_dy, const float* bound_x, int B, int Tin,
+                          int Ci, int Co, int k, void* stream);
+
 int ign_timing_enable(int on);
 int ign_timing_read(const char* label, double* total_ms, long long* launches);
 
diff --git a/speech-imagery-eeg_amd/csrc/ign_bn.hip b/speech-imagery-eeg_amd/csrc/ign_bn.hip
--- a/speech-imagery-eeg_amd/csrc/ign_bn.hip
+++ b/speech-imagery-eeg_amd/csrc/ign_bn.hip
@@ -90,6 +90,65 @@
     dgamma[c] = (float)q;
 }
 
+__device__ __forceinline__ void bn_fold_coefs(int c, float s, float q, const float* __restrict__ a, const float* __restrict__ mean,
+                                              const float* __restrict__ invstd, float invR, float* __restrict__ c1,
+                                              float* __restrict__ c0) {
+    const float ca = a[c];
+    float mv = mean[c], iv = invstd[c];
+    c1[c] = -ca * iv * q * invR;
+    c0[c] = -ca * (s - mv * iv * q) * invR;
+}
+
+__global__ void __launch_bounds__(1024) bn_finalize_bwd_fold_kernel(const float* __restrict__ part, int nparts, int C,
+                                                                    const float* __restrict__ a, const float* __restrict__ mean,
+                                                                    const float* __restrict__ invstd, float invR,
+                                                                    float* __restrict__ dbeta, float* __restrict__ dgamma,
+                                                                    float* __restrict__ c1, float* __restrict__ c0) {
+    double s, q;
+    bn_sum_partials(part, nparts, C, &s, &q);
+    const int c = blockIdx.x * BN_CH + threadIdx.x % BN_CH;
+    if (threadIdx.x / BN_CH != 0 || c >= C) return;
+    dbeta[c] = (float)s;
+    dgamma[c] = (float)q;
+    bn_fold_coefs(c, (float)s, (float)q, a, mean, invstd, invR, c1, c0);
+}
+
+__global__ void __launch_bounds__(1024) bn_finalize_bwd_pool_kernel(const float* __restrict__ part, int nparts, int C,
+                                                                    const float* __restrict__ ext, const float* __restrict__ gpool,
+                                                                    int blocks_per_sample, float invT, const float* __restrict__ a,
+                                                                    const float* __restrict__ mean, const float* __restrict__ invstd,
+                                                                    float invR, float* __restrict__ dbeta, float* __restrict__ dgamma,
+                                                                    float* __restrict__ c1, float* __restrict__ c0,
+                                                                    float* __restrict__ dy_bound) {
+    __shared__ float shk[2][BN_CH];
+    double s, q;
+    bn_sum_partials(part, nparts, C, &s, &q);
+    const int cl = threadIdx.x % BN_CH, sl = threadIdx.x / BN_CH;
+    const int c = blockIdx.x * BN_CH + cl;
+    if (sl == 0 && c < C) {
+        dbeta[c] = (float)s;
+        dgamma[c] = (float)q;
+        bn_fold_coefs(c, (float)s, (float)q, a, mean, invstd, invR, c1, c0);
+        shk[0][cl] = c1[c];
+        shk[1][cl] = c0[c];
+    }
+    if (!dy_bound) return;
+    __syncthreads();
+    if (c >= C) return;
+    const float ca = a[c], k1 = shk[0][cl], k0 = shk[1][cl];
+    float m = 0.f;
+    const int per = (nparts + BN_SL - 1) / BN_SL;
+    const int i1 = min(nparts, (sl + 1) * per);
+    for (int i = sl * per; i < i1; ++i) {
+        const float gv = gpool[(size_t)(i / blocks_per_sample) * C + c] * invT;
+        const float* e = ext + (size_t)i * 4 * C + c;
+        const float lo1 = e[0], hi1 = e[C], lo0 = e[2 * C], hi0 = e[3 * C];
+        if (lo1 <= hi1) m = fmaxf(m, fmaxf(fabsf(fmaf(ca, gv, fmaf(k1, lo1, k0))), fabsf(fmaf(ca, gv, fmaf(k1, hi1, k0)))));
+        if (lo0 <= hi0) m = fmaxf(m, fmaxf(fabsf(fmaf(ca, 0.f, fmaf(k1, lo0, k0))), fabsf(fmaf(ca, 0.f, fmaf(k1, hi0, k0)))));
+    }
+    atomic_absmax(dy_bound, m);
+}
+
 __global__ void __launch_bounds__(256) bn_relu_pool_fwd_kernel(const float* __restrict__ y, const float* __restrict__ a,
                                                                const float* __restrict__ b, float* __restrict__ pooled, int T,
                                                                int C, const float* __restrict__ W,
@@ -132,16 +191,21 @@
 }
 
 constexpr int POOL_ROWS = 128;
+template <bool EXT>
 __global__ void __launch_bounds__(256) bn_relu_pool_bwd_kernel(const float* __restrict__ y, const float* __restrict__ gpool,
                                                                const float* __restrict__ a, const float* __restrict__ b,
                                                                const float* __restrict__ mean, const float* __restrict__ invstd,
-                                                               float* __restrict__ g, float* __restrict__ part, int T, int C) {
+                                                               float* __restrict__ g, float* __restrict__ part, int T, int C,
+                                                               float* __restrict__ ext) {
     extern __shared__ float sm[];
     const int c4 = C / 4, rif = 256 / c4;
     const int col = (threadIdx.x % c4) * 4, rofs = threadIdx.x / c4;
     const int bi = blockIdx.y;
     const int t0 = blockIdx.x * POOL_ROWS, t1 = min(T, t0 + POOL_ROWS);
     float s0[4] = {0.f, 0.f, 0.f, 0.f}, s1[4] = {0.f, 0.f, 0.f, 0.f};
+    float lo1[4], hi1[4], lo0[4], hi0[4];
+#pragma unroll
+    for (int q = 0; q < 4; ++q) { lo1[q] = lo0[q] = INFINITY; hi1[q] = hi0[q] = -INFINITY; }
     if (rofs < rif) {
         float av[4], bv[4], mv[4], iv[4], gp[4];
         vload<4>(av, a + col); vload<4>(bv, b + col); vload<4>(mv, mean + col); vload<4>(iv, invstd + col);
@@ -153,14 +217,25 @@
             vload<4>(yy, y + off);
 #pragma unroll
             for (int q = 0; q < 4; ++q) {
-                gg[q] = (fmaf(av[q], yy[q], bv[q]) > 0.f) ? gp[q] * invT : 0.f;
+                const bool on = fmaf(av[q], yy[q], bv[q]) > 0.f;
+                gg[q] = on ? gp[q] * invT : 0.f;
                 s0[q] += gg[q];
                 s1[q] = fmaf(gg[q], (yy[q] - mv[q]) * iv[q], s1[q]);
+                if (EXT) {
+                    if (on) { lo1[q] = fminf(lo1[q], yy[q]); hi1[q] = fmaxf(hi1[q], yy[q]); }
+                    else { lo0[q] = fminf(lo0[q], yy[q]); hi0[q] = fmaxf(hi0[q], yy[q]); }
+                }
             }
-            vstore<4>(g + off, gg);
-        }
-#pragma unroll
-        for (int q = 0; q < 4; ++q) { sm[rofs * C + col + q] = s0[q]; sm[(rif + rofs) * C + col + q] = s1[q]; }
+            if (!EXT) vstore<4>(g + off, gg);
+        }
+#pragma unroll
+        for (int q = 0; q < 4; ++q) {
+            sm[rofs * C + col + q] = s0[q]; sm[(rif + rofs) * C + col + q] = s1[q];
+            if (EXT) {
+                sm[(2 * rif + rofs) * C + col + q] = lo1[q]; sm[(3 * rif + rofs) * C + col + q] = hi1[q];
+                sm[(4 * rif + rofs) * C + col + q] = lo0[q]; sm[(5 * rif + rofs) * C + col + q] = hi0[q];
+            }
+        }
     }
     __syncthreads();
     const size_t pi = (size_t)bi * gridDim.x + blockIdx.x;
@@ -169,6 +244,15 @@
         for (int q = 0; q < rif; ++q) { u += sm[q * C + c]; v += sm[(rif + q) * C + c]; }
         part[(pi * 2 + 0) * C + c] = u;
         part[(pi * 2 + 1) * C + c] = v;
+        if (EXT) {
+            float e[4] = {INFINITY, -INFINITY, INFINITY, -INFINITY};
+            for (int q = 0; q < rif; ++q) {
+                e[0] = fminf(e[0], sm[(2 * rif + q) * C + c]); e[1] = fmaxf(e[1], sm[(3 * rif + q) * C + c]);
+                e[2] = fminf(e[2], sm[(4 * rif + q) * C + c]); e[3] = fmaxf(e[3], sm[(5 * rif + q) * C + c]);
+            }
+#pragma unroll
+            for (int k = 0; k < 4; ++k) ext[(pi * 4 + k) * C + c] = e[k];
+        }
     }
 }
 
@@ -402,9 +486,48 @@
     if (!y || !gpool || !a || !b || !mean || !invstd || !g || !part) { ign_set_error("ign_bn_relu_pool_bwd: null pointer"); return IGN_E_ARG; }
     const int rif = 256 / (C / 4);
     IgnScopedTimer tm("bn_relu_pool_bwd", (hipStream_t)stream);
-    hipLaunchKernelGGL(bn_relu_pool_bwd_kernel, dim3((T + POOL_ROWS - 1) / POOL_ROWS, B), dim3(256), (size_t)2 * rif * C * 4,
-                       (hipStream_t)stream, y, gpool, a, b, mean, invstd, g, part, T, C);
+    hipLaunchKernelGGL(bn_relu_pool_bwd_kernel<false>, dim3((T + POOL_ROWS - 1) / POOL_ROWS, B), dim3(256), (size_t)2 * rif * C * 4,
+                       (hipStream_t)stream, y, gpool, a, b, mean, invstd, g, part, T, C, (float*)nullptr);
     return ign_check_launch("bn_relu_pool_bwd_kernel");
+}
+
+extern "C" int ign_bn_relu_pool_bwd_ext(const float* y, const float* gpool, const float* a, const float* b, const float* mean,
+                                        const float* invstd, float* part, float* ext, int B, int T, int C, void* stream) {
+    int rc;
+    if ((rc = bn_check("ign_bn_relu_pool_bwd_ext", (long long)B * T, C))) return rc;
+    if (!y || !gpool || !a || !b || !mean || !invstd || !part || !ext) { ign_set_error("ign_bn_relu_pool_bwd_ext: null pointer"); return IGN_E_ARG; }
+    const int rif = 256 / (C / 4);
+    IgnScopedTimer tm("bn_relu_pool_bwd", (hipStream_t)stream);
+    hipLaunchKernelGGL(bn_relu_pool_bwd_kernel<true>, dim3((T + POOL_ROWS - 1) / POOL_ROWS, B), dim3(256), (size_t)6 * rif * C * 4,
+                       (hipStream_t)stream, y, gpool, a, b, mean, invstd, (float*)nullptr, part, T, C, ext);
+    return ign_check_launch("bn_relu_pool_bwd_kernel");
+}
+
+extern "C" int ign_bn_finalize_bwd_fold(const float* part, int nparts, long long R, int C, const float* a, const float* mean,
+                                        const float* invstd, float* dbeta, float* dgamma, float* c1, float* c0, void* stream) {
+    if (!part || nparts <= 0 || R <= 0 || C <= 0 || !a || !mean || !invstd || !dbeta || !dgamma || !c1 || !c0) {
+        ign_set_error("ign_bn_finalize_bwd_fold: bad argument");
+        return IGN_E_ARG;
+    }
+    hipLaunchKernelGGL(bn_finalize_bwd_fold_kernel, dim3((C + BN_CH - 1) / BN_CH), dim3(BN_CH * BN_SL), 0, (hipStream_t)stream, part,
+                       nparts, C, a, mean, invstd, 1.0f / (float)R, dbeta, dgamma, c1, c0);
+    return ign_check_launch("bn_finalize_bwd_fold_kernel");
+}
+
+extern "C" int ign_bn_finalize_bwd_pool(const float* part, const float* ext, const float* gpool, int B, int T, int C, const float* a,
+                                        const float* mean, const float* invstd, float* dbeta, float* dgamma, float* c1, float* c0,
+                                        float* dy_bound, void* stream) {
+    int rc;
+    if ((rc = bn_check("ign_bn_finalize_bwd_pool", (long long)B * T, C))) return rc;
+    if (!part || !ext || !gpool || !a || !mean || !invstd || !dbeta || !dgamma || !c1 || !c0) {
+        ign_set_error("ign_bn_finalize_bwd_pool: bad argument");
+        return IGN_E_ARG;
+    }
+    const int bps = (T + POOL_ROWS - 1) / POOL_ROWS;
+    hipLaunchKernelGGL(bn_finalize_bwd_pool_kernel, dim3((C + BN_CH - 1) / BN_CH), dim3(BN_CH * BN_SL), 0, (hipStream_t)stream, part,
+                       B * bps, C, ext, gpool, bps, 1.0f / (float)T, a, mean, invstd, 1.0f / (float)((long long)B * T), dbeta, dgamma,
+                       c1, c0, dy_bound);
+    return ign_check_launch("bn_finalize_bwd_pool_kernel");
 }
 
 extern "C" int ign_bn_bwd_apply(const float* g, const float* y, const float* a, const float* mean, const float* invstd,
diff --git a/speech-imagery-eeg_amd/csrc/ign_clconv.h b/speech-imagery-eeg_amd/csrc/ign_clconv.h
--- a/speech-imagery-eeg_amd/csrc/ign_clconv.h
+++ b/speech-imagery-eeg_amd/csrc/ign_clconv.h
@@ -143,6 +143,14 @@
 }
 
 
+enum { FOLD_NONE = 0, FOLD_G = 2, FOLD_POOL = 3 };
+struct BnBwdFold {
+    const float* g; const float* gp; const float* y;
+    const float* fa; const float* fb; const float* c1; const float* c0;
+    int T, pad;
+    float invT;
+};
+
 struct ConvX6Args {
     GemmNTArgs g;
     long long sample_pitch;
@@ -153,6 +161,7 @@
     int nprod;
     const float* bound_a;
     const float* bound_b;
+    BnBwdFold fold;
 };
 
 __device__ __forceinline__ float ign_pow2_scale(const float* bound) {
@@ -169,4 +178,5 @@
 inline int ign_vec_width(int c) { return (c % 4 == 0) ? 4 : (c % 2 == 0) ? 2 : 1; }
 
 int ign_clconv_launch_x6t(const ConvX6Args& a, int epi, int V, bool pro, hipStream_t s);
+int ign_clconv_launch_x6t_fold(const ConvX6Args& a, int mode, hipStream_t s);
 int ign_clconv_launch_wgrad_reduce(const float* part, float* dw_oik, int nsplit, int Co, int Ci, int k, hipStream_t s);
diff --git a/speech-imagery-eeg_amd/csrc/ign_clconv_f32.hip b/speech-imagery-eeg_amd/csrc/ign_clconv_f32.hip
--- a/speech-imagery-eeg_amd/csrc/ign_clconv_f32.hip
+++ b/speech-imagery-eeg_amd/csrc/ign_clconv_f32.hip
@@ -474,6 +474,37 @@
     if (!bound_dy || !bound_w) { ign_set_error("ign_clconv_dgrad_h3: null operand bound"); return IGN_E_ARG; }
     return clconv_dgrad_impl("ign_clconv_dgrad_h3", 3, dyp, wt_h2_dgrad, y_in, a_in, b_in, mean_in, invstd_in, g_in, stat_part, B,
                              Tin, Ci, Co, k, stream, bound_dy, bound_w);
+}
+
+extern "C" int ign_clconv_dgrad_fold(int nprod, const float* g, const float* gpool, const float* y, const float* fa, const float* fb,
+                                     const float* c1, const float* c0, const void* wt_dgrad, const float* y_in, const float* a_in,
+                                     const float* b_in, const float* mean_in, const float* invstd_in, float* g_in, float* stat_part,
+                                     const float* bound_dy, const float* bound_w, float* amax_g, int B, int Tin, int Ci, int Co, int k,
+                                     void* stream) {
+    const char* who = "ign_clconv_dgrad_fold";
+    const int Tout = Tin - k + 1;
+    if (!y || !fa || !c1 || !c0 || (!g && (!gpool || !fb)) || !wt_dgrad || !y_in || !a_in || !b_in || !mean_in || !invstd_in || !g_in ||
+        B <= 0 || Ci <= 0 || Co <= 0 || k <= 0 || Tout <= 0 || (nprod != 1 && nprod != 3 && nprod != 6) ||
+        (nprod == 3 && (!bound_dy || !bound_w))) {
+        ign_set_error("%s: bad argument (nprod=%d B=%d Tin=%d Ci=%d Co=%d k=%d)", who, nprod, B, Tin, Ci, Co, k);
+        return IGN_E_ARG;
+    }
+    if (k > 16 || Co % 4) { ign_set_error("%s: needs k <= 16 and Co %% 4 == 0 (k=%d Co=%d)", who, k, Co); return IGN_E_UNSUP; }
+    const long long M = (long long)B * Tin;
+    if (M > 0x7fffffffLL / 2) { ign_set_error("%s: B*Tin = %lld rows exceed the 2^30 row index space", who, M); return IGN_E_TOOBIG; }
+    ConvX6Args c{};
+    GemmNTArgs& a = c.g;
+    a.A = y; a.am = RowMap{Tin, 0, Co, (long long)(Tout + 2 * (k - 1)) * Co}; a.K = k * Co;
+    a.C = g_in; a.M = (int)M; a.N = Ci; a.B3 = (const unsigned short*)wt_dgrad;
+    a.part = stat_part; a.ey = y_in; a.ea = a_in; a.eb = b_in; a.emean = mean_in; a.einv = invstd_in;
+    a.amax_out = nprod == 3 ? amax_g : nullptr;
+    a.ntiles = (Ci + TN - 1) / TN;
+    c.cin = Co; c.cp = (Co + 15) / 16 * 16; c.k = k; a.Kp = k * c.cp;
+    c.sample_pitch = (long long)(Tout + 2 * (k - 1)) * Co; c.rows_in = Tout + 2 * (k - 1); c.trows = Tin; c.tps = (Tin + TM - 1) / TM;
+    a.mtiles = B * c.tps; c.nprod = nprod; c.bound_a = bound_dy; c.bound_b = bound_w;
+    c.fold = BnBwdFold{g, gpool, y, fa, fb, c1, c0, Tout, k - 1, 1.0f / (float)Tout};
+    IgnScopedTimer tm("clconv_dgrad", (hipStream_t)stream);
+    return ign_clconv_launch_x6t_fold(c, g ? FOLD_G : FOLD_POOL, (hipStream_t)stream);
 }
 
 static int wgrad_splits(long long M, int tiles) {
diff --git a/speech-imagery-eeg_amd/csrc/ign_clconv_x6.hip b/speech-imagery-eeg_amd/csrc/ign_clconv_x6.hip
--- a/speech-imagery-eeg_amd/csrc/ign_clconv_x6.hip
+++ b/speech-imagery-eeg_amd/csrc/ign_clconv_x6.hip
@@ -114,7 +114,7 @@
     static constexpr size_t BYTES = (size_t)2 * (ABUF + BBUF) * sizeof(unsigned short);
 };
 template <int NP, int EPI> struct X6tWaves { static constexpr int N = (NP == 2 && EPI == EPI_BIAS_STATS) ? IGN_H3_WAVES : 2; };
-template <int V, bool PRO, int EPI, int NP>
+template <int V, int PRO, int EPI, int NP>
 __global__ void __launch_bounds__(256, (X6tWaves<NP, EPI>::N)) clconv_x6t_kernel(const ConvX6Args ca) {
     const GemmNTArgs& a = ca.g;
     constexpr int VPR = KC / V;
@@ -152,8 +152,12 @@
 #pragma unroll
             for (int r = 0; r < 16; ++r) acc[i][j][r] = 0.f;
 
+    constexpr bool FOLD = PRO >= FOLD_G;
     float ra[APASS][V];
+    float rg[FOLD_G == PRO ? APASS : 1][V];
+    bool rv[FOLD ? APASS : 1];
     float pa[V], pb[V];
+    float f1[FOLD ? V : 1], f0[FOLD ? V : 1], fg[PRO == FOLD_POOL ? V : 1];
     bool a_ok = false;
     uint4 rb00, rb01 = {}, rb02 = {}, rb10, rb11 = {}, rb12 = {};
     const int ncc = ca.cp / KC;
@@ -164,12 +168,35 @@
     auto aload = [&](int cc) {
         const int ch = cc * KC + (tid % VPR) * V;
         a_ok = ch < ca.cin;
-        if (PRO && a_ok) {
+        if (PRO == 1 && a_ok) {
             vload<V>(pa, a.pro_a + ch); vload<V>(pb, a.pro_b + ch);
             if constexpr (NP == 2) {
 #pragma unroll
                 for (int v = 0; v < V; ++v) { pa[v] *= sa; pb[v] *= sa; }
             }
+        }
+        if constexpr (FOLD) {
+            const BnBwdFold& f = ca.fold;
+            if (a_ok) {
+                vload<V>(pa, f.fa + ch); vload<V>(f1, f.c1 + ch); vload<V>(f0, f.c0 + ch);
+                if constexpr (PRO == FOLD_POOL) {
+                    vload<V>(pb, f.fb + ch); vload<V>(fg, f.gp + (long long)bi * ca.cin + ch);
+#pragma unroll
+                    for (int v = 0; v < V; ++v) fg[v] *= f.invT;
+                }
+            }
+            const long long sbase = (long long)bi * f.T * ca.cin + ch;
+#pragma unroll
+            for (int p = 0; p < APASS; ++p) {
+                const int idx = tid + p * 256;
+                const int t = t0 + idx / VPR - f.pad;
+                rv[p] = a_ok && idx < nvec && t >= 0 && t < f.T;
+                if (rv[p]) {
+                    vload<V>(ra[p], f.y + sbase + (long long)t * ca.cin);
+                    if constexpr (PRO == FOLD_G) vload<V>(rg[p], f.g + sbase + (long long)t * ca.cin);
+                }
+            }
+            return;
         }
 #pragma unroll
         for (int p = 0; p < APASS; ++p) {
@@ -193,7 +220,14 @@
 #pragma unroll
                 for (int v = 0; v < V; ++v) {
                     tv[v] = ra[p][v];
-                    if (PRO && a_ok) tv[v] = fmaxf(fmaf(pa[v], tv[v], pb[v]), 0.f);
+                    if constexpr (PRO == FOLD_G) {
+                        tv[v] = rv[p] ? fmaf(pa[v], rg[p][v], fmaf(f1[v], tv[v], f0[v])) : 0.f;
+                        if constexpr (NP == 2) tv[v] *= sa;
+                    } else if constexpr (PRO == FOLD_POOL) {
+                        const float gv = (fmaf(pa[v], tv[v], pb[v]) > 0.f) ? fg[v] : 0.f;
+                        tv[v] = rv[p] ? fmaf(pa[v], gv, fmaf(f1[v], tv[v], f0[v])) : 0.f;
+                        if constexpr (NP == 2) tv[v] *= sa;
+                    } else if (PRO == 1 && a_ok) tv[v] = fmaxf(fmaf(pa[v], tv[v], pb[v]), 0.f);
                     else if (NP == 2) tv[v] *= sa;
                 }
                 split_store<V, NP>(tv, st + row * X6_PITCH + q * V, X6T_APLANE);
@@ -477,6 +511,7 @@
     int cps;
     int nunits, nsplit, citiles;
     const float* bound_dy; const float* bound_x;
+    BnBwdFold fold;
 };
 
 __device__ __forceinline__ bf16x8 lds_tr8(const __bf16* p0, const __bf16* p1) {
@@ -487,7 +522,7 @@
     return __builtin_bit_cast(bf16x8, v);
 }
 
-template <int KT, int NR, int VX, bool PRO, int NP>
+template <int KT, int NR, int VX, bool PRO, int NP, int DYF = FOLD_NONE>
 __global__ void __launch_bounds__(256, ((NP == 2 && KT <= 5) ? IGN_H3_WAVES : 2)) clconv_wgrad_x6_kernel(const WgradX6Args a) {
     constexpr int RU = 16 * NR;
     constexpr int SPAN = RU + KT - 1;
@@ -531,16 +566,44 @@
 #pragma unroll
         for (int r = 0; r < 16; ++r) acc[j][r] = 0.f;
 
+    constexpr bool FOLD = DYF != FOLD_NONE;
+    float fa[FOLD ? 4 : 1], fb[DYF == FOLD_POOL ? 4 : 1], f1[FOLD ? 4 : 1], f0[FOLD ? 4 : 1];
+    float rg[DYF == FOLD_G ? DPASS : 1][4], fg[DYF == FOLD_POOL ? 4 : 1];
+    bool dv[FOLD ? DPASS : 1];
+    if constexpr (FOLD) {
+        if (d_ok) {
+            vload<4>(fa, a.fold.fa + co0 + dc); vload<4>(f1, a.fold.c1 + co0 + dc); vload<4>(f0, a.fold.c0 + co0 + dc);
+            if constexpr (DYF == FOLD_POOL) vload<4>(fb, a.fold.fb + co0 + dc);
+        }
+    }
+
     float rd[DPASS][4], rx[XPASS][VX];
     auto gload = [&](int u) {
         const int b = u / a.cps, t0 = (u - b * a.cps) * RU;
         const float* dyb = a.dy + (long long)b * a.dy_sample_pitch + (long long)a.dy_row0 * a.Co + co0 + dc;
         const float* xb = a.x + (long long)b * a.x_sample_pitch + ci0 + xq;
-#pragma unroll
-        for (int p = 0; p < DPASS; ++p) {
-            const int t = t0 + dr + 16 * p;
-            if (d_ok && t < a.Tout) vload<4>(rd[p], dyb + (long long)t * a.Co);
-            else { rd[p][0] = rd[p][1] = rd[p][2] = rd[p][3] = 0.f; }
+        if constexpr (FOLD) {
+            const long long sb = (long long)b * a.Tout * a.Co + co0 + dc;
+            if constexpr (DYF == FOLD_POOL) {
+                if (d_ok) vload<4>(fg, a.fold.gp + (long long)b * a.Co + co0 + dc);
+                else fg[0] = fg[1] = fg[2] = fg[3] = 0.f;
+            }
+#pragma unroll
+            for (int p = 0; p < DPASS; ++p) {
+                const int t = t0 + dr + 16 * p;
+                dv[p] = d_ok && t < a.Tout;
+                if (dv[p]) {
+                    vload<4>(rd[p], a.fold.y + sb + (long long)t * a.Co);
+                    if constexpr (DYF == FOLD_G) vload<4>(rg[p], a.fold.g + sb + (long long)t * a.Co);
+                }
+            }
+        } else {
+#pragma unroll
+            for (int p = 0; p < DPASS; ++p) {
+                const int t = t0 + dr + 16 * p;
+                if (d_ok && t < a.Tout) vload<4>(rd[p], dyb + (long long)t * a.Co);
+                else { rd[p][0] = rd[p][1] = rd[p][2] = rd[p][3] = 0.f; }
+            }
         }
 #pragma unroll
         for (int p = 0; p < XPASS; ++p) {
@@ -557,7 +620,20 @@
         __bf16* Q = P + NPL * PPLANE;
 #pragma unroll
         for (int p = 0; p < DPASS; ++p) {
-            if constexpr (NP == 2) {
+            if constexpr (DYF == FOLD_G) {
+#pragma unroll
+                for (int v = 0; v < 4; ++v) {
+                    rd[p][v] = dv[p] ? fmaf(fa[v], rg[p][v], fmaf(f1[v], rd[p][v], f0[v])) : 0.f;
+                    if constexpr (NP == 2) rd[p][v] *= sdy;
+                }
+            } else if constexpr (DYF == FOLD_POOL) {
+#pragma unroll
+                for (int v = 0; v < 4; ++v) {
+                    const float gv = (fmaf(fa[v], rd[p][v], fb[v]) > 0.f) ? fg[v] * a.fold.invT : 0.f;
+                    rd[p][v] = dv[p] ? fmaf(fa[v], gv, fmaf(f1[v], rd[p][v], f0[v])) : 0.f;
+                    if constexpr (NP == 2) rd[p][v] *= sdy;
+                }
+            } else if constexpr (NP == 2) {
 #pragma unroll
                 for (int v = 0; v < 4; ++v) rd[p][v] *= sdy;
             }
@@ -809,6 +885,31 @@
     return ign_check_launch("clconv_x6t_kernel");
 }
 
+template <int MODE, int NP>
+static int launch_x6t_fold(const ConvX6Args& a, hipStream_t s) {
+    static bool once = false;
+    if (!once) {
+        (void)hipFuncSetAttribute(reinterpret_cast<const void*>(&clconv_x6t_kernel<4, MODE, EPI_MASK_STATS, NP>),
+                                  hipFuncAttributeMaxDynamicSharedMemorySize, (int)X6tLds<NP>::BYTES);
+        once = true;
+    }
+    hipLaunchKernelGGL((clconv_x6t_kernel<4, MODE, EPI_MASK_STATS, NP>), dim3((unsigned)(a.g.mtiles * a.g.ntiles)), dim3(256),
+                       X6tLds<NP>::BYTES, s, a);
+    return ign_check_launch("clconv_x6t_kernel");
+}
+
+int ign_clconv_launch_x6t_fold(const ConvX6Args& a, int mode, hipStream_t s) {
+    if (a.cin % 4 || (mode != FOLD_G && mode != FOLD_POOL) || (a.nprod != 1 && a.nprod != 3 && a.nprod != 6)) {
+        ign_set_error("ign_clconv_launch_x6t_fold: needs C %% 4 == 0, a fold mode and a split arithmetic (C=%d mode=%d nprod=%d)", a.cin, mode,
+                      a.nprod);
+        return IGN_E_UNSUP;
+    }
+    if (mode == FOLD_G)
+        return a.nprod == 1 ? launch_x6t_fold<FOLD_G, 1>(a, s) : a.nprod == 3 ? launch_x6t_fold<FOLD_G, 2>(a, s) : launch_x6t_fold<FOLD_G, 3>(a, s);
+    return a.nprod == 1 ? launch_x6t_fold<FOLD_POOL, 1>(a, s) : a.nprod == 3 ? launch_x6t_fold<FOLD_POOL, 2>(a, s)
+                                                                             : launch_x6t_fold<FOLD_POOL, 3>(a, s);
+}
+
 template <int NP, int EPI = EPI_BIAS_STATS>
 static int launch_x6w(const ConvX6Args& a, hipStream_t s) {
     static bool once = false;
@@ -901,24 +1002,30 @@
     return ign_check_launch("pack_weights_x3t_multi_kernel");
 }
 
-template <int KT, int NR, int NP>
+template <int KT, int NR, int NP, int DYF = FOLD_NONE>
 static int launch_wgrad_x6(const WgradX6Args& a, int V, bool pro, dim3 grid, hipStream_t s) {
     constexpr size_t lds = (size_t)2 * (NP == 2 ? 2 : 3) * ((16 * NR) + (16 * NR + KT - 1)) * WG_PITCH * sizeof(unsigned short);
 #define IGN_WG(VV, PP)                                                                                                       \
     do {                                                                                                                     \
         static bool once = false;                                                                                            \
         if (!once) {                                                                                                         \
-            (void)hipFuncSetAttribute(reinterpret_cast<const void*>(&clconv_wgrad_x6_kernel<KT, NR, VV, PP, NP>),             \
+            (void)hipFuncSetAttribute(reinterpret_cast<const void*>(&clconv_wgrad_x6_kernel<KT, NR, VV, PP, NP, DYF>),        \
                                       hipFuncAttributeMaxDynamicSharedMemorySize, (int)lds);                                 \
             once = true;                                                                                                     \
         }                                                                                                                    \
-        hipLaunchKernelGGL((clconv_wgrad_x6_kernel<KT, NR, VV, PP, NP>), grid, dim3(256), lds, s, a);                         \
+        hipLaunchKernelGGL((clconv_wgrad_x6_kernel<KT, NR, VV, PP, NP, DYF>), grid, dim3(256), lds, s, a);                    \
     } while (0)
     if (V == 4) { if (pro) IGN_WG(4, true); else IGN_WG(4, false); }
     else if (V == 2) { if (pro) IGN_WG(2, true); else IGN_WG(2, false); }
     else { if (pro) IGN_WG(1, true); else IGN_WG(1, false); }
 #undef IGN_WG
     return ign_check_launch("clconv_wgrad_x6_kernel");
+}
+template <int KT, int NR, int NP>
+static int launch_wgrad_x6_dyf(const WgradX6Args& a, int dyf, int V, bool pro, dim3 grid, hipStream_t s) {
+    if (dyf == FOLD_G) return launch_wgrad_x6<KT, NR, NP, FOLD_G>(a, V, pro, grid, s);
+    if (dyf == FOLD_POOL) return launch_wgrad_x6<KT, NR, NP, FOLD_POOL>(a, V, pro, grid, s);
+    return launch_wgrad_x6<KT, NR, NP>(a, V, pro, grid, s);
 }
 
 static int wgrad_x6_rows_per_unit(int k) { return (k == 8 || k == 5) ? 16 : (k == 3 || k == 2) ? 32 : 0; }
@@ -953,7 +1060,8 @@
 template <int NP>
 static int wgrad_x6_impl(const char* who, const float* dyp, int dy_pad, const float* x, const float* pro_a, const float* pro_b,
                          float* dw_oik, void* workspace, int B, int Tin, int Ci, int Co, int k, void* stream,
-                         float* db = nullptr, const float* bound_dy = nullptr, const float* bound_x = nullptr) {
+                         float* db = nullptr, const float* bound_dy = nullptr, const float* bound_x = nullptr,
+                         const BnBwdFold* fold = nullptr, int dyf = FOLD_NONE) {
     const int Tout = Tin - k + 1, ru = wgrad_x6_rows_per_unit(k);
     const bool defer = dw_oik == nullptr && k > 1;
     if (!dyp || !x || (!dw_oik && !defer) || !workspace || B <= 0 || Ci <= 0 || Co <= 0 || k <= 0 || Tout <= 0 || dy_pad < 0 ||
@@ -962,6 +1070,7 @@
         return IGN_E_ARG;
     }
     hipStream_t s = (hipStream_t)stream;
+    if (dyf != FOLD_NONE && (k == 1 || !fold)) { ign_set_error("%s: the folded BatchNorm backward needs k > 1", who); return IGN_E_UNSUP; }
     if (k == 1) {
         if (Co % 4 || Ci % 4 || dy_pad || pro_a) {
             ign_set_error("%s: k = 1 needs Co %% 4 == 0, Ci %% 4 == 0, no padding, no prologue (Co=%d Ci=%d)", who, Co, Ci);
@@ -998,6 +1107,7 @@
     a.part = (float*)workspace; a.B = B; a.Tin = Tin; a.Tout = Tout; a.Ci = Ci; a.Co = Co; a.k = k;
     a.cps = (Tout + ru - 1) / ru; a.nunits = B * a.cps;
     a.bound_dy = bound_dy; a.bound_x = bound_x;
+    if (fold) a.fold = *fold;
     a.citiles = (Ci + 63) / 64;
     const int tiles = ((Co + 63) / 64) * a.citiles;
     a.nsplit = wgrad_x6_splits(a.nunits, tiles);
@@ -1007,10 +1117,10 @@
     int rc;
     {
         IgnScopedTimer tm("clconv_wgrad", s);
-        if (k == 8) rc = launch_wgrad_x6<8, 1, NP>(a, V, pro, grid, s);
-        else if (k == 5) rc = launch_wgrad_x6<5, 1, NP>(a, V, pro, grid, s);
-        else if (k == 3) rc = launch_wgrad_x6<3, 2, NP>(a, V, pro, grid, s);
-        else rc = launch_wgrad_x6<2, 2, NP>(a, V, pro, grid, s);
+        if (k == 8) rc = launch_wgrad_x6_dyf<8, 1, NP>(a, dyf, V, pro, grid, s);
+        else if (k == 5) rc = launch_wgrad_x6_dyf<5, 1, NP>(a, dyf, V, pro, grid, s);
+        else if (k == 3) rc = launch_wgrad_x6_dyf<3, 2, NP>(a, dyf, V, pro, grid, s);
+        else rc = launch_wgrad_x6_dyf<2, 2, NP>(a, dyf, V, pro, grid, s);
     }
     if (rc) return rc;
     if (defer) return 0;
@@ -1059,3 +1169,27 @@
     if (M <= 0 || M > 0x7fffffffLL) { ign_set_error("ign_linear_wgrad_bf16: M = %lld rows out of range", M); return IGN_E_ARG; }
     return wgrad_x6_impl<1>("ign_linear_wgrad_bf16", dy, 0, x, nullptr, nullptr, dw, workspace, 1, (int)M, Ci, Co, 1, stream, db);
 }
+
+extern "C" int ign_clconv_wgrad_fold(int nprod, const float* g, const float* gpool, const float* y, const float* fa, const float* fb,
+                                     const float* c1, const float* c0, const float* x, const float* pro_a, const float* pro_b,
+                                     float* dw_oik, void* workspace, const float* bound_dy, const float* bound_x, int B, int Tin,
+                                     int Ci, int Co, int k, void* stream) {
+    const int Tout = Tin - k + 1;
+    if (!y || !fa || !c1 || !c0 || (!g && (!gpool || !fb)) || Tout <= 0 || (nprod == 3 && (!bound_dy || !bound_x))) {
+        ign_set_error("ign_clconv_wgrad_fold: null operand / coefficient / bound or Tout <= 0");
+        return IGN_E_ARG;
+    }
+    BnBwdFold f{g, gpool, y, fa, fb, c1, c0, Tout, 0, 1.0f / (float)Tout};
+    const int dyf = g ? FOLD_G : FOLD_POOL;
+    if (nprod == 3)
+        return wgrad_x6_impl<2>("ign_clconv_wgrad_fold", y, 0, x, pro_a, pro_b, dw_oik, workspace, B, Tin, Ci, Co, k, stream, nullptr,
+                                bound_dy, bound_x, &f, dyf);
+    if (nprod == 1)
+        return wgrad_x6_impl<1>("ign_clconv_wgrad_fold", y, 0, x, pro_a, pro_b, dw_oik, workspace, B, Tin, Ci, Co, k, stream, nullptr,
+                                nullptr, nullptr, &f, dyf);
+    if (nprod == 6)
+        return wgrad_x6_impl<3>("ign_clconv_wgrad_fold", y, 0, x, pro_a, pro_b, dw_oik, workspace, B, Tin, Ci, Co, k, stream, nullptr,
+                                nullptr, nullptr, &f, dyf);
+    ign_set_error("ign_clconv_wgrad_fold: nprod = %d is not 6, 1 or 3", nprod);
+    return IGN_E_ARG;
+}
diff --git a/speech-imagery-eeg_amd/ign_hip/_lib.py b/speech-imagery-eeg_amd/ign_hip/_lib.py
--- a/speech-imagery-eeg_amd/ign_hip/_lib.py
+++ b/speech-imagery-eeg_amd/ign_hip/_lib.py
@@ -118,6 +118,11 @@
     "ign_clconv_wgrad_h3": (ci, [vp, ci, vp, vp, vp, vp, vp, vp, vp, ci, ci, ci, ci, ci, vp]),
     "ign_linear_wgrad_h3": (ci, [vp, vp, vp, vp, vp, vp, vp, ll, ci, ci, vp]),
     "ign_bn_bwd_apply_amax": (ci, [vp, vp, vp, vp, vp, vp, vp, vp, vp, ci, ci, ci, ci, ci, vp]),
+    "ign_bn_relu_pool_bwd_ext": (ci, [vp, vp, vp, vp, vp, vp, vp, vp, ci, ci, ci, vp]),
+    "ign_bn_finalize_bwd_pool": (ci, [vp, vp, vp, ci, ci, ci, vp, vp, vp, vp, vp, vp, vp, vp, vp]),
+    "ign_bn_finalize_bwd_fold": (ci, [vp, ci, ll, ci, vp, vp, vp, vp, vp, vp, vp, vp]),
+    "ign_clconv_dgrad_fold": (ci, [ci, vp, vp, vp, vp, vp, vp, vp, vp, vp, vp, vp, vp, vp, vp, vp, vp, vp, vp, ci, ci, ci, ci, ci, vp]),
+    "ign_clconv_wgrad_fold": (ci, [ci, vp, vp, vp, vp, vp, vp, vp, vp, vp, vp, vp, vp, vp, vp, ci, ci, ci, ci, ci, vp]),
     "ign_head_bwd_acc": (ci, [vp, vp, vp, vp, vp, vp, vp, vp, ci, ci, ci, ll, vp]),
     "ign_loss_fwd_bwd_reg": (ci, [vp, vp, vp, vp, vp, vp, vp, vp, vp, ci, ci, cf, vp]),
     "ign_sbm_reg_workspace_bytes": (sz, [ci, ci, ll]),
diff --git a/speech-imagery-eeg_amd/ign_hip/fcn.py b/speech-imagery-eeg_amd/ign_hip/fcn.py
--- a/speech-imagery-eeg_amd/ign_hip/fcn.py
+++ b/speech-imagery-eeg_amd/ign_hip/fcn.py
@@ -8,6 +8,7 @@
 
 CONV_MATH = os.environ.get("IGN_CONV_MATH", "f16x3")
 DEBUG = None
+FOLD_BN = True
 
 
 def _ptr(t):
@@ -161,6 +162,8 @@
             wds.append(wd)
             shapes.append((Co, Ci, k, Tin, Tout))
             pa, pb = a, bb
+        fold = FOLD_BN and x6 and need_grad and nl <= 8 and all(st.use_batch_stats for st in states) and \
+            all(sh[2] in (2, 3, 5, 8) for sh in shapes)
         y_last = inputs[-1]
         Cl, Tl = y_last.shape[2], y_last.shape[1]
         pooled = torch.empty(B, Cl, **f32)
@@ -180,7 +183,7 @@
                        "ign_bn_relu_pool_fwd")
         ctx.head = head
         ctx.head_needs = tuple(ctx.needs_input_grad[-2:]) if has_head else None
-        ctx.saved = (inputs, affine, wds, shapes, [st.use_batch_stats for st in states], math, slots, zbuf, xbound) \
+        ctx.saved = (inputs, affine, wds, shapes, [st.use_batch_stats for st in states], math, slots, zbuf, xbound, fold) \
             if (need_grad or (has_head and any(ctx.head_needs))) else None
         ctx.body_grad = need_grad
         return out
@@ -192,7 +195,7 @@
         if ctx.needs_input_grad[0]:
             raise _lib.IgnError("fcn_body: gradient w.r.t. the input series is not implemented (inputs are data)")
         L = _lib.lib()
-        inputs, affine, wds, shapes, batch_stats, math, slots, zbuf, xbound = ctx.saved
+        inputs, affine, wds, shapes, batch_stats, math, slots, zbuf, xbound, fold = ctx.saved
         h3 = math == "f16x3"
         x6 = math in ("bf16x6", "bf16", "f16x3")
         fp = lambda t, off: ctypes.c_void_p(t.data_ptr() + 4 * off)
@@ -222,6 +225,11 @@
             ztot += Co_ if bs_ else 0
         if zbuf is None or zbuf.numel() != ztot:
             zbuf = torch.zeros(ztot, **f32) if ztot else None
+
+        if fold:
+            grads = _backward_folded(L, gpool, inputs, affine, wds, shapes, math, slots, xbound, zbuf, zoff)
+            ctx.saved = None
+            return (None, None, *grads, *head_grads)
 
         Co, Ci, k, Tin, Tout = shapes[-1]
         a, bb, mean, invstd = affine[-1]
@@ -293,6 +301,87 @@
         return (None, None, *grads, *head_grads)
 
 
+def _backward_folded(L, gpool, inputs, affine, wds, shapes, math, slots, xbound, zbuf, zoff):
+    h3 = math == "f16x3"
+    nprod = {"bf16x6": 6, "bf16": 1, "f16x3": 3}[math]
+    fp = lambda t, off: ctypes.c_void_p(t.data_ptr() + 4 * off)
+    nl = len(shapes)
+    B = inputs[0].shape[0]
+    f32 = dict(device=gpool.device, dtype=torch.float32)
+    grads = [None] * (4 * nl)
+    deferred = []
+    g = part = nparts = None
+    for l in range(nl - 1, -1, -1):
+        Co, Ci, k, Tin, Tout = shapes[l]
+        a, bb, mean, invstd = affine[l]
+        y = inputs[l + 1]
+        dbeta, dgamma = torch.empty(Co, **f32), torch.empty(Co, **f32)
+        dyb = fp(slots, 4 * l + 2) if h3 else None
+        pad = (k - 1) if l > 0 else 0
+        dyp = None
+        if l == nl - 1:
+            nparts = int(L.ign_bn_relu_pool_bwd_parts(B, Tout))
+            part = torch.empty(nparts, 2, Co, **f32)
+            ext = torch.empty(nparts, 4, Co, **f32)
+            _lib.check(L.ign_bn_relu_pool_bwd_ext(_ptr(y), _ptr(gpool), _ptr(a), _ptr(bb), _ptr(mean), _ptr(invstd), _ptr(part), _ptr(ext),
+                                                  B, Tout, Co, _stream()), "ign_bn_relu_pool_bwd_ext")
+            c1, c0 = torch.empty(Co, **f32), torch.empty(Co, **f32)
+            _lib.check(L.ign_bn_finalize_bwd_pool(_ptr(part), _ptr(ext), _ptr(gpool), B, Tout, Co, _ptr(a), _ptr(mean), _ptr(invstd),
+                                                  _ptr(dbeta), _ptr(dgamma), _ptr(c1), _ptr(c0), dyb, _stream()), "ign_bn_finalize_bwd_pool")
+            fold_args = (None, _ptr(gpool), _ptr(y), _ptr(a), _ptr(bb), _ptr(c1), _ptr(c0))
+        elif h3:
+            _lib.check(L.ign_bn_finalize_bwd(_ptr(part), nparts, Co, _ptr(dbeta), _ptr(dgamma), _stream()), "ign_bn_finalize_bwd")
+            dyp = torch.empty(B, Tout + 2 * pad, Co, **f32)
+            _lib.check(L.ign_bn_bwd_apply_amax(_ptr(g), _ptr(y), _ptr(a), _ptr(mean), _ptr(invstd), _ptr(dbeta), _ptr(dgamma), _ptr(dyp),
+                                               dyb, B, Tout, Co, pad, 1, _stream()), "ign_bn_bwd_apply")
+        else:
+            c1, c0 = torch.empty(Co, **f32), torch.empty(Co, **f32)
+            _lib.check(L.ign_bn_finalize_bwd_fold(_ptr(part), nparts, B * Tout, Co, _ptr(a), _ptr(mean), _ptr(invstd), _ptr(dbeta),
+                                                  _ptr(dgamma), _ptr(c1), _ptr(c0), _stream()), "ign_bn_finalize_bwd_fold")
+            fold_args = (_ptr(g), None, _ptr(y), _ptr(a), None, _ptr(c1), _ptr(c0))
+        if DEBUG is not None:
+            DEBUG[f"dbeta{l}"], DEBUG[f"dgamma{l}"] = dbeta.clone(), dgamma.clone()
+            if dyp is not None:
+                DEBUG[f"dyp{l}"] = dyp.clone()
+        pa, pb = (affine[l - 1][0], affine[l - 1][1]) if l > 0 else (None, None)
+        ws = torch.empty(int(L.ign_clconv_wgrad_x6_workspace_bytes(B, Tin, Ci, Co, k)) // 4, **f32)
+        dw = torch.empty(Co, Ci, k, **f32)
+        xb = (fp(slots, 4 * l + 1) if l else _ptr(xbound)) if h3 else None
+        if dyp is not None:
+            _lib.check(L.ign_clconv_wgrad_h3(_ptr(dyp), pad, _ptr(inputs[l]), _ptr(pa), _ptr(pb), None, _ptr(ws), dyb, xb, B, Tin, Ci, Co, k,
+                                             _stream()), "ign_clconv_wgrad_h3")
+        else:
+            _lib.check(L.ign_clconv_wgrad_fold(nprod, *fold_args, _ptr(inputs[l]), _ptr(pa), _ptr(pb), None, _ptr(ws), dyb, xb, B, Tin, Ci,
+                                               Co, k, _stream()), "ign_clconv_wgrad_fold")
+        deferred.append((ws, dw, int(L.ign_clconv_wgrad_x6_nsplit(B, Tin, Ci, Co, k)), Co, Ci, k))
+        grads[4 * l + 0] = dw
+        grads[4 * l + 1] = zbuf[zoff[l]:zoff[l] + Co]
+        grads[4 * l + 2] = dgamma
+        grads[4 * l + 3] = dbeta
+        if l > 0:
+            pa_, pb_, pm_, pi_ = affine[l - 1]
+            gn = torch.empty(B, Tin, Ci, **f32)
+            nparts = int(L.ign_clconv_x6_mtiles(B, Tin))
+            part = torch.empty(nparts, 2, Ci, **f32)
+            wb = fp(slots, 4 * l) if h3 else None
+            if dyp is not None:
+                _lib.check(L.ign_clconv_dgrad_h3(_ptr(dyp), _ptr(wds[l]), _ptr(inputs[l]), _ptr(pa_), _ptr(pb_), _ptr(pm_), _ptr(pi_),
+                                                 _ptr(gn), _ptr(part), dyb, wb, B, Tin, Ci, Co, k, _stream()), "ign_clconv_dgrad_h3")
+            else:
+                _lib.check(L.ign_clconv_dgrad_fold(nprod, *fold_args, _ptr(wds[l]), _ptr(inputs[l]), _ptr(pa_), _ptr(pb_), _ptr(pm_),
+                                                   _ptr(pi_), _ptr(gn), _ptr(part), dyb, wb, None, B, Tin, Ci, Co, k, _stream()),
+                           "ign_clconv_dgrad_fold")
+            g = gn
+        del dyp
+    n = len(deferred)
+    vpa, ia = ctypes.c_void_p * n, ctypes.c_int * n
+    _lib.check(L.ign_clconv_wgrad_reduce_multi(n, vpa(*[d[0].data_ptr() for d in deferred]), vpa(*[d[1].data_ptr() for d in deferred]),
+                                               ia(*[d[2] for d in deferred]), ia(*[d[3] for d in deferred]),
+                                               ia(*[d[4] for d in deferred]), ia(*[d[5] for d in deferred]), _stream()),
+               "ign_clconv_wgrad_reduce_multi")
+    return grads
+
+
 def fcn_body(x, blocks, math=None, head=None):
     if math is None:
         math = "bf16" if torch.is_autocast_enabled() else CONV_MATH
```

After: 2.878, median of 6. Within noise of the previous version (-0.1%).
